# lsl036/STM-Multifrontal-QR-Factorization-Empowered-by-GCN

Hardware: AMD Instinct MI355X
Metric: numerical-factorization GFLOP/s (higher is better)
Workload: dtype f64; 1 GPU; xenon1_colamd_standin: m=49248 n=49248 nnz=1258432 fronts=686 flops/step=5.029e+11, ordering default (COLAMD: qrtest without an ordering argument) (stand-in for xenon1.mtx, absent from the reference checkout); inputs=values resident in HBM, factors left in HBM, parallelism=replica x1, levels=16, retries=0

## Files before the change

include/stmmqr_hip.h:

```cpp
#ifndef STMMQR_HIP_H
#define STMMQR_HIP_H

#include <stddef.h>

#ifdef __cplusplus
extern "C" {
#endif

typedef long stm_long;

#define STMMQR_OK                0
#define STMMQR_ERR_OUT_OF_MEMORY (-2)
#define STMMQR_ERR_TOO_LARGE     (-3)
#define STMMQR_ERR_INVALID       (-4)
#define STMMQR_ERR_DEVICE        (-5)
#define STMMQR_ERR_RESCHEDULE    (-6)


typedef struct stm_sparse_csc {
    size_t nrow, ncol, nzmax;
    void *p, *i, *nz, *x, *z;
    int stype, itype, xtype, dtype, sorted, packed;
} stm_sparse_csc;

typedef struct stm_qr_symbolic {
    stm_long m, n, anz;
    stm_long *Sp, *Sj, *Qfill, *PLinv, *Sleft;
    stm_long nf, maxfn;
    stm_long *Parent, *Child, *Childp, *Super, *Rp, *Rj, *Post;
    stm_long rjsize, do_rank_detection, maxstack, hisize, keepH;
    stm_long *Hip;
    stm_long ntasks, ns;
    stm_long *TaskChildp, *TaskChild, *TaskStack, *TaskFront, *TaskFrontp, *On_stack, *Stack_maxstack;
    stm_long *Fm, *Cm;
} stm_qr_symbolic;

typedef struct stm_qr_numeric {
    double **Rblock;
    double **Stacks;
    stm_long *Stack_size;
    stm_long hisize, n, m, nf, ntasks, ns, maxstack;
    char *Rdead;
    stm_long rank, rank1, maxfrank;
    double norm_E_fro;
    stm_long keepH, rjsize;
    stm_long *HStair;
    double *HTau;
    stm_long *Hii, *HPinv, *Hm, *Hr;
    stm_long maxfm;
} stm_qr_numeric;

typedef struct sparse_common_struct stm_sparse_common;
typedef struct stm_common_layout {
    size_t status, malloc_count, memory_usage, memory_inuse, blas_ok;
    size_t SPQR_grain, SPQR_small, SPQR_shrink, SPQR_flopcount, SPQR_flopcount_bound;
} stm_common_layout;
void stmmqr_set_common_layout(const stm_common_layout *layout);
void stmmqr_get_common_layout(stm_common_layout *layout);
void *stmmqr_cc_malloc(size_t n, size_t size, stm_sparse_common *cc);
void stmmqr_cc_free(size_t n, size_t size, void *p, stm_sparse_common *cc);
void stmmqr_cc_set_status(stm_sparse_common *cc, int code);


stm_qr_numeric *qr_factorize(stm_sparse_csc **Ahandle, stm_long freeA, double tol, stm_long ntol,
                             stm_qr_symbolic *QRsym, stm_sparse_common *cc);

void stmmqr_plan_cache_clear(void);
void stmmqr_free_numeric(stm_qr_numeric **QRnum, stm_sparse_common *cc);

int chunk_getSettings(size_t fchunk, size_t small_, size_t minchunk, size_t minchunk_ratio);

void qr_stranspose2(stm_sparse_csc *A, stm_long *Qfill, stm_long *Sp, stm_long *PLinv, double *Sx, stm_long *W);
void qr_hpinv(stm_qr_symbolic *QRsym, stm_qr_numeric *QRnum, stm_long *W);
stm_long qr_fsize(stm_long f, stm_long *Super, stm_long *Rp, stm_long *Rj, stm_long *Sleft, stm_long *Child,
                  stm_long *Childp, stm_long *Cm, stm_long *Fmap, stm_long *Stair);
void qr_assemble(stm_long f, stm_long fm, int keepH, stm_long *Super, stm_long *Rp, stm_long *Rj, stm_long *Sp,
                 stm_long *Sj, stm_long *Sleft, stm_long *Child, stm_long *Childp, double *Sx, stm_long *Fmap,
                 stm_long *Cm, double **Cblock, stm_long *Hr, stm_long *Stair, stm_long *Hii, stm_long *Hip,
                 double *F, stm_long *Cmap);
stm_long qr_csize(stm_long c, stm_long *Rp, stm_long *Cm, stm_long *Super);
stm_long qr_front(stm_long m, stm_long n, stm_long npiv, double tol, stm_long ntol, stm_long fchunk, double *F,
                  stm_long *Stair, char *Rdead, double *Tau, double *W, double *wscale, double *wssq,
                  stm_sparse_common *cc);
stm_long qr_fcsize(stm_long m, stm_long n, stm_long npiv, stm_long g);
stm_long qr_cpack(stm_long m, stm_long n, stm_long npiv, stm_long g, double *F, double *C);
stm_long qr_rhpack(int keepH, stm_long m, stm_long n, stm_long npiv, stm_long *Stair, double *F, double *R,
                   stm_long *p_rm);
void qr_larftb(int method, stm_long m, stm_long n, stm_long k, stm_long ldc, stm_long ldv, double *V,
               double *Tau, double *C, double *W, stm_sparse_common *cc);


typedef struct stmmqr_symbolic_view {
    stm_long m, n, anz, nf, maxfn, rjsize, hisize, do_rank_detection;
    const stm_long *Sp, *Sj, *Qfill, *PLinv, *Sleft;
    const stm_long *Child, *Childp, *Super, *Rp, *Rj, *Post, *Hip, *Fm;
    stm_long maxstack;
} stmmqr_symbolic_view;

typedef struct stmmqr_stats {
    double flops;
    double ms_total;
    double ms_assemble;
    double ms_front;
    double ms_pack;
    double ms_h2d, ms_d2h;
    double ms_host;
    double bytes_assemble;
    double bytes_pack;
    double flops_update;
    double ms_update;
    stm_long nlaunch;
    stm_long nlevels;
    double ms_panel;
    double ms_small;
    stm_long npanel_launch, nupdate_launch;
    stm_long nsteps;
    double flops_update_pair;
    stm_long retries;
    double device_bytes;
    stm_long reschedules;
} stmmqr_stats;

typedef struct stmmqr_plan stmmqr_plan;

stmmqr_plan *stmmqr_plan_create(const stmmqr_symbolic_view *sym, int device, int *status);
void stmmqr_plan_destroy(stmmqr_plan *plan);

int stmmqr_plan_set_pattern(stmmqr_plan *plan, const stm_long *Ap, const stm_long *Ai);

int stmmqr_factorize_device(stmmqr_plan *plan, const stm_long *Ap, const stm_long *Ai, const double *Ax,
                            int ax_on_device, double tol, stm_long ntol, stmmqr_stats *stats);

int stmmqr_factorize_begin(stmmqr_plan *plan, const stm_long *Ap, const stm_long *Ai, const double *Ax,
                           int ax_on_device, double tol, stm_long ntol);
int stmmqr_factorize_group(stmmqr_plan *plan, int group, int detail);
int stmmqr_factorize_finish(stmmqr_plan *plan, stmmqr_stats *stats);

int stmmqr_plan_set_groups(stmmqr_plan *plan, const int *group );
int stmmqr_plan_front_info(stmmqr_plan *plan, stm_long f, stm_long *info);
int stmmqr_plan_export_front(stmmqr_plan *plan, stm_long f, double *C, stm_long *rows, int c_on_device);
int stmmqr_plan_import_front(stmmqr_plan *plan, stm_long f, stm_long fm, stm_long rank, stm_long cm, const double *C,
                             const stm_long *rows, int c_on_device);

#define STMMQR_GROUP_SHARED  (1 << 30)
#define STMMQR_STEP_PREP     1
#define STMMQR_STEP_PANEL    2
#define STMMQR_STEP_UPDATE   4
#define STMMQR_STEP_GRAM     8
#define STMMQR_STEP_POST     16
int stmmqr_plan_group_steps(stmmqr_plan *plan, int group);
int stmmqr_factorize_step(stmmqr_plan *plan, int group, int step, int what, int cb_first, int cb_stride, int cb_count);
int stmmqr_plan_panel_doubles(stmmqr_plan *plan, stm_long f, stm_long *ndoubles);
int stmmqr_plan_export_panel(stmmqr_plan *plan, stm_long f, stm_long p, double *buf, int on_device);
int stmmqr_plan_import_panel(stmmqr_plan *plan, stm_long f, stm_long p, const double *buf, int on_device);
int stmmqr_plan_export_front_cols(stmmqr_plan *plan, stm_long f, int part, int nparts, double *buf, int on_device,
                                  stm_long *ndoubles);
int stmmqr_plan_import_front_cols(stmmqr_plan *plan, stm_long f, int part, int nparts, const double *buf, int on_device);
typedef struct stmmqr_transport {
    void *ctx;
    int (*send)(void *ctx, const void *dev_buf, size_t bytes, int peer, void *hip_stream);
    int (*recv)(void *ctx, void *dev_buf, size_t bytes, int peer, void *hip_stream);
    int (*group_begin)(void *ctx);
    int (*group_end)(void *ctx);
    int rank, size;
} stmmqr_transport;
int stmmqr_factorize_shared_front(stmmqr_plan *plan, int group, stm_long f, int first_rank, int nranks, const stmmqr_transport *tr);
int stmmqr_factorize_exchange(stmmqr_plan *plan, stm_long nout, const stm_long *out_front, const int *out_peer, stm_long nin,
                              const stm_long *in_front, const int *in_peer, const stmmqr_transport *tr);
int stmmqr_shared_front_gather(stmmqr_plan *plan, stm_long f, int first_rank, int nranks, const stmmqr_transport *tr);
int stmmqr_plan_set_early_end(stmmqr_plan *plan, int mode);
typedef struct stmmqr_shard_phases {
    int nphase;
    const stm_long *out_ptr, *out_front;
    const int *out_peer;
    const stm_long *in_ptr, *in_front;
    const int *in_peer;
    const stm_long *shared_front;
    const int *shared_first, *shared_span;
    const int *has_group;
} stmmqr_shard_phases;
int stmmqr_factorize_phases(stmmqr_plan *plan, const stmmqr_shard_phases *ph, const stmmqr_transport *tr);
int stmmqr_device_copy(void *dst, const void *src, size_t bytes, void *hip_stream);
int stmmqr_rccl_unique_id(char id[128]);
int stmmqr_rccl_transport_create(int world, int rank, const char id[128], stmmqr_transport **out);
void stmmqr_rccl_transport_destroy(stmmqr_transport *tr);
int stmmqr_transport_sendrecv(const stmmqr_transport *tr, const void *sendbuf, size_t sendbytes, int dst, void *recvbuf, size_t recvbytes,
                              int src, void *hip_stream);

int stmmqr_plan_front_rhoff(stmmqr_plan *plan, stm_long f, stm_long *off);

double stmmqr_plan_device_bytes(const stmmqr_plan *plan);

int stmmqr_plan_front_flops(stmmqr_plan *plan, stm_long f, double *out);

int stmmqr_plan_result_sizes(const stmmqr_plan *plan, stm_long *rh_total, stm_long *rank);

int stmmqr_plan_download(stmmqr_plan *plan, double *Stack, stm_long *Rblock_off, char *Rdead, stm_long *HStair,
                         double *HTau, stm_long *Hii, stm_long *HPinv, stm_long *Hm, stm_long *Hr,
                         stm_long *scalars , stmmqr_stats *stats);

int stmmqr_factorize_arrays(const stmmqr_symbolic_view *sym, const stm_long *Ap, const stm_long *Ai,
                            const double *Ax, double tol, stm_long ntol, double *Stack, stm_long stack_cap,
                            stm_long *Rblock_off, char *Rdead, stm_long *HStair, double *HTau, stm_long *Hii,
                            stm_long *HPinv, stm_long *Hm, stm_long *Hr, stm_long *scalars, stmmqr_stats *stats);

int stmmqr_plan_qmult(stmmqr_plan *plan, int method, double *X, stm_long ldx, stm_long nrhs);
int stmmqr_plan_solve(stmmqr_plan *plan, const double *B, stm_long ldb, double *X, stm_long ldx, stm_long nrhs);
int stmmqr_plan_rsolve(stmmqr_plan *plan, int system, const double *B, stm_long ldb, double *X, stm_long ldx,
                       stm_long nrhs);

stm_long stmmqr_front(stm_long m, stm_long n, stm_long npiv, double tol, stm_long ntol, double *F,
                      stm_long *Stair, char *Rdead, double *Tau, double *flops);
int stmmqr_larftb_qtx(stm_long m, stm_long n, stm_long k, stm_long ldc, stm_long ldv, const double *V,
                      const double *Tau, double *C);
int stmmqr_larftb(int method, stm_long m, stm_long n, stm_long k, stm_long ldc, stm_long ldv, const double *V,
                  const double *Tau, double *C);
double stmmqr_last_seam_ms(void);

typedef struct stmmqr_options {
    int panel_width;
    int big_front_cols;
    int verbose;
    int use_graph;
    int panel_algo;
    int split_update;
    int tall_min_rows;
    int lookahead;
    int fused_update;
    int pair_update;
} stmmqr_options;
void stmmqr_get_options(stmmqr_options *opt);
void stmmqr_set_options(const stmmqr_options *opt);

int stmmqr_read_matrix_market(const char *path, stm_long *nrow, stm_long *ncol, stm_long *nnz, stm_long **Ap,
                              stm_long **Ai, double **Ax);
const char *stmmqr_mm_last_error(void);
void stmmqr_free(void *p);

typedef struct stmmqr_relax { stm_long nrelax[3]; double zrelax[3]; } stmmqr_relax;
typedef struct stmmqr_analysis stmmqr_analysis;
void stmmqr_relax_for_qr(stm_long n, stm_long nnz, stmmqr_relax *relax);
int stmmqr_analyze(stm_long m, stm_long n, const stm_long *Ap, const stm_long *Ai, const stm_long *Quser,
                   int do_rank_detection, const stmmqr_relax *relax, stmmqr_analysis **out);
const stm_qr_symbolic *stmmqr_analysis_symbolic(const stmmqr_analysis *a);
int stmmqr_analysis_info(const stmmqr_analysis *a, double *info);
void stmmqr_analysis_free(stmmqr_analysis *a);

typedef struct stmmqr_qr stmmqr_qr;
int stmmqr_sparseqr(int ordering, double tol, stm_long m, stm_long n, const stm_long *Ap, const stm_long *Ai, const double *Ax,
                    const stm_long *Quser, const stmmqr_relax *relax, int device, stmmqr_qr **out);
int stmmqr_sparseqr_symbolic(int ordering, double tol, stm_long m, stm_long n, const stm_long *Ap, const stm_long *Ai,
                             const double *Ax, const stm_long *Quser, const stmmqr_relax *relax, stmmqr_qr **out);
int stmmqr_sparseqr_numeric(stmmqr_qr *qr, int device);
void stmmqr_sparseqr_free(stmmqr_qr *qr);
int stmmqr_sparseqr_info(const stmmqr_qr *qr, double *info);
double stmmqr_sparseqr_tol(const stmmqr_qr *qr);
const stm_long *stmmqr_sparseqr_q1fill(const stmmqr_qr *qr);
const stm_qr_symbolic *stmmqr_sparseqr_symbolic_view(const stmmqr_qr *qr);
stmmqr_plan *stmmqr_sparseqr_plan(stmmqr_qr *qr);
int stmmqr_sparseqr_y(const stmmqr_qr *qr, const stm_long **Yp, const stm_long **Yi, const double **Yx);
int stmmqr_sparseqr_qmult(stmmqr_qr *qr, int method, const double *X, stm_long ldx, stm_long nrow, stm_long ncol, double *Y,
                          stm_long ldy);
int stmmqr_sparseqr_solve(stmmqr_qr *qr, int system, const double *B, stm_long ldb, stm_long nrhs, double *X, stm_long ldx);

void qr_rcount(stm_qr_symbolic *QRsym, stm_qr_numeric *QRnum, stm_long n1rows, stm_long econ, stm_long n2, int getT, stm_long *Ra,
               stm_long *Rb, stm_long *H2p, stm_long *p_nh);
void qr_rconvert(stm_qr_symbolic *QRsym, stm_qr_numeric *QRnum, stm_long n1rows, stm_long econ, stm_long n2, int getT,
                 stm_long *Rap, stm_long *Rai, double *Rax, stm_long *Rbp, stm_long *Rbi, double *Rbx, stm_long *H2p, stm_long *H2i,
                 double *H2x, double *H2Tau);
stm_long qr_trapezoidal(stm_long n, stm_long *Rp, stm_long *Ri, double *Rx, stm_long bncols, stm_long *Qfill,
                        int skip_if_trapezoidal, stm_long **p_Tp, stm_long **p_Ti, double **p_Tx, stm_long **p_Qtrap,
                        stm_sparse_common *cc);
int stmmqr_plan_export_r(stmmqr_plan *plan, const stm_qr_symbolic *sym, stm_long econ, stm_long **Rp, stm_long **Ri, double **Rx,
                         stm_long *nh, stm_long **Hp, stm_long **Hi, double **Hx, double **HTau);
int stmmqr_sparselq(int ordering, double tol, stm_long m, stm_long n, const stm_long *Ap, const stm_long *Ai, const double *Ax,
                    const stmmqr_relax *relax, int device, stmmqr_qr **out);

void stmmqr_shutdown(void);
int stmmqr_device_alloc(size_t bytes, void **ptr);
int stmmqr_device_free(void *ptr);
int stmmqr_device_count(void);
const char *stmmqr_device_name(int device);
const char *stmmqr_last_error(void);
const char *stmmqr_version(void);

#ifdef __cplusplus
}
#endif
#endif
```

stm-multifrontal-qr-factorization-empowered-by-gcn_amd/capi.py:

```python
from __future__ import annotations

import ctypes as C
from pathlib import Path

import numpy as np

_HERE = Path(__file__).resolve().parent
lib_path = _HERE / "libstmmqr_hip.so"

c_long_p = C.POINTER(C.c_long)
c_double_p = C.POINTER(C.c_double)
I64 = np.int64


class StmmqrError(RuntimeError):
    code = 0


ERR_RESCHEDULE = -6


if not lib_path.exists():
    raise ImportError(
        f"{lib_path} is missing: build it with `python -c 'import __graft_entry__ as g; g.build()'` "
        "(hipcc --offload-arch=gfx950).  There is no CPU fallback for this path.")


def _preload_torch_hip_runtime():
    import importlib.util
    import os
    if os.environ.get("STMMQR_SYSTEM_HIP") == "1":
        return
    try:
        spec = importlib.util.find_spec("torch")
    except (ImportError, ValueError):
        spec = None
    if spec is None or not spec.origin:
        return
    rt = Path(spec.origin).parent / "lib" / "libamdhip64.so"
    if rt.exists():
        C.CDLL(str(rt), mode=C.RTLD_GLOBAL)


_preload_torch_hip_runtime()
lib = C.CDLL(str(lib_path))


class SymbolicView(C.Structure):
    _fields_ = [(k, C.c_long) for k in ["m", "n", "anz", "nf", "maxfn", "rjsize", "hisize", "do_rank_detection"]] + \
               [(k, c_long_p) for k in ["Sp", "Sj", "Qfill", "PLinv", "Sleft", "Child", "Childp", "Super", "Rp", "Rj",
                                        "Post", "Hip", "Fm"]] + [("maxstack", C.c_long)]


class Stats(C.Structure):
    _fields_ = [(k, C.c_double) for k in ["flops", "ms_total", "ms_assemble", "ms_front", "ms_pack", "ms_h2d", "ms_d2h",
                                          "ms_host", "bytes_assemble", "bytes_pack", "flops_update", "ms_update"]] + \
               [("nlaunch", C.c_long), ("nlevels", C.c_long), ("ms_panel", C.c_double), ("ms_small", C.c_double),
                ("npanel_launch", C.c_long), ("nupdate_launch", C.c_long), ("nsteps", C.c_long),
                ("flops_update_pair", C.c_double), ("retries", C.c_long), ("device_bytes", C.c_double), ("reschedules", C.c_long)]

    def as_dict(self):
        return {k: getattr(self, k) for k, _ in self._fields_}


class Options(C.Structure):
    _fields_ = [("panel_width", C.c_int), ("big_front_cols", C.c_int), ("verbose", C.c_int), ("use_graph", C.c_int),
                ("panel_algo", C.c_int), ("split_update", C.c_int), ("tall_min_rows", C.c_int),
                ("lookahead", C.c_int), ("fused_update", C.c_int), ("pair_update", C.c_int)]


def _ip(a):
    return None if a is None else a.ctypes.data_as(c_long_p)


def _dp(a):
    return None if a is None else a.ctypes.data_as(c_double_p)


lib.stmmqr_last_error.restype = C.c_char_p
lib.stmmqr_version.restype = C.c_char_p
lib.stmmqr_device_name.restype = C.c_char_p
lib.stmmqr_device_name.argtypes = [C.c_int]
lib.stmmqr_plan_create.restype = C.c_void_p
lib.stmmqr_plan_create.argtypes = [C.POINTER(SymbolicView), C.c_int, C.POINTER(C.c_int)]
lib.stmmqr_plan_destroy.argtypes = [C.c_void_p]
lib.stmmqr_plan_destroy.restype = None
lib.stmmqr_plan_set_pattern.argtypes = [C.c_void_p, c_long_p, c_long_p]
lib.stmmqr_factorize_device.argtypes = [C.c_void_p, c_long_p, c_long_p, C.c_void_p, C.c_int, C.c_double, C.c_long,
                                        C.POINTER(Stats)]
lib.stmmqr_plan_result_sizes.argtypes = [C.c_void_p, c_long_p, c_long_p]
lib.stmmqr_plan_download.argtypes = [C.c_void_p, c_double_p, c_long_p, C.c_char_p, c_long_p, c_double_p, c_long_p,
                                     c_long_p, c_long_p, c_long_p, c_long_p, C.POINTER(Stats)]
lib.stmmqr_front.restype = C.c_long
lib.stmmqr_front.argtypes = [C.c_long, C.c_long, C.c_long, C.c_double, C.c_long, c_double_p, c_long_p, C.c_char_p,
                             c_double_p, c_double_p]
lib.stmmqr_larftb_qtx.argtypes = [C.c_long] * 5 + [c_double_p, c_double_p, c_double_p]
lib.stmmqr_larftb.argtypes = [C.c_int] + [C.c_long] * 5 + [c_double_p, c_double_p, c_double_p]
lib.qr_larftb.restype = None
lib.qr_larftb.argtypes = [C.c_int] + [C.c_long] * 5 + [c_double_p, c_double_p, c_double_p, c_double_p, C.c_void_p]
lib.stmmqr_last_seam_ms.restype = C.c_double
lib.stmmqr_last_seam_ms.argtypes = []
lib.qr_cpack.restype = C.c_long
lib.qr_cpack.argtypes = [C.c_long] * 4 + [c_double_p, c_double_p]
lib.qr_rhpack.restype = C.c_long
lib.qr_rhpack.argtypes = [C.c_int, C.c_long, C.c_long, C.c_long, c_long_p, c_double_p, c_double_p, c_long_p]
lib.qr_fcsize.restype = C.c_long
lib.qr_fcsize.argtypes = [C.c_long] * 4
lib.qr_assemble.restype = None
lib.qr_assemble.argtypes = [C.c_long, C.c_long, C.c_int] + [c_long_p] * 8 + [c_double_p, c_long_p, c_long_p,
                                                                             C.POINTER(c_double_p), c_long_p, c_long_p,
                                                                             c_long_p, c_long_p, c_double_p, c_long_p]
lib.stmmqr_plan_rsolve.argtypes = [C.c_void_p, C.c_int, c_double_p, C.c_long, c_double_p, C.c_long, C.c_long]
lib.stmmqr_read_matrix_market.argtypes = [C.c_char_p, c_long_p, c_long_p, c_long_p, C.POINTER(c_long_p), C.POINTER(c_long_p), C.POINTER(c_double_p)]
lib.qr_fsize.argtypes = [C.c_long] + [c_long_p] * 9
lib.stmmqr_factorize_begin.argtypes = [C.c_void_p, c_long_p, c_long_p, C.c_void_p, C.c_int, C.c_double, C.c_long]
lib.stmmqr_factorize_group.argtypes = [C.c_void_p, C.c_int, C.c_int]
lib.stmmqr_factorize_finish.argtypes = [C.c_void_p, C.POINTER(Stats)]
lib.stmmqr_plan_set_groups.argtypes = [C.c_void_p, C.POINTER(C.c_int)]
lib.stmmqr_plan_set_early_end.argtypes = [C.c_void_p, C.c_int]
lib.stmmqr_plan_front_info.argtypes = [C.c_void_p, C.c_long, c_long_p]
lib.stmmqr_plan_export_front.argtypes = [C.c_void_p, C.c_long, C.c_void_p, c_long_p, C.c_int]
lib.stmmqr_plan_import_front.argtypes = [C.c_void_p, C.c_long, C.c_long, C.c_long, C.c_long, C.c_void_p, c_long_p, C.c_int]
lib.stmmqr_plan_qmult.argtypes = [C.c_void_p, C.c_int, c_double_p, C.c_long, C.c_long]
lib.stmmqr_plan_group_steps.argtypes = [C.c_void_p, C.c_int]
lib.stmmqr_factorize_step.argtypes = [C.c_void_p] + [C.c_int] * 6
lib.stmmqr_plan_panel_doubles.argtypes = [C.c_void_p, C.c_long, c_long_p]
lib.stmmqr_plan_export_panel.argtypes = [C.c_void_p, C.c_long, C.c_long, C.c_void_p, C.c_int]
lib.stmmqr_plan_import_panel.argtypes = [C.c_void_p, C.c_long, C.c_long, C.c_void_p, C.c_int]
lib.stmmqr_plan_export_front_cols.argtypes = [C.c_void_p, C.c_long, C.c_int, C.c_int, C.c_void_p, C.c_int, c_long_p]
lib.stmmqr_plan_import_front_cols.argtypes = [C.c_void_p, C.c_long, C.c_int, C.c_int, C.c_void_p, C.c_int]
lib.stmmqr_plan_front_rhoff.argtypes = [C.c_void_p, C.c_long, c_long_p]
lib.stmmqr_plan_front_flops.argtypes = [C.c_void_p, C.c_long, c_double_p]
lib.stmmqr_plan_device_bytes.argtypes = [C.c_void_p]
lib.stmmqr_plan_device_bytes.restype = C.c_double
lib.stmmqr_plan_solve.argtypes = [C.c_void_p, c_double_p, C.c_long, c_double_p, C.c_long, C.c_long]
lib.stmmqr_get_options.argtypes = [C.POINTER(Options)]
lib.stmmqr_set_options.argtypes = [C.POINTER(Options)]


class TransportC(C.Structure):
    SEND = C.CFUNCTYPE(C.c_int, C.c_void_p, C.c_void_p, C.c_size_t, C.c_int, C.c_void_p)
    RECV = C.CFUNCTYPE(C.c_int, C.c_void_p, C.c_void_p, C.c_size_t, C.c_int, C.c_void_p)
    GRP = C.CFUNCTYPE(C.c_int, C.c_void_p)
    _fields_ = [("ctx", C.c_void_p), ("send", SEND), ("recv", RECV), ("group_begin", GRP), ("group_end", GRP), ("rank", C.c_int),
                ("size", C.c_int)]


lib.stmmqr_factorize_shared_front.argtypes = [C.c_void_p, C.c_int, C.c_long, C.c_int, C.c_int, C.POINTER(TransportC)]


class ShardPhasesC(C.Structure):
    _LP, _IP = C.POINTER(C.c_long), C.POINTER(C.c_int)
    _fields_ = [("nphase", C.c_int), ("out_ptr", _LP), ("out_front", _LP), ("out_peer", _IP), ("in_ptr", _LP), ("in_front", _LP),
                ("in_peer", _IP), ("shared_front", _LP), ("shared_first", _IP), ("shared_span", _IP), ("has_group", _IP)]


lib.stmmqr_factorize_exchange.argtypes = [C.c_void_p, C.c_long, C.POINTER(C.c_long), C.POINTER(C.c_int), C.c_long, C.POINTER(C.c_long),
                                          C.POINTER(C.c_int), C.POINTER(TransportC)]
lib.stmmqr_shared_front_gather.argtypes = [C.c_void_p, C.c_long, C.c_int, C.c_int, C.POINTER(TransportC)]
lib.stmmqr_factorize_phases.argtypes = [C.c_void_p, C.POINTER(ShardPhasesC), C.POINTER(TransportC)]
lib.stmmqr_rccl_unique_id.argtypes = [C.c_char_p]
lib.stmmqr_rccl_transport_create.argtypes = [C.c_int, C.c_int, C.c_char_p, C.POINTER(C.POINTER(TransportC))]
lib.stmmqr_rccl_transport_destroy.restype = None
lib.stmmqr_rccl_transport_destroy.argtypes = [C.POINTER(TransportC)]
lib.stmmqr_transport_sendrecv.argtypes = [C.POINTER(TransportC), C.c_void_p, C.c_size_t, C.c_int, C.c_void_p, C.c_size_t, C.c_int, C.c_void_p]
lib.stmmqr_device_copy.argtypes = [C.c_void_p, C.c_void_p, C.c_size_t, C.c_void_p]


class RcclTransport:

    def __init__(self, dist, device=None):
        import torch
        rank, world = dist.get_rank(), dist.get_world_size()
        ident = C.create_string_buffer(128)
        if rank == 0:
            _check(lib.stmmqr_rccl_unique_id(ident), "stmmqr_rccl_unique_id")
        t = torch.frombuffer(bytearray(ident.raw), dtype=torch.uint8).clone()
        if device is not None and dist.get_backend() == "nccl":
            t = t.to(device)
        dist.broadcast(t, 0)
        raw = bytes(t.cpu().numpy().tobytes())
        self._p = C.POINTER(TransportC)()
        _check(lib.stmmqr_rccl_transport_create(world, rank, raw, C.byref(self._p)), "stmmqr_rccl_transport_create")
        self.rank, self.size = rank, world

    @property
    def ptr(self):
        return self._p

    def sendrecv(self, send_ptr, send_bytes, dst, recv_ptr, recv_bytes, src, stream=None):
        _check(lib.stmmqr_transport_sendrecv(self._p, send_ptr, send_bytes, dst, recv_ptr, recv_bytes, src, stream), "stmmqr_transport_sendrecv")

    def close(self):
        if self._p:
            lib.stmmqr_rccl_transport_destroy(self._p)
            self._p = C.POINTER(TransportC)()


class CallbackTransport:

    def __init__(self, rank, size, send, recv):
        self._send = TransportC.SEND(lambda ctx, buf, nbytes, peer, stream: int(send(buf, nbytes, peer, stream) or 0))
        self._recv = TransportC.RECV(lambda ctx, buf, nbytes, peer, stream: int(recv(buf, nbytes, peer, stream) or 0))
        self._t = TransportC(None, self._send, self._recv, TransportC.GRP(), TransportC.GRP(), rank, size)
        self.rank, self.size = rank, size

    @property
    def ptr(self):
        return C.pointer(self._t)


def device_copy(dst: int, src: int, nbytes: int, stream=None):
    _check(lib.stmmqr_device_copy(C.c_void_p(dst), C.c_void_p(src), nbytes, stream), "stmmqr_device_copy")


def last_error() -> str:
    return lib.stmmqr_last_error().decode()


def device_count() -> int:
    return int(lib.stmmqr_device_count())


def device_name(i: int = 0) -> str:
    return lib.stmmqr_device_name(i).decode()


def get_options() -> dict:
    o = Options()
    lib.stmmqr_get_options(C.byref(o))
    return {k: getattr(o, k) for k, _ in o._fields_}


lib.stmmqr_device_alloc.argtypes = [C.c_size_t, C.POINTER(C.c_void_p)]
lib.stmmqr_device_free.argtypes = [C.c_void_p]


def device_alloc(nbytes: int) -> int:
    p = C.c_void_p()
    _check(lib.stmmqr_device_alloc(nbytes, C.byref(p)), "stmmqr_device_alloc")
    return p.value


def device_free(ptr: int):
    _check(lib.stmmqr_device_free(ptr), "stmmqr_device_free")


def set_options(**kw):
    o = Options()
    lib.stmmqr_get_options(C.byref(o))
    for k, v in kw.items():
        setattr(o, k, v)
    lib.stmmqr_set_options(C.byref(o))


def _check(rc: int, what: str):
    if rc != 0:
        e = StmmqrError(f"{what} failed ({rc}): {last_error()}")
        e.code = int(rc)
        raise e


class QRNumeric:

    def __init__(self, nf, n, m, rjsize, hisize, rh_total):
        self.Stack = np.zeros(max(rh_total, 1))
        self.Rblock_off = np.zeros(max(nf, 1), I64)
        self.Rdead = np.zeros(max(n, 1), np.int8)
        self.HStair = np.zeros(max(rjsize, 1), I64)
        self.HTau = np.zeros(max(rjsize, 1))
        self.Hii = np.zeros(max(hisize, 1), I64)
        self.HPinv = np.zeros(max(m, 1), I64)
        self.Hm = np.zeros(max(nf, 1), I64)
        self.Hr = np.zeros(max(nf, 1), I64)
        self.rh_total = rh_total
        self.rank = self.rank1 = self.maxfrank = self.maxfm = 0
        self.stats = {}


class HipQR:

    def __init__(self, sym: dict, device: int = -1):
        self._keep = {}
        v = SymbolicView()
        for k in ["m", "n", "anz", "nf", "maxfn", "rjsize", "hisize", "do_rank_detection"]:
            setattr(v, k, int(sym[k]))
        for k in ["Sp", "Sj", "Qfill", "PLinv", "Sleft", "Child", "Childp", "Super", "Rp", "Rj", "Post", "Hip", "Fm"]:
            a = sym.get(k)
            if a is not None and np.size(a) == 0 and k == "Qfill":
                a = None
            if a is not None:
                a = np.ascontiguousarray(a, dtype=I64)
                self._keep[k] = a
            setattr(v, k, _ip(a))
        v.maxstack = int(sym.get("maxstack", 0) or 0)
        self.sym = {k: int(sym[k]) for k in ["m", "n", "anz", "nf", "maxfn", "rjsize", "hisize"]}
        st = C.c_int(0)
        self._h = lib.stmmqr_plan_create(C.byref(v), device, C.byref(st))
        if not self._h:
            raise StmmqrError(f"stmmqr_plan_create failed ({st.value}): {last_error()}")

    def close(self):
        if getattr(self, "_h", None):
            lib.stmmqr_plan_destroy(self._h)
            self._h = None

    __del__ = close

    def set_pattern(self, Ap, Ai):
        Ap = np.ascontiguousarray(Ap, I64); Ai = np.ascontiguousarray(Ai, I64)
        _check(lib.stmmqr_plan_set_pattern(self._h, _ip(Ap), _ip(Ai)), "stmmqr_plan_set_pattern")

    def factorize(self, Ax, tol, ntol, Ap=None, Ai=None, device_ptr: int | None = None, detail=False) -> dict:
        st = Stats()
        if detail:
            st.nlaunch = -1
        if Ap is not None:
            Ap = np.ascontiguousarray(Ap, I64); Ai = np.ascontiguousarray(Ai, I64)
        if device_ptr is not None:
            rc = lib.stmmqr_factorize_device(self._h, _ip(Ap), _ip(Ai), C.c_void_p(device_ptr), 1, float(tol), int(ntol),
                                             C.byref(st))
        else:
            Ax = np.ascontiguousarray(Ax, np.float64)
            rc = lib.stmmqr_factorize_device(self._h, _ip(Ap), _ip(Ai), Ax.ctypes.data_as(C.c_void_p), 0, float(tol),
                                             int(ntol), C.byref(st))
        _check(rc, "stmmqr_factorize_device")
        return st.as_dict()

    def set_groups(self, group):
        g = np.ascontiguousarray(group, np.int32)
        assert g.size == self.sym["nf"]
        _check(lib.stmmqr_plan_set_groups(self._h, g.ctypes.data_as(C.POINTER(C.c_int))), "stmmqr_plan_set_groups")

    def set_early_end(self, mode: int):
        _check(lib.stmmqr_plan_set_early_end(self._h, int(mode)), "stmmqr_plan_set_early_end")

    def begin(self, Ax, tol, ntol, Ap=None, Ai=None, device_ptr=None):
        if Ap is not None:
            Ap = np.ascontiguousarray(Ap, I64); Ai = np.ascontiguousarray(Ai, I64)
        if device_ptr is not None:
            rc = lib.stmmqr_factorize_begin(self._h, _ip(Ap), _ip(Ai), C.c_void_p(device_ptr), 1, float(tol), int(ntol))
        else:
            Ax = np.ascontiguousarray(Ax, np.float64)
            rc = lib.stmmqr_factorize_begin(self._h, _ip(Ap), _ip(Ai), Ax.ctypes.data_as(C.c_void_p), 0, float(tol), int(ntol))
        _check(rc, "stmmqr_factorize_begin")

    def run_group(self, g, detail=False):
        _check(lib.stmmqr_factorize_group(self._h, int(g), int(detail)), "stmmqr_factorize_group")

    def finish(self) -> dict:
        st = Stats()
        _check(lib.stmmqr_factorize_finish(self._h, C.byref(st)), "stmmqr_factorize_finish")
        return st.as_dict()

    def front_info(self, f) -> dict:
        info = np.zeros(6, I64)
        _check(lib.stmmqr_plan_front_info(self._h, int(f), _ip(info)), "stmmqr_plan_front_info")
        return dict(zip(["fm", "rank", "cm", "csize", "fn", "fp"], (int(x) for x in info)))

    def export_front(self, f):
        info = self.front_info(f)
        Cb = np.zeros(max(info["csize"], 1)); rows = np.zeros(max(info["cm"], 1), I64)
# ... 551 lines not shown
```

stm-multifrontal-qr-factorization-empowered-by-gcn_amd/csrc/stmmqr_host.cpp:

```cpp
#include "stmmqr_plan.h"

thread_local std::string g_err;
stmmqr_options g_opt = {STM_NB, 64, 0, 0, 0, 1, STM_TALL_MIN, 2, 0, 4};
size_t g_chunk[4] = {32, 5000, 4, 4};

stm_common_layout g_layout = {
     1004,  1032,  1040,  1048,
     1100,  1104,  1112,  1120,
     1128,  1136};

int fail(int code, const std::string &msg)
{
    g_err = msg;
    if (g_opt.verbose) fprintf(stderr, "[stmmqr_hip] error %d: %s\n", code, msg.c_str());
    return code;
}

namespace {

const int LDS_CAP_DOUBLES = STM_LDS_CAP_DOUBLES;
const int LDS_CAP_SMALL = 15360;

std::mutex g_side_mu;
hipStream_t g_side[64] = {};
// ... 153 lines not shown
            *objs[(size_t)i].out = at;
            peak = std::max(peak, top);
        }
    }
    return peak;
}

std::pair<long long, long long> timeline_offsets(stmmqr_plan &P, const std::vector<char> &kept, int nstep, bool apply)
{
    const long nf = P.nf;
    std::vector<long long> foff((size_t)std::max(1L, nf), 0), coff((size_t)std::max(1L, nf), 0);
    long long base = 0;
    for (long f = 0; f < nf; f++)
        if (kept[(size_t)f]) { foff[(size_t)f] = base; base += (long long)P.fs[f].ld * P.fs[f].fn; }
    std::vector<TlObj> fo, co;
    for (long f = 0; f < nf; f++) {
        const FrontSym &s = P.fs[f];
        if (!kept[(size_t)f]) fo.push_back({(long long)s.ld * s.fn, P.f_t0[f], P.f_t1[f], &foff[(size_t)f]});
        const long cn = s.fn - s.fp, fm = s.fm_ub;
        const long cm = P.do_rank ? std::min(fm, cn) : std::min(std::max(fm - std::min(fm, (long)s.fp), 0L), cn);
        const long long csz = (long long)cm * (cm + 1) / 2 + (long long)cm * (cn - cm);
        if (apply) P.c_slot[(size_t)f] = csz;
        co.push_back({csz, P.f_t1[f], std::max(P.f_t1[f], P.c_t1[f]), &coff[(size_t)f]});
    }
    const long long fpeak = timeline_first_fit(fo, base, nstep), cpeak = timeline_first_fit(co, 0, nstep);
    if (apply)
        for (long f = 0; f < nf; f++) { P.fs[f].foff = foff[(size_t)f]; P.fs[f].coff = coff[(size_t)f]; }
    return {std::max(1LL, fpeak), std::max(1LL, cpeak)};
}

void build_schedule(stmmqr_plan &P, std::vector<int> &tslot)
{
    P.sched_gen++;
    P.tune = getenv("STMMQR_TUNE") ? atoi(getenv("STMMQR_TUNE")) : 0;
    P.tall_min = g_opt.tall_min_rows;
    P.plan_algo = g_opt.panel_algo;
    P.ca_min = getenv("STMMQR_CA_MIN") ? atoi(getenv("STMMQR_CA_MIN")) : STM_CA_MIN_ROWS;
    const long nf = P.nf;
    int ngroups = 1;
    for (long f = 0; f < nf; f++) ngroups = std::max(ngroups, P.group[f] + 1);
    {
        bool whole = (ngroups == 1) && nf > 0;
        for (long f = 0; f < nf && whole; f++) whole = (P.group[f] == 0) && !((size_t)f < P.shared.size() && P.shared[(size_t)f]);
        const char *ev = getenv("STMMQR_RECYCLE");
        const int mode = ev ? atoi(ev) : 1;
        long long slabs = 0;
        for (long f = 0; f < nf; f++) slabs += (long long)P.fs[f].ld * P.fs[f].fn;
        P.recycle = whole && !P.overflowed && (mode == 2 || (mode == 1 && slabs >= (32LL << 20)));
    }
    auto is_big = [&](int f) {
        const FrontSym &s = P.fs[f];
        return s.fn >= g_opt.big_front_cols && s.fm_ub >= 64;
    };
    const int sched_policy = getenv("STMMQR_SCHED") ? atoi(getenv("STMMQR_SCHED")) : 0;
    const long pair_min = getenv("STMMQR_PAIR_MIN") ? atol(getenv("STMMQR_PAIR_MIN")) : STM_PAIR_MIN_ROWS;
    auto is_pair = [&](int f) {
        const FrontSym &s = P.fs[f];
        if ((size_t)f < P.shared.size() && P.shared[f]) return false;
        return g_opt.pair_update && is_big(f) && s.fm_est >= pair_min && s.npanels >= 4;
    };
    P.sweep = (g_opt.pair_update == 4) ? 4 : 2;
    P.pair_front.assign(std::max(1L, nf), 0);
    for (long f = 0; f < nf; f++) P.pair_front[f] = (P.group[f] >= 0 && is_pair((int)f)) ? 1 : 0;
    P.ypoff.assign(std::max(1L, nf), -1);
    P.yp_doubles = 0;
    for (long f = 0; f < nf; f++)
        if (P.pair_front[f]) {
            P.ypoff[f] = P.yp_doubles;
            P.yp_doubles += (long long)((P.fs[f].fn + 31) / 32) * (P.sweep * STM_NB * 32);
        }
    tslot.assign(std::max(1L, nf), 0);
    P.glevels.assign(ngroups, std::vector<Level>());
    P.gsteps.assign(ngroups, std::vector<Step>());
    P.lists.clear();
    P.wlists.clear();
    P.tslots = 1;
    P.gp_slabs = 1;
    P.wp_doubles = 0;
    P.wp2_doubles = 0;
    {
        bool whole = (ngroups == 1) && nf > 0;
        for (long f = 0; f < nf && whole; f++) whole = (P.group[f] == 0) && !((size_t)f < P.shared.size() && P.shared[(size_t)f]);
        const bool early = (whole || P.early_phased) && !P.full_schedule && !(getenv("STMMQR_EARLY_END") && atoi(getenv("STMMQR_EARLY_END")) == 0);
        const int slack = getenv("STMMQR_EARLY_SLACK") ? atoi(getenv("STMMQR_EARLY_SLACK")) : 0;
        for (long f = 0; f < nf; f++) {
            FrontSym &s = P.fs[f];
            s.nsched = s.npanels;
            if (early && is_big((int)f) && !is_pair((int)f) && P.group[f] >= 0 && !((size_t)f < P.shared.size() && P.shared[(size_t)f])) s.nsched = std::min(s.npanels, std::min(s.fm_est, s.fn) / STM_NB + 1 + slack);
        }
        P.early_end = early;
    }
    for (int grp = 0; grp < ngroups; grp++) {
        std::vector<int> level(nf, -1), start(nf, 0), end(nf, 0);
        int nlev = 0, nstep = 0;
        for (long kf = 0; kf < nf; kf++) {
            const long f = P.Post[kf];
            if (P.group[f] != grp) continue;
            int lv = 0, t0 = 0;
            for (long q = P.Childp[f]; q < P.Childp[f + 1]; q++) {
                const long ch = P.Child[q];
                if (P.group[ch] != grp) continue;
                lv = std::max(lv, level[ch] + 1);
                t0 = std::max(t0, end[ch]);
            }
            level[f] = lv;
            nlev = std::max(nlev, lv + 1);
            start[f] = t0;
            end[f] = t0 + (is_big((int)f) ? P.fs[f].nsched : 1);
            nstep = std::max(nstep, end[f]);
        }
        std::vector<int> lstart(nf, 0), lend(nf, 0);
        int nstep_level = 0;
        {
            std::vector<int> lvl_end(nlev + 1, 0);
            for (int lv = 0; lv < nlev; lv++) {
                int e1 = lvl_end[lv];
                for (long kf = 0; kf < nf; kf++) {
                    const long f = P.Post[kf];
                    if (P.group[f] != grp || level[f] != lv) continue;
                    lstart[f] = lvl_end[lv];
                    lend[f] = lstart[f] + (is_big((int)f) ? P.fs[f].nsched : 1);
                    e1 = std::max(e1, lend[f]);
                }
                lvl_end[lv + 1] = e1;
            }
            nstep_level = lvl_end[nlev];
        }
        const bool use_level = sched_policy == 1 || (sched_policy == 0 && 100L * nstep > 97L * nstep_level);
        if (use_level) {
            start = lstart; end = lend;
            nstep = nstep_level;
        }
        std::vector<std::vector<int>> byl(nlev);
        for (long kf = 0; kf < nf; kf++)
            if (P.group[P.Post[kf]] == grp) byl[level[P.Post[kf]]].push_back((int)P.Post[kf]);
        std::vector<Level> &LV = P.glevels[grp];
        LV.assign(nlev, Level());
        for (int lv = 0; lv < nlev; lv++) {
            Level &L = LV[lv];
            std::vector<int> small, big;
            for (int f : byl[lv]) (is_big(f) ? big : small).push_back(f);
            std::stable_sort(big.begin(), big.end(), [&](int a, int b) { return P.fs[a].npanels > P.fs[b].npanels; });
            L.all_off = (int)P.lists.size();
            L.n_small = (int)small.size(); L.n_big = (int)big.size(); L.n_all = L.n_small + L.n_big;
            P.lists.insert(P.lists.end(), small.begin(), small.end());
            P.lists.insert(P.lists.end(), big.begin(), big.end());
        }
        std::vector<std::vector<std::pair<int, int>>> panel_at;
        std::vector<std::vector<int>> small_at;
        if (use_level || sched_policy == 2) {
            panel_at.assign(nstep, {});
            small_at.assign(nstep, {});
            for (long kf = 0; kf < nf; kf++) {
                const int f = (int)P.Post[kf];
                if (P.group[f] != grp) continue;
                if (!is_big(f)) { small_at[start[f]].push_back(f); continue; }
                for (int q = 0; q < P.fs[f].nsched; q++) panel_at[start[f] + q].push_back({f, q});
            }
        } else {
            std::vector<int> parent_in(nf, -1), pend(nf, 0), tails(nf, 0);
            for (long f = 0; f < nf; f++) {
                if (P.group[f] != grp) continue;
                for (long q = P.Childp[f]; q < P.Childp[f + 1]; q++)
                    if (P.group[P.Child[q]] == grp) { parent_in[P.Child[q]] = (int)f; pend[f]++; }
            }
            for (long kf = nf; kf-- > 0;) {
                const long f = P.Post[kf];
                if (P.group[f] != grp) continue;
                tails[f] = (is_big((int)f) ? P.fs[f].nsched : 1) + (parent_in[f] >= 0 ? tails[parent_in[f]] : 0);
            }
            std::vector<int> ready;
            for (long kf = 0; kf < nf; kf++)
                if (P.group[P.Post[kf]] == grp && pend[P.Post[kf]] == 0) ready.push_back((int)P.Post[kf]);
            const double ride = getenv("STMMQR_RIDE") ? atof(getenv("STMMQR_RIDE")) : 1.0;
            struct Fly { int f, p; };
            std::vector<Fly> fly;
            while (!ready.empty() || !fly.empty()) {
                std::vector<int> newly, smalls;
                for (int f : ready) {
                    if (is_big(f)) fly.push_back({f, 0});
                    else smalls.push_back(f);
                }
                panel_at.push_back({});
                small_at.push_back(smalls);
                auto finish = [&](int f) {
                    const int pf = parent_in[f];
                    if (pf >= 0 && --pend[pf] == 0) newly.push_back(pf);
                };
                if (!fly.empty()) {
                    auto rem = [&](const Fly &e) { return tails[e.f] - e.p; };
                    auto rows = [&](const Fly &e) { return stm_panel_rows_est(P.fs[e.f], e.p); };
                    int rl = 0, env = 0;
                    for (const Fly &e : fly) rl = std::max(rl, rem(e));
                    for (const Fly &e : fly)
                        if (rem(e) == rl) env = std::max(env, rows(e));
                    std::vector<Fly> keep;
                    for (Fly &e : fly) {
                        if (rem(e) == rl || rows(e) <= ride * env) {
                            panel_at.back().push_back({e.f, e.p});
                            if (++e.p >= P.fs[e.f].nsched) { finish(e.f); continue; }
                        }
                        keep.push_back(e);
                    }
                    fly.swap(keep);
                }
                for (int f : smalls) finish(f);
                ready.swap(newly);
            }
            nstep = (int)panel_at.size();
        }
        std::vector<std::vector<int>> starting(nstep), ending(nstep);
        std::vector<int> pan_now(nf, 0);
        for (int t = 0; t < nstep; t++) {
            for (int f : small_at[t]) starting[t].push_back(f);
            for (const auto &fp : panel_at[t]) {
                if (fp.second == 0) starting[t].push_back(fp.first);
                if (fp.second == P.fs[fp.first].nsched - 1) ending[t].push_back(fp.first);
            }
        }
        for (int t = 0, carry_from = -1; t < nstep; t++) {
            const bool flush = (t + 1 == nstep) || !starting[t + 1].empty();
            if (carry_from >= 0 && carry_from != t) {
                ending[t].insert(ending[t].begin(), ending[carry_from].begin(), ending[carry_from].end());
                ending[carry_from].clear();
            }
            carry_from = (flush || ending[t].empty()) ? -1 : t;
            if (!flush && !ending[t].empty()) carry_from = t;
        }
        std::vector<Step> &SV = P.gsteps[grp];
        SV.assign(nstep, Step());
        std::vector<int> active, freeslots;
        int nslots = 0;
        for (int t = 0; t < nstep; t++) {
            Step &S = SV[t];
            std::vector<int> small, big;
            for (int f : starting[t]) (is_big(f) ? big : small).push_back(f);
            S.start_off = (int)P.lists.size();
            S.n_small = (int)small.size(); S.n_start = (int)(small.size() + big.size());
            P.lists.insert(P.lists.end(), small.begin(), small.end());
            P.lists.insert(P.lists.end(), big.begin(), big.end());
            S.asm_parts_off = (int)P.lists.size();
            long maxfm_small = 0;
            for (int i = 0; i < S.n_start; i++) {
                const FrontSym &s = P.fs[P.lists[S.start_off + i]];
                const long work = (long)s.fm_ub * s.fn;
                static const long pg = getenv("STMMQR_PART_GRAIN") ? atol(getenv("STMMQR_PART_GRAIN")) : 2048, pc = getenv("STMMQR_PART_CAP") ? atol(getenv("STMMQR_PART_CAP")) : 4096;
                const int parts = (int)std::min(pc, std::max(1L, (work + pg - 1) / pg));
                P.lists.push_back(parts);
                S.asm_maxparts = std::max(S.asm_maxparts, parts);
                if (i < S.n_small) maxfm_small = std::max(maxfm_small, (long)s.fm_ub);
            }
            S.lds_small = (int)std::min((long)LDS_CAP_SMALL, (((maxfm_small + 63) & ~63L) | 1) * STM_NB + 64);
            if (S.n_small > 0) S.lds_small = std::max(S.lds_small, STM_NB * 128 + 64);
            for (int f : big) {
                if (!freeslots.empty()) { tslot[f] = freeslots.back(); freeslots.pop_back(); }
                else tslot[f] = nslots++;
            }
            active.clear();
            for (const auto &fp : panel_at[t]) { active.push_back(fp.first); pan_now[fp.first] = fp.second; }
            auto work_at = [&](int f) { return (long)stm_upd_ncb(P.fs[f], pan_now[f]) * stm_upd_nsl(P.fs[f]); };
            auto cls = [&](int f) { return !is_pair(f) ? 0 : 1 + pan_now[f] % P.sweep; };
            std::stable_sort(active.begin(), active.end(), [&](int a, int b) {
                return cls(a) != cls(b) ? cls(a) < cls(b) : work_at(a) > work_at(b);
            });
            S.act_off = (int)P.lists.size();
            S.n_act = (int)active.size();
            P.lists.insert(P.lists.end(), active.begin(), active.end());
            S.plist_off = (int)P.lists.size();
            for (int f : active) P.lists.push_back(pan_now[f]);
            S.wp_off = (int)P.wlists.size();
            long long wp = 0, ncbsum = 0;
            long maxfm_big = 0;
            for (int f : active) {
                const FrontSym &s = P.fs[f];
                const int p = pan_now[f];
                const int ncb = stm_upd_ncb(s, p), nsl = stm_upd_nsl(s);
                P.wlists.push_back(wp);
                if (is_pair(f))
                    wp += std::max((long long)(ncb + P.sweep - 1) * (P.sweep == 4 ? stm_quad_slots(nsl, P.tune) : stm_pair_slots(nsl, P.tune)) *
                                       (P.sweep * STM_NB * 32),
                                   (P.sweep + 1LL) * nsl * (STM_NB * 32));
                else
                    wp += (long long)(ncb + 1) * nsl * (STM_NB * 32);
                const int k = cls(f);
                if (k == 0) {
                    S.n_norm++;
                    ncbsum += ncb;
                    S.maxcb = std::max(S.maxcb, ncb);
                    S.maxsl = std::max(S.maxsl, nsl);
                } else {
                    S.n_pk[k - 1]++;
                    S.maxsl_pk[k - 1] = std::max(S.maxsl_pk[k - 1], nsl);
                    if (k == P.sweep) S.maxcbp_po = std::max(S.maxcbp_po, ncb - 1);
                }
                S.nsub = std::max(S.nsub, stm_tall_launches(s, p, P.tall_min));
                S.nca = std::max(S.nca, stm_ca_slabs(s));
                (stm_use_ca(s, p, g_opt.panel_algo, P.ca_min) ? S.nca_use : S.npipe_use)++;
                P.gp_slabs = std::max(P.gp_slabs, stm_ca_slabs(s));
                maxfm_big = std::max(maxfm_big, (long)s.fm_ub);
                if (!stm_tall_panel(s, p, P.tall_min) && !stm_use_ca(s, p, g_opt.panel_algo, P.ca_min))
                    S.lds_plan = std::max(S.lds_plan, stm_front_lds(s));
                if (stm_tall_panel(s, p, P.tall_min) && !stm_use_ca(s, p, g_opt.panel_algo, P.ca_min))
                    S.lds_plan = std::max(S.lds_plan, STM_NB * STM_WP_ROWS);
            }
            S.lds_big = (int)std::min((long)LDS_CAP_DOUBLES, (((maxfm_big + 63) & ~63L) | 1) * STM_NB + 64);
            S.split = (S.maxsl >= 3 || ncbsum >= 512) ? 1 : 0;
            P.wp_doubles = std::max(P.wp_doubles, wp);
            if (S.n_sweep() == 0) P.wp2_doubles = std::max(P.wp2_doubles, wp);
            S.cpk_off = (int)P.lists.size();
            S.n_cpk = (int)ending[t].size();
            P.lists.insert(P.lists.end(), ending[t].begin(), ending[t].end());
            S.cpk_parts_off = (int)P.lists.size();
            for (int f : ending[t]) {
                const FrontSym &s = P.fs[f];
                const long cn = s.fn - s.fp;
                const long work = cn * std::min((long)s.fm_ub, cn);
                static const long pg = getenv("STMMQR_PART_GRAIN") ? atol(getenv("STMMQR_PART_GRAIN")) : 2048, pc = getenv("STMMQR_PART_CAP") ? atol(getenv("STMMQR_PART_CAP")) : 4096;
                const int parts = (int)std::min(pc, std::max(1L, (work + pg - 1) / pg));
                P.lists.push_back(parts);
                S.cpk_maxparts = std::max(S.cpk_maxparts, parts);
                freeslots.push_back(tslot[f]);
            }
        }
        P.tslots = std::max(P.tslots, nslots);
        if (P.recycle && grp == 0) {
            P.f_t0.assign((size_t)std::max(1L, nf), 0); P.f_t1.assign((size_t)std::max(1L, nf), 0); P.c_t1.assign((size_t)std::max(1L, nf), 0);
            for (int t = 0; t < nstep; t++) {
                for (int f : starting[t]) { P.f_t0[(size_t)f] = t; if (!is_big(f)) P.f_t1[(size_t)f] = t; }
                for (int f : ending[t]) P.f_t1[(size_t)f] = t;
            }
            for (long f = 0; f < nf; f++) {
                const int par = P.fs[f].parent;
                P.c_t1[(size_t)f] = (par >= 0) ? P.f_t0[(size_t)par] : P.f_t1[(size_t)f];
            }
            std::vector<int> bysize((size_t)nf);
            for (long f = 0; f < nf; f++) bysize[(size_t)f] = (int)f;
            std::stable_sort(bysize.begin(), bysize.end(), [&](int a, int b) {
                return (long long)P.fs[a].ld * P.fs[a].fn > (long long)P.fs[b].ld * P.fs[b].fn; });
            long long best = -1;
            int bestk = 0;
            for (int k = 0; k <= std::min(3L, nf); k++) {
                std::vector<char> kp((size_t)std::max(1L, nf), 0);
                long long rec = 0;
                for (int q = 0; q < k; q++) kp[(size_t)bysize[(size_t)q]] = 1;
                for (long f = 0; f < nf; f++) if (!kp[(size_t)f]) rec += (long long)P.fs[f].ld * P.fs[f].fn;
                const auto pk = timeline_offsets(P, kp, nstep, false);
                const long long cap = (P.maxstack > 0) ? std::min((long long)P.maxstack, rec) : rec;
                const long long tot = pk.first + pk.second + cap;
                if (best < 0 || tot < best - best / 50) { best = tot; bestk = k; }
            }
            P.kept.assign((size_t)std::max(1L, nf), 0);
            long long rec = 0;
            for (int q = 0; q < bestk; q++) P.kept[(size_t)bysize[(size_t)q]] = 1;
            for (long f = 0; f < nf; f++) if (!P.kept[(size_t)f]) rec += (long long)P.fs[f].ld * P.fs[f].fn;
            P.rh_cap = std::max(1LL, (P.maxstack > 0) ? std::min((long long)P.maxstack, rec) : rec);
            if (!P.rh_grow && P.rh_est_total > 0) {
                const double sc = getenv("STMMQR_RH_EST_SCALE") ? atof(getenv("STMMQR_RH_EST_SCALE")) : 1.0;
                const long long est = (long long)((double)P.rh_est_total * sc);
                P.rh_cap = std::max(1LL, std::min(P.rh_cap, est + est / 8 + 4096));
            }
            const auto pk = timeline_offsets(P, P.kept, nstep, true);
            P.farena = pk.first; P.carena = pk.second;
            P.has_c.assign((size_t)std::max(1L, nf), 1);
            for (int t = 0; t < nstep; t++) {
                Step &S = SV[t];
                std::vector<int> rhp;
                for (int f : starting[t]) if (!is_big(f) && !P.kept[(size_t)f]) rhp.push_back(f);
                for (int f : ending[t]) if (!P.kept[(size_t)f]) rhp.push_back(f);
                S.rhp_off = (int)P.lists.size();
                S.n_rhp = (int)rhp.size();
                P.lists.insert(P.lists.end(), rhp.begin(), rhp.end());
                S.rhp_parts_off = (int)P.lists.size();
                for (int f : rhp) {
                    const int parts = std::min(256, std::max(1, P.fs[f].fn / 16));
                    P.lists.push_back(parts);
                    S.rhp_maxparts = std::max(S.rhp_maxparts, parts);
                }
            }
            P.fs_scr = P.fs;
            P.scr_doubles = 1;
            for (size_t l = 0; l < LV.size(); l++) {
                long long o = 0;
                for (int q = 0; q < LV[l].n_all; q++) {
                    const int f = P.lists[(size_t)(LV[l].all_off + q)];
                    if (P.kept[(size_t)f]) continue;
                    P.fs_scr[(size_t)f].foff = o;
                    o += (long long)P.fs[f].ld * P.fs[f].fn;
                }
                P.scr_doubles = std::max(P.scr_doubles, o);
            }
        }
    }
    P.own_off = (int)P.lists.size();
    P.n_own = 0;
    for (long kf = 0; kf < nf; kf++)
        if (P.group[P.Post[kf]] >= 0) { P.lists.push_back((int)P.Post[kf]); P.n_own++; }
    P.rh_parts_off = (int)P.lists.size();
    P.rh_maxparts = 1;
    for (long kf = 0; kf < nf; kf++) {
        if (P.group[P.Post[kf]] < 0) continue;
        const FrontSym &s = P.fs[P.Post[kf]];
        int parts = std::min(256, std::max(1, s.fn / 16));
        P.lists.push_back(parts);
        P.rh_maxparts = std::max(P.rh_maxparts, parts);
    }
    P.post_off = (int)P.lists.size();
    for (long kf = 0; kf < nf; kf++) P.lists.push_back((int)P.Post[kf]);
    if (P.lists.empty()) P.lists.push_back(0);
    if (P.wlists.empty()) P.wlists.push_back(0);
    P.h_tslot = tslot;
}

int upload_recycle(stmmqr_plan &P)
{
    if (!P.d_rhtop.p) LCHK(P.d_rhtop.alloc(2));
    if (!P.d_fin.p || P.d_fin.n < (size_t)std::max(1L, P.nf)) LCHK(P.d_fin.alloc((size_t)std::max(1L, P.nf)));
    HIPCHK(hipMemsetAsync(P.d_rhtop.p, 0, 2 * sizeof(long long), P.stream));
    if (!P.recycle) return 0;
    LCHK(P.d_kept.upload(P.kept, P.stream));
    HIPCHK(hipStreamSynchronize(P.stream));
    P.d_scr.release();
    P.d_RH.release();
    return 0;
}

int build_plan(stmmqr_plan &P, const stmmqr_symbolic_view &v)
{
    P.m = v.m; P.n = v.n; P.anz = v.anz; P.nf = v.nf; P.maxfn = v.maxfn; P.rjsize = v.rjsize;
    P.hisize = v.hisize; P.do_rank = v.do_rank_detection ? 1 : 0;
    P.maxstack = v.maxstack > 0 ? v.maxstack : 0;
    const long m = v.m, n = v.n, nf = v.nf;
    if (m < 0 || n < 0 || nf < 0) return fail(STMMQR_ERR_INVALID, "negative dimension");
    if (v.anz >= (1L << 31) - 1 || v.rjsize >= (1L << 31) - 1 || v.hisize >= (1L << 31) - 1 || m >= (1L << 30) ||
        n >= (1L << 30))
        return fail(STMMQR_ERR_TOO_LARGE, "problem exceeds the 32-bit device index range");
    auto cp = [](std::vector<long> &dst, const stm_long *src, long cnt) {
        dst.assign(src, src + (cnt > 0 ? cnt : 0));
    };
    cp(P.Sp, v.Sp, m + 1); cp(P.Sj, v.Sj, v.anz); cp(P.PLinv, v.PLinv, m); cp(P.Sleft, v.Sleft, n + 2);
    cp(P.Child, v.Child, nf + 1); cp(P.Childp, v.Childp, nf + 2); cp(P.Super, v.Super, nf + 1);
    cp(P.Rp, v.Rp, nf + 1); cp(P.Rj, v.Rj, v.rjsize); cp(P.Post, v.Post, nf); cp(P.Hip, v.Hip, nf + 1);
    P.has_qfill = v.Qfill != nullptr;
    if (P.has_qfill) cp(P.Qfill, v.Qfill, n);

    std::vector<long> parent(nf, -1);
    for (long f = 0; f < nf; f++)
        for (long q = P.Childp[f]; q < P.Childp[f + 1]; q++) parent[P.Child[q]] = f;

    P.Fm.assign(nf, 0);
    if (v.Fm) {
        for (long f = 0; f < nf; f++) P.Fm[f] = v.Fm[f];
    } else {
        std::vector<long> cmub(nf, 0);
        for (long kf = 0; kf < nf; kf++) {
            const long f = P.Post[kf];
            const long fp = P.Super[f + 1] - P.Super[f], fn = P.Rp[f + 1] - P.Rp[f];
            long fm = P.Sleft[P.Super[f + 1]] - P.Sleft[P.Super[f]];
            for (long q = P.Childp[f]; q < P.Childp[f + 1]; q++) fm += cmub[P.Child[q]];
            P.Fm[f] = fm;
            const long cn = fn - fp;
            cmub[f] = P.do_rank ? std::min(fm, cn) : std::min(std::max(fm - std::min(fm, fp), 0L), cn);
        }
    }

    std::vector<long> fmest(nf, 0), cmest(nf, 0);
    for (long kf = 0; kf < nf; kf++) {
        const long f = P.Post[kf];
        const long fp = P.Super[f + 1] - P.Super[f], fn = P.Rp[f + 1] - P.Rp[f];
        long fe = P.Sleft[P.Super[f + 1]] - P.Sleft[P.Super[f]];
        for (long q = P.Childp[f]; q < P.Childp[f + 1]; q++) fe += cmest[P.Child[q]];
        fmest[f] = std::min(fe, P.Fm[f]);
        cmest[f] = std::min(std::max(fe - std::min(fe, fp), 0L), fn - fp);
    }

    P.fs.assign(nf, FrontSym());
    long long foff = 0, coff = 0, tpan_total = 0;
    for (long kf = 0; kf < nf; kf++) {
        const long f = P.Post[kf];
        FrontSym &s = P.fs[f];
        const long fp = P.Super[f + 1] - P.Super[f], fn = P.Rp[f + 1] - P.Rp[f];
        const long fm = P.Fm[f];
        if (fm * fn >= (1L << 36)) return fail(STMMQR_ERR_TOO_LARGE, "a single front exceeds 2^36 entries");
        s.fn = (int)fn; s.fp = (int)fp; s.col1 = (int)P.Super[f]; s.rp = (int)P.Rp[f]; s.hip = (int)P.Hip[f];
        s.child0 = (int)P.Childp[f]; s.child1 = (int)P.Childp[f + 1];
        s.srow0 = (int)P.Sleft[P.Super[f]]; s.srow1 = (int)P.Sleft[P.Super[f + 1]];
        s.fm_ub = (int)fm;
        s.fm_est = (int)fmest[f];
        s.ld = (int)std::max(2L, (fm + 1) & ~1L);
        s.npanels = (int)((fn + STM_NB - 1) / STM_NB);
        s.tpan = (int)tpan_total;
        tpan_total += s.npanels;
        {
            const long qbig_min = getenv("STMMQR_QBIG_MIN") ? atol(getenv("STMMQR_QBIG_MIN")) : (1L << 20);
            s.qbig = (fm * fn >= qbig_min && fn >= 1) ? 1 : 0;
        }
        s.parent = (int)parent[f];
        s.foff = 0; s.coff = 0;
    }
    (void)foff; (void)coff;
    P.tpanels = tpan_total;

    std::vector<int> Rjrel(std::max(1L, v.rjsize), 0), Sjrel(std::max(1L, v.anz), 0), Sj0(std::max(1L, m), -1);
    {
        std::vector<int> Fmap(std::max(1L, n), -1);
        for (long f = 0; f < nf; f++) {
            const long p1 = P.Rp[f], fn = P.Rp[f + 1] - p1;
            for (long j = 0; j < fn; j++) Fmap[P.Rj[p1 + j]] = (int)j;
            for (long r = P.fs[f].srow0; r < P.fs[f].srow1; r++)
                for (long p = P.Sp[r]; p < P.Sp[r + 1]; p++) Sjrel[p] = Fmap[P.Sj[p]];
            for (long q = P.Childp[f]; q < P.Childp[f + 1]; q++) {
                const long c = P.Child[q];
                const long fpc = P.Super[c + 1] - P.Super[c], pc = P.Rp[c] + fpc, cn = P.Rp[c + 1] - pc;
                for (long cj = 0; cj < cn; cj++) Rjrel[pc + cj] = Fmap[P.Rj[pc + cj]];
                P.bytes_assemble_idx += 4.0 * (double)(2 * cn);
            }
        }
        for (long r = 0; r < m; r++)
            if (P.Sp[r + 1] > P.Sp[r]) Sj0[r] = (int)P.Sj[P.Sp[r]];
        P.bytes_assemble_idx += 4.0 * (double)v.anz;
    }
    P.rh_est_total = 0;
    {
        std::vector<long> stair;
        for (long kf = 0; kf < nf; kf++) {
            const long f = P.Post[kf];
            const long fp = P.fs[f].fp, fn = P.fs[f].fn, fm = fmest[f];
            stair.assign((size_t)fn + 1, 0);
            for (long j = 0; j < fp; j++) stair[(size_t)j] = P.Sleft[P.Super[f] + j + 1] - P.Sleft[P.Super[f] + j];
            for (long q = P.Childp[f]; q < P.Childp[f + 1]; q++) {
                const long c = P.Child[q];
                const long fpc = P.Super[c + 1] - P.Super[c], pc = P.Rp[c] + fpc;
                for (long i = 0; i < cmest[c]; i++) stair[(size_t)Rjrel[(size_t)(pc + i)]]++;
            }
            long run = 0;
            for (long j = 0; j < fn; j++) { run += stair[(size_t)j]; stair[(size_t)j] = run; }
            long g = 0, rm = 0;
            long long sz = 0;
            for (long k = 0; k < fn; k++) {
                long t;
                if (g >= fm) t = (k < fp) ? 0 : fm;
                else { t = std::min(fm, std::max(g + 1, stair[(size_t)k])); g++; }
                if (k < fp) { if (t > 0) rm++; sz += (t > 0) ? t : rm; }
                else { const long h = std::min(rm + (k - fp) + 1, fm); sz += rm + std::max(t - h, 0L); }
            }
            P.rh_est_total += sz;
        }
    }

    P.group.assign(nf, 0);
    assign_arenas(P);
    std::vector<int> tslot;
    build_schedule(P, tslot);

    size_t freeb = 0, totalb = 0;
    HIPCHK(hipMemGetInfo(&freeb, &totalb));
    const double need = 8.0 * 1024.0 * (double)P.tpanels * 1.05 + 64.0 * (double)(v.rjsize + v.anz);
    if (need > 0.92 * (double)freeb)
        return fail(STMMQR_ERR_OUT_OF_MEMORY, "the plan's index arrays do not fit in free HBM");
    hipStream_t st = P.stream;
    auto up32 = [&](DevBuf<int> &d, const std::vector<long> &h) {
        std::vector<int> t(h.begin(), h.end());
        return d.upload(t, st);
    };
    LCHK(P.d_fs.upload(P.fs, st));
    LCHK(P.d_fnum.alloc(std::max(1L, nf)));
    HIPCHK(hipMemsetAsync(P.d_fnum.p, 0, std::max(1L, nf) * sizeof(FrontNum), st));
    LCHK(P.d_T.alloc((size_t)STM_PD_RING * P.tslots * STM_NB * STM_NB));
    LCHK(P.d_Gp.alloc((size_t)P.tslots * (P.gp_slabs + 1) * STM_NB * STM_NB));
    LCHK(P.d_Tall.alloc((size_t)std::max(1LL, P.tpanels) * STM_NB * STM_NB));
    LCHK(P.d_Wp.alloc((size_t)P.wp_doubles));
    LCHK(P.d_Ypend.alloc((size_t)std::max(1LL, P.yp_doubles)));
    LCHK(P.d_ypoff.upload(P.ypoff, st));
    LCHK(P.d_Wp2.alloc((size_t)std::max(1LL, P.wp2_doubles)));
    P.wcnt_n = (size_t)(P.wp_doubles / (STM_NB * 32) + 1);
    LCHK(P.d_wcnt.alloc(P.wcnt_n));
    LCHK(P.d_wcnt2.alloc(P.wcnt_n));
    LCHK(P.d_wflag.alloc(P.wcnt_n));
    if (!P.d_abort.p) LCHK(P.d_abort.alloc(4));
    LCHK(P.d_wflag2.alloc(P.wcnt_n));
    HIPCHK(hipMemset(P.d_wcnt.p, 0, P.wcnt_n * sizeof(int)));
    HIPCHK(hipMemset(P.d_wcnt2.p, 0, P.wcnt_n * sizeof(int)));
    LCHK(P.d_tslot.upload(tslot, st));
    LCHK(P.d_Sx.alloc((size_t)v.anz));
    LCHK(P.d_Ax.alloc((size_t)v.anz));
    LCHK(P.d_smap.alloc((size_t)v.anz));
    LCHK(up32(P.d_Sp, P.Sp));
    LCHK(P.d_Sjrel.upload(Sjrel, st));
    LCHK(P.d_Sj0.upload(Sj0, st));
    LCHK(up32(P.d_Sleft, P.Sleft));
    LCHK(up32(P.d_Child, P.Child));
    LCHK(P.d_Rjrel.upload(Rjrel, st));
    LCHK(P.d_Stair.alloc((size_t)v.rjsize));
    LCHK(P.d_Tau.alloc((size_t)v.rjsize));
    LCHK(P.d_Hii.alloc((size_t)v.hisize));
    LCHK(P.d_Cmap.alloc((size_t)v.rjsize));
    LCHK(P.d_Cursor.alloc((size_t)v.rjsize));
    LCHK(P.d_Rhoff.alloc((size_t)v.rjsize));
    LCHK(P.d_Rboff.alloc((size_t)std::max(1L, nf)));
    LCHK(P.d_total.alloc(1));
    LCHK(P.d_dbg.alloc(2048));
    LCHK(P.d_amax.alloc(1));
    LCHK(P.d_sig.alloc(2));
    HIPCHK(hipMemsetAsync(P.d_dbg.p, 0, 2048 * sizeof(unsigned long long), st));
    LCHK(P.d_Rdead.alloc((size_t)std::max(1L, n)));
    LCHK(P.d_lists.upload(P.lists, st));
    LCHK(P.d_wlists.upload(P.wlists, st));
    HIPCHK(hipStreamSynchronize(st));
    LCHK(upload_recycle(P));
    return 0;
}

int set_pattern(stmmqr_plan &P, const stm_long *Ap, const stm_long *Ai)
{
    const long m = P.m, n = P.n;
    if (!Ap || !Ai) return fail(STMMQR_ERR_INVALID, "Ap/Ai are required");
    if (Ap[n] != P.anz) return fail(STMMQR_ERR_INVALID, "nnz(A) differs from the symbolic analysis");
    std::vector<long> W(P.Sp.begin(), P.Sp.begin() + m);
    std::vector<int> smap(std::max(1L, P.anz), 0);
    for (long col = 0; col < n; col++) {
        const long j = P.has_qfill ? P.Qfill[col] : col;
        for (long p = Ap[j]; p < Ap[j + 1]; p++) {
            const long i = Ai[p];
            if (i < 0 || i >= m) return fail(STMMQR_ERR_INVALID, "row index out of range");
            smap[W[P.PLinv[i]]++] = (int)p;
        }
    }
    if (P.anz > 0)
        HIPCHK(hipMemcpyAsync(P.d_smap.p, smap.data(), (size_t)P.anz * sizeof(int), hipMemcpyHostToDevice, P.stream));
    HIPCHK(hipStreamSynchronize(P.stream));
    P.pattern_set = true;
    return 0;
}

int reset_factorization(stmmqr_plan &P)
{
    hipStream_t st = P.stream;
    LCHK(ensure_arenas(P));
    if (!P.recycle) HIPCHK(hipMemsetAsync(P.d_F.p, 0, (size_t)P.farena * sizeof(double), st));
    HIPCHK(hipMemsetAsync(P.d_rhtop.p, 0, 2 * sizeof(long long), st));
    HIPCHK(hipMemsetAsync(P.d_Rdead.p, 0, (size_t)std::max(1L, P.n), st));
    HIPCHK(hipMemsetAsync(P.d_fnum.p, 0, (size_t)std::max(1L, P.nf) * sizeof(FrontNum), st));
    HIPCHK(hipMemsetAsync(P.d_wcnt.p, 0, P.wcnt_n * sizeof(int), st));
    HIPCHK(hipMemsetAsync(P.d_wcnt2.p, 0, P.wcnt_n * sizeof(int), st));
    HIPCHK(hipMemsetAsync(P.d_wflag.p, 0, P.wcnt_n * sizeof(int), st));
    HIPCHK(hipMemsetAsync(P.d_wflag2.p, 0, P.wcnt_n * sizeof(int), st));
    HIPCHK(hipMemsetAsync(P.d_abort.p, 0, 4 * sizeof(int), st));
    LCHK(stm_launch_sigma(P.d_Ax.p, (int)P.anz, P.d_amax.p, P.d_sig.p, st));
    LCHK(stm_launch_gather_sx(P.d_Ax.p, P.d_smap.p, P.d_Sx.p, (int)P.anz, st));
    P.stats.nlaunch += 6;
    return 0;
}

int reset_group(stmmqr_plan &P, int grp)
{
    hipStream_t st = P.stream;
    const FrontNum zero = FrontNum();
    for (long f = 0; f < P.nf; f++) {
        if (P.group[f] != grp) continue;
        const FrontSym &s = P.fs[f];
        HIPCHK(hipMemsetAsync(P.d_F.p + s.foff, 0, (size_t)s.ld * (size_t)s.fn * sizeof(double), st));
        HIPCHK(hipMemcpyAsync(P.d_fnum.p + f, &zero, sizeof zero, hipMemcpyHostToDevice, st));
        if (s.fp > 0) HIPCHK(hipMemsetAsync(P.d_Rdead.p + s.col1, 0, (size_t)s.fp, st));
    }
    HIPCHK(hipMemsetAsync(P.d_wcnt.p, 0, P.wcnt_n * sizeof(int), st));
    HIPCHK(hipMemsetAsync(P.d_wcnt2.p, 0, P.wcnt_n * sizeof(int), st));
    HIPCHK(hipMemsetAsync(P.d_wflag.p, 0, P.wcnt_n * sizeof(int), st));
    HIPCHK(hipMemsetAsync(P.d_wflag2.p, 0, P.wcnt_n * sizeof(int), st));
    HIPCHK(hipMemsetAsync(P.d_abort.p, 0, 3 * sizeof(int), st));
    if (P.recycle) HIPCHK(hipMemsetAsync(P.d_rhtop.p, 0, 2 * sizeof(long long), st));
    HIPCHK(hipStreamSynchronize(st));
    return 0;
}


static unsigned la_event_flags()
{
    const bool sysfence = getenv("STMMQR_LA_SYSFENCE") && atoi(getenv("STMMQR_LA_SYSFENCE")) != 0;
    return hipEventDisableTiming | (sysfence ? 0u : (unsigned)hipEventDisableSystemFence);
}

int run_schedule(stmmqr_plan &P, bool detail, int grp, const StepReq *req = nullptr)
{
    hipStream_t st = P.stream;
    DevCtx c = P.ctx();
    if (req) c.cbskip = std::max(1, req->cb_stride) - 1;
    const int *L0 = P.d_lists.p;
    long nlaunch = 0;
    enum { CAT_ASM = 0, CAT_SMALL = 1, CAT_PANEL = 2, CAT_UPD = 3, CAT_CPK = 4 };
    int cur_step = 0;
    auto timed = [&](int cat, auto &&fn) -> int {
        if (!detail) return fn();
        if (P.evused == P.evpairs.size()) {
            stmmqr_plan::EvPair q = {nullptr, nullptr, 0, 0};
            HIPCHK(hipEventCreate(&q.a));
            HIPCHK(hipEventCreate(&q.b));
            P.evpairs.push_back(q);
        }
        stmmqr_plan::EvPair &q = P.evpairs[P.evused++];
        q.cat = cat;
        q.step = cur_step;
        HIPCHK(hipEventRecord(q.a, st));
        int e = fn();
        if (e) return e;
        HIPCHK(hipEventRecord(q.b, st));
        return 0;
    };
    const int t_asm = CAT_ASM, t_front = CAT_SMALL, t_panel = CAT_PANEL, t_upd = CAT_UPD, t_cpk = CAT_CPK;

    if (grp < 0 || grp >= (int)P.gsteps.size()) return fail(STMMQR_ERR_INVALID, "no such front group");
    const std::vector<Step> &SV = P.gsteps[grp];
    auto prep = [&](const Step &S, hipStream_t q) -> int {
        const int *starting = L0 + S.start_off;
        if (S.n_start > 0) {
            int e = timed(t_asm, [&]() -> int {
                if (P.recycle) { LCHK(stm_launch_zero_slabs(c, starting, S.n_start, S.asm_maxparts, q)); nlaunch++; }
                LCHK(stm_launch_setup(c, starting, S.n_start, q));
                LCHK(stm_launch_assemble(c, starting, L0 + S.asm_parts_off, S.n_start, S.asm_maxparts, q));
                return 0;
            });
            if (e) return e;
            nlaunch += 2;
        }
        if (S.n_small > 0) {
            int e = timed(t_front, [&]() -> int {
                LCHK(stm_launch_front_wg(c, starting, S.n_small, S.lds_small, q));
                return 0;
            });
            if (e) return e;
            nlaunch++;
        }
        return 0;
    };
    auto panels = [&](const Step &S) -> int {
        const int *act = L0 + S.act_off, *pl = L0 + S.plist_off;
        return timed(t_panel, [&]() -> int {
            if (S.nca_use && !P.serial_panels) { LCHK(stm_launch_panel_ca(c, act, pl, S.n_act, S.nca, 1, st)); nlaunch++; }
            if (S.npipe_use || P.serial_panels) {
                const int lds = (P.serial_panels || (c.dbg & (64 | 256))) ? S.lds_big : S.lds_plan;
                LCHK(stm_launch_panel(c, act, pl, S.n_act, S.nsub, 1, lds, st));
                nlaunch++;
            }
            return 0;
        });
    };
    auto update = [&](const Step &S, int cb0, int ncb, bool gram, double *Wp, hipStream_t q) -> int {
        const bool split = S.split && g_opt.split_update;
        const bool whole = (cb0 == 0 && gram);
        const bool pairs = whole && S.n_sweep() > 0;
        if (S.n_norm <= 0 || (ncb <= 0 && !(gram && split))) {
            if (!pairs) return 0;
        }
        const int *act = L0 + S.act_off, *pl = L0 + S.plist_off;
        const bool main_ws = (Wp == P.d_Wp.p);
        int *wcnt = main_ws ? P.d_wcnt.p : P.d_wcnt2.p;
        const long long *wl = P.d_wlists.p + S.wp_off;
        return timed(t_upd, [&]() -> int {
            if (S.n_norm > 0 && (ncb > 0 || (gram && split))) {
                if (split && g_opt.fused_update && S.maxsl <= 256 && !P.serial_panels && c.cbskip == 0) {
                    const int epoch = (int)(&S - SV.data()) + 1 + grp * (1 << 20);
                    LCHK(stm_launch_update_fused(c, act, pl, S.n_norm, cb0, ncb, S.maxsl, Wp, wl, wcnt,
                                                 main_ws ? P.d_wflag.p : P.d_wflag2.p, epoch, gram ? 1 : 0, q));
                    nlaunch++;
                } else if (split) {
                    LCHK(stm_launch_update_split(c, act, pl, S.n_norm, cb0, ncb, S.maxsl, Wp, wl, wcnt, gram ? 1 : 0, q));
                    nlaunch += 2;
                } else {
                    LCHK(stm_launch_update(c, act, pl, S.n_norm, cb0, ncb, q));
                    nlaunch++;
                }
            }
            if (pairs) {
                int o = S.n_norm;
                for (int r = 0; r < P.sweep; r++) {
                    const int n = S.n_pk[r];
                    if (n <= 0) continue;
                    LCHK(stm_launch_update_split(c, act + o, pl + o, n, 0, P.sweep - r, S.maxsl_pk[r], Wp, wl + o, wcnt, 1, q));
                    nlaunch += 2;
                    if (r == P.sweep - 1) {
                        if (P.sweep == 4) LCHK(stm_launch_update_quad(c, act + o, pl + o, n, S.maxcbp_po, S.maxsl_pk[r], Wp, wl + o, wcnt, q));
                        else LCHK(stm_launch_update_pair(c, act + o, pl + o, n, S.maxcbp_po, S.maxsl_pk[r], Wp, wl + o, wcnt, q));
                        nlaunch += 3;
                    }
                    o += n;
                }
            }
            return 0;
        });
    };
    auto update_b0_fused = [&](const Step &S, hipStream_t q) -> int {
        const int *act = L0 + S.act_off, *pl = L0 + S.plist_off;
        const long long *wl = P.d_wlists.p + S.wp_off;
        const int epoch = (int)(&S - SV.data()) + 1 + grp * (1 << 20);
        nlaunch++;
        return timed(t_upd, [&]() -> int {
            LCHK(stm_launch_update_fused(c, act, pl, S.n_norm, 0, 1, S.maxsl, P.d_Wp.p, wl, P.d_wcnt.p, P.d_wflag.p, epoch, 1, q));
            return 0;
        });
    };
    auto post = [&](const Step &S, hipStream_t q) -> int {
        if (S.n_cpk <= 0 && !(P.recycle && S.n_rhp > 0)) return 0;
        return timed(t_cpk, [&]() -> int {
            if (S.n_cpk > 0) { LCHK(stm_launch_cpack(c, L0 + S.cpk_off, L0 + S.cpk_parts_off, S.n_cpk, S.cpk_maxparts, q)); nlaunch++; }
            if (P.recycle && S.n_rhp > 0) {
                LCHK(stm_launch_rh_count(c, L0 + S.rhp_off, S.n_rhp, q));
                LCHK(stm_launch_rh_copy(c, L0 + S.rhp_off, L0 + S.rhp_parts_off, S.n_rhp, S.rhp_maxparts, P.d_RH.p, q));
                nlaunch += 2;
            }
            return 0;
        });
    };
    if (req) {
        if (req->step < 0 || req->step >= (int)SV.size()) return fail(STMMQR_ERR_INVALID, "no such step in the group");
        const Step &S = SV[(size_t)req->step];
        cur_step = req->step;
        int e = 0;
        if (req->what & STMMQR_STEP_PREP) e = prep(S, st);
        if (!e && (req->what & STMMQR_STEP_PANEL) && S.n_act > 0) e = panels(S);
        if (!e && (req->what & (STMMQR_STEP_UPDATE | STMMQR_STEP_GRAM)) && S.n_act > 0) {
            if (S.n_sweep() > 0) return fail(STMMQR_ERR_INVALID, "pair-update fronts cannot be stepped (mark the front STMMQR_GROUP_SHARED)");
            int nmine = 0;
            if ((req->what & STMMQR_STEP_UPDATE) && req->cb_first >= 0 && req->cb_first < S.maxcb)
                nmine = (S.maxcb - req->cb_first + c.cbskip) / (1 + c.cbskip);
            if (req->cb_count >= 0) nmine = std::min(nmine, req->cb_count);
            e = update(S, std::max(0, req->cb_first), nmine, (req->what & STMMQR_STEP_GRAM) != 0, P.d_Wp.p, st);
        }
        if (!e && (req->what & STMMQR_STEP_POST)) e = post(S, st);
        P.stats.nlaunch += nlaunch;
        return e;
    }
    const long la_min = getenv("STMMQR_LA_MIN") ? atol(getenv("STMMQR_LA_MIN")) : 2500;
    const int la_fused_rows = getenv("STMMQR_LA_FUSED_ROWS") ? atoi(getenv("STMMQR_LA_FUSED_ROWS")) : 5120;
    const long la_min_fused = getenv("STMMQR_LA_MIN_FUSED") ? atol(getenv("STMMQR_LA_MIN_FUSED")) : 1500;
    const long la_slots = 2 * (getenv("STMMQR_SIDE_RESERVE") ? std::max(0L, atol(getenv("STMMQR_SIDE_RESERVE"))) : 32L);
    auto b0_fused = [&](const Step &S) -> bool {
        if (la_fused_rows <= 0 || !S.split || !g_opt.split_update || S.maxsl > 256 || S.n_sweep() > 0 || c.cbskip != 0) return false;
        long wgs = 0;
        for (int i = 0; i < S.n_norm; i++) wgs += 2L * stm_upd_nsl(P.fs[P.lists[S.act_off + i]]);
        if (wgs > la_slots) return false;
        for (int i = 0; i < S.n_act; i++)
            if (stm_panel_rows_est(P.fs[P.lists[S.act_off + i]], P.lists[S.plist_off + i]) > la_fused_rows) return false;
        return true;
    };
    const long la_maxpwg = getenv("STMMQR_LA_MAXPWG") ? atol(getenv("STMMQR_LA_MAXPWG")) : 48;
    auto worth_it = [&](const Step &S) -> bool {
        long tiles = 0, pwg = 0;
        for (int i = 0; i < S.n_act; i++) {
            const FrontSym &fsym = P.fs[P.lists[S.act_off + i]];
            const int p = P.lists[S.plist_off + i];
            const int ncb = stm_upd_ncb(fsym, p);
            if (ncb > 1) tiles += (long)(ncb - 1) * ((stm_panel_rows_est(fsym, p) + STM_UPD_SLAB - 1) / STM_UPD_SLAB);
            pwg += stm_use_ca(fsym, p, P.plan_algo, P.ca_min) ? stm_ca_slabs(fsym) : stm_tall_launches(fsym, p, P.tall_min);
        }
        return tiles >= (b0_fused(S) ? std::min(la_min, la_min_fused) : la_min) && pwg <= la_maxpwg && S.n_sweep() == 0;
    };
    const bool pass = g_opt.lookahead >= 2 && !detail && !P.serial_panels && c.cbskip == 0 && g_opt.split_update && !(c.dbg & 512) &&
                      !(getenv("STMMQR_PASSENGERS") && atoi(getenv("STMMQR_PASSENGERS")) == 0);
    bool la = g_opt.lookahead && !pass && !detail && !P.serial_panels && SV.size() > 1;
    if (la) {
        bool any = false;
        for (const Step &S : SV)
            if (S.n_act > 0 && S.maxcb > 1 && worth_it(S)) { any = true; break; }
        la = any;
    }
    if (pass) {
        const long fw_max = getenv("STMMQR_PASS_MAXWG") ? atol(getenv("STMMQR_PASS_MAXWG")) : 384;
        const int pass_rows = getenv("STMMQR_PASS_ROWS") ? atoi(getenv("STMMQR_PASS_ROWS")) : 16384;
        const double pass_k = getenv("STMMQR_PASS_K") ? atof(getenv("STMMQR_PASS_K")) : 1e30;
        const long pass_tiles = getenv("STMMQR_PASS_TILES") ? atol(getenv("STMMQR_PASS_TILES")) : (1L << 40);
        const int abl = getenv("STMMQR_PASS_ABL") ? atoi(getenv("STMMQR_PASS_ABL")) : 0;
        const Step *pend = nullptr;
        auto flush_alone = [&]() -> int {
            if (!pend) return 0;
            const Step &Q = *pend;
            pend = nullptr;
            LCHK(stm_launch_update_c(c, L0 + Q.act_off, L0 + Q.plist_off, Q.n_norm, 1, Q.maxcb - 1, Q.maxsl, P.d_Wp2.p,
                                     P.d_wlists.p + Q.wp_off, st));
            nlaunch++;
            return 0;
        };
        for (const Step &S : SV) {
            cur_step = (int)(&S - SV.data());
            int e = prep(S, st);
            if (e) return e;
            if (S.n_act > 0) {
                const int *act = L0 + S.act_off, *pl = L0 + S.plist_off;
                if (S.nca_use && !S.npipe_use && pend && !(abl & 6) && !(getenv("STMMQR_CA_RIDERS") && atoi(getenv("STMMQR_CA_RIDERS")) == 0)) {
                    const Step &Q = *pend;
                    pend = nullptr;
                    LCHK(stm_launch_panel_ca_pc(c, act, pl, S.n_act, S.nca, 1, L0 + Q.act_off, L0 + Q.plist_off, Q.n_norm, 1, Q.maxcb - 1, Q.maxsl,
                                                P.d_Wp2.p, P.d_wlists.p + Q.wp_off, st));
                    nlaunch++;
                } else if (S.nca_use) { LCHK(stm_launch_panel_ca(c, act, pl, S.n_act, S.nca, 1, st)); nlaunch++; }
                if (S.npipe_use) {
                    const int lds = (c.dbg & (64 | 256)) ? S.lds_big : S.lds_plan;
                    if (pend && (abl & 2)) pend = nullptr;
                    if (pend) {
                        long tiles = 0;
                        for (int i = 0; i < pend->n_norm; i++) {
                            const FrontSym &fsym = P.fs[P.lists[pend->act_off + i]];
                            const int pp = P.lists[pend->plist_off + i];
                            const int ncb = stm_upd_ncb(fsym, pp);
                            if (ncb > 1) tiles += (long)(ncb - 1) * ((stm_panel_rows_est(fsym, pp) + STM_UPD_SLAB - 1) / STM_UPD_SLAB);
                        }
                        int prow = 0;
                        for (int i = 0; i < S.n_act; i++) prow = std::max(prow, stm_panel_rows_est(P.fs[P.lists[S.act_off + i]], P.lists[S.plist_off + i]));
                        const double panel_us = prow <= 512 ? 25.0 : prow <= 4096 ? 48.0 : 72.0;
                        if ((tiles > pass_tiles || (double)tiles > pass_k * panel_us) && (e = flush_alone())) return e;
                    }
                    if (pend && (abl & 4)) {
                        LCHK(stm_launch_panel(c, act, pl, S.n_act, S.nsub, 1, lds, st));
                        if (abl & 8) {
                            const Step &Q = *pend;
                            pend = nullptr;
                            LCHK(stm_launch_panel_pc(c, act, pl, -1, S.nsub, 1, lds, L0 + Q.act_off, L0 + Q.plist_off, Q.n_norm, 1, Q.maxcb - 1,
                                                     Q.maxsl, P.d_Wp2.p, P.d_wlists.p + Q.wp_off, st));
                        }
                        if ((e = flush_alone())) return e;
                    } else if (pend) {
                        const Step &Q = *pend;
                        pend = nullptr;
                        LCHK(stm_launch_panel_pc(c, act, pl, S.n_act, S.nsub, 1, lds, L0 + Q.act_off, L0 + Q.plist_off, Q.n_norm, 1, Q.maxcb - 1,
                                                 Q.maxsl, P.d_Wp2.p, P.d_wlists.p + Q.wp_off, st));
                    } else
                        LCHK(stm_launch_panel(c, act, pl, S.n_act, S.nsub, 1, lds, st));
                    nlaunch++;
                } else if ((e = flush_alone()))
                    return e;
                long fwg = 0;
                int rows_max = 0;
                for (int i = 0; i < S.n_norm; i++) {
                    fwg += 2L * stm_upd_nsl(P.fs[P.lists[S.act_off + i]]);
                    rows_max = std::max(rows_max, stm_panel_rows_est(P.fs[P.lists[S.act_off + i]], P.lists[S.plist_off + i]));
                }
                const bool ride = S.split && S.n_sweep() == 0 && S.n_norm > 0 && S.maxcb > 1 && S.maxsl <= 256 && fwg <= fw_max &&
                                  rows_max <= pass_rows && !g_opt.fused_update;
                if (ride) {
                    const int epoch = cur_step + 1 + grp * (1 << 20);
                    if (abl & 4) {
                        LCHK(stm_launch_update_fw(c, act, pl, S.n_norm, 1, S.maxsl, P.d_Wp.p, P.d_wlists.p + S.wp_off, P.d_wcnt.p, P.d_wflag.p,
                                                  epoch, P.d_Wp2.p, P.d_wcnt2.p, st));
                        LCHK(stm_launch_update_w(c, act, pl, S.n_norm, 1, S.maxcb - 1, S.maxsl, P.d_Wp2.p, P.d_wlists.p + S.wp_off, P.d_wcnt2.p, st));
                    } else
                    LCHK(stm_launch_update_fw(c, act, pl, S.n_norm, (abl & 1) ? 1 : S.maxcb, S.maxsl, P.d_Wp.p, P.d_wlists.p + S.wp_off, P.d_wcnt.p,
                                              P.d_wflag.p, epoch, P.d_Wp2.p, P.d_wcnt2.p, st));
                    nlaunch++;
                    pend = &S;
                } else if ((e = update(S, 0, S.maxcb, true, P.d_Wp.p, st)))
                    return e;
            }
            if (pend && P.early_end && (S.n_cpk > 0 || (P.recycle && S.n_rhp > 0)) && (e = flush_alone())) return e;
            if ((e = post(S, st))) return e;
        }
        int e = flush_alone();
        if (e) return e;
    } else if (!la) {
        for (const Step &S : SV) {
            cur_step = (int)(&S - SV.data());
            int e = prep(S, st);
            if (!e && S.n_act > 0) e = panels(S);
            if (!e && S.n_act > 0) e = update(S, 0, S.maxcb, true, P.d_Wp.p, st);
            if (!e) e = post(S, st);
            if (e) return e;
        }
    } else {
        const size_t ns = SV.size();
        for (auto *v : {&P.ev_main, &P.ev_prep, &P.ev_side})
            while (v->size() < ns + 1) {
                hipEvent_t ev = nullptr;
                HIPCHK(hipEventCreateWithFlags(&ev, la_event_flags()));
                v->push_back(ev);
            }
        hipStream_t sd = P.side;
        long side_ev = -1;
        bool prep_on_side = false;
        int e = 0;
        for (size_t t = 0; t < ns; t++) {
            const Step &S = SV[t];
            if (prep_on_side) HIPCHK(hipStreamWaitEvent(st, P.ev_prep[t], 0));
            else {
                if (S.n_start > 0 && side_ev >= 0) { HIPCHK(hipStreamWaitEvent(st, P.ev_side[side_ev], 0)); side_ev = -1; }
                if ((e = prep(S, st))) return e;
            }
            prep_on_side = false;
            if (S.n_act > 0 && (e = panels(S))) return e;
            const bool offload = S.n_act > 0 && S.maxcb > 1 && worth_it(S) && !(P.early_end && (S.n_cpk > 0 || (P.recycle && S.n_rhp > 0)));
            if (!offload) {
                if (S.n_act > 0) {
                    if (side_ev >= 0) { HIPCHK(hipStreamWaitEvent(st, P.ev_side[side_ev], 0)); side_ev = -1; }
                    if ((e = update(S, 0, S.maxcb, true, P.d_Wp.p, st))) return e;
                }
                if ((e = post(S, st))) return e;
                continue;
            }
            if (b0_fused(S)) {
                if (side_ev >= 0) { HIPCHK(hipStreamWaitEvent(st, P.ev_side[side_ev], 0)); side_ev = -1; }
                if ((e = update_b0_fused(S, st))) return e;
                HIPCHK(hipEventRecord(P.ev_main[t], st));
            } else {
                if ((e = update(S, 0, 0, true, P.d_Wp.p, st))) return e;
                HIPCHK(hipEventRecord(P.ev_main[t], st));
                if (side_ev >= 0) { HIPCHK(hipStreamWaitEvent(st, P.ev_side[side_ev], 0)); side_ev = -1; }
                if ((e = update(S, 0, 1, false, P.d_Wp.p, st))) return e;
            }
            HIPCHK(hipStreamWaitEvent(sd, P.ev_main[t], 0));
            if ((e = post(S, sd))) return e;
            if (t + 1 < ns && SV[t + 1].n_start > 0) {
                if ((e = prep(SV[t + 1], sd))) return e;
                HIPCHK(hipEventRecord(P.ev_prep[t + 1], sd));
                prep_on_side = true;
            }
            if ((e = update(S, 1, S.maxcb - 1, false, P.d_Wp2.p, sd))) return e;
            HIPCHK(hipEventRecord(P.ev_side[t], sd));
            side_ev = (long)t;
        }
        if (side_ev >= 0) HIPCHK(hipStreamWaitEvent(st, P.ev_side[side_ev], 0));
    }
    P.stats.nlaunch += nlaunch;
    P.stats.nlevels += (long)P.glevels[grp].size();
    P.stats.nsteps += (long)P.gsteps[grp].size();
    return 0;
}

int run_pack(stmmqr_plan &P)
{
    hipStream_t st = P.stream;
    const DevCtx c = P.ctx();
    const int *L0 = P.d_lists.p;
    if (P.recycle) {
        std::vector<int> kl;
        for (long f = 0; f < P.nf; f++) if (P.kept[(size_t)f]) kl.push_back((int)f);
        if (!kl.empty()) {
            DevBuf<int> d_kl;
            LCHK(d_kl.upload(kl, st));
            DevCtx ck = c;
            ck.rh_top = nullptr;
            LCHK(stm_launch_rh_count(ck, d_kl.p, (int)kl.size(), st));
            HIPCHK(hipStreamSynchronize(st));
        }
        LCHK(stm_launch_rh_scan(c, L0 + P.post_off, (int)P.nf, P.d_total.p, P.d_fin.p, st));
        long long total = 0, top[2] = {0, 0};
        HIPCHK(hipMemcpyAsync(&total, P.d_total.p, sizeof(long long), hipMemcpyDeviceToHost, st));
        HIPCHK(hipMemcpyAsync(top, P.d_rhtop.p, 2 * sizeof(long long), hipMemcpyDeviceToHost, st));
        HIPCHK(hipStreamSynchronize(st));
        P.rh_total = total;
        P.stats.nlaunch += 2;
        if (top[1] != 0) {
            if (!P.rh_grow) P.rh_grow = 1;
            else P.overflowed = true;
            P.arena_overflow = true;
            return fail(STMMQR_ERR_OUT_OF_MEMORY, "the packed factors exceed the R+H arena of the slab recycling");
        }
        return 0;
    }
    LCHK(stm_launch_rh_count(c, L0 + P.own_off, P.n_own, st));
    LCHK(stm_launch_rh_scan(c, L0 + P.post_off, (int)P.nf, P.d_total.p, P.d_Rboff.p, st));
    long long total = 0;
    HIPCHK(hipMemcpyAsync(&total, P.d_total.p, sizeof(long long), hipMemcpyDeviceToHost, st));
    HIPCHK(hipStreamSynchronize(st));
    P.rh_total = total;
    if ((size_t)total > P.d_RH.n) LCHK(P.d_RH.alloc((size_t)(total + total / 64 + 1024)));
    LCHK(stm_launch_rh_copy(c, L0 + P.own_off, L0 + P.rh_parts_off, P.n_own, P.rh_maxparts, P.d_RH.p, st));
    P.stats.nlaunch += 3;
    return 0;
}

}

int stm_run_schedule(stmmqr_plan &P, bool detail, int grp, const StepReq *req) { return run_schedule(P, detail, grp, req); }
int stm_ensure_device(int device) { return ensure_device(device); }

extern "C" {

const char *stmmqr_version(void) { return "stmmqr_hip 0.1 (gfx950)"; }
const char *stmmqr_last_error(void) { return g_err.c_str(); }
void stmmqr_get_options(stmmqr_options *o) { if (o) *o = g_opt; }
void stmmqr_set_options(const stmmqr_options *o)
{
    if (!o) return;
    g_opt = *o;
    if (g_opt.big_front_cols < 1) g_opt.big_front_cols = 1;
}
void stmmqr_set_common_layout(const stm_common_layout *l) { if (l) g_layout = *l; }
void stmmqr_get_common_layout(stm_common_layout *l) { if (l) *l = g_layout; }

int stmmqr_device_alloc(size_t bytes, void **ptr)
{
    if (!ptr) return fail(STMMQR_ERR_INVALID, "null argument");
    *ptr = nullptr;
    if (hipMalloc(ptr, bytes ? bytes : 1) != hipSuccess) return fail(STMMQR_ERR_OUT_OF_MEMORY, "hipMalloc failed");
    return 0;
}
int stmmqr_device_copy(void *dst, const void *src, size_t bytes, void *hip_stream)
{
    if (hip_stream) HIPCHK(hipStreamSynchronize((hipStream_t)hip_stream));
    if (bytes) HIPCHK(hipMemcpy(dst, src, bytes, hipMemcpyDeviceToDevice));
    HIPCHK(hipDeviceSynchronize());
    return 0;
}
int stmmqr_device_free(void *ptr)
{
    if (ptr && hipFree(ptr) != hipSuccess) return fail(STMMQR_ERR_DEVICE, "hipFree failed");
    return 0;
}

void stmmqr_plan_cache_clear(void);
void stmmqr_shutdown(void)
{
    stmmqr_plan_cache_clear();
    int cnt = 0;
    if (hipGetDeviceCount(&cnt) == hipSuccess && cnt > 0) {
        (void)hipDeviceSynchronize();
        int dev = 0;
        (void)hipGetDevice(&dev);
        destroy_side_streams();
        (void)hipSetDevice(dev);
    }
}

int stmmqr_device_count(void)
{
    int cnt = 0;
    if (hipGetDeviceCount(&cnt) != hipSuccess) return 0;
    return cnt;
}
const char *stmmqr_device_name(int device)
{
    static thread_local char name[256];
    hipDeviceProp_t prop;
    if (hipGetDeviceProperties(&prop, device) != hipSuccess) return "";
    snprintf(name, sizeof name, "%s", prop.gcnArchName);
    return name;
}

int chunk_getSettings(size_t a, size_t b, size_t c, size_t d)
{
    g_chunk[0] = a; g_chunk[1] = b; g_chunk[2] = c; g_chunk[3] = d;
    return 0;
}

stmmqr_plan *stmmqr_plan_create(const stmmqr_symbolic_view *sym, int device, int *status)
{
    int st = 0;
    stmmqr_plan *P = nullptr;
    if (!sym) st = fail(STMMQR_ERR_INVALID, "null symbolic view");
    if (!st) st = ensure_device(device);
    if (!st) {
        P = new (std::nothrow) stmmqr_plan();
        if (!P) st = fail(STMMQR_ERR_OUT_OF_MEMORY, "host allocation failed");
    }
    if (!st) {
        (void)hipGetDevice(&P->device);
        int prio_lo = 0, prio_hi = 0;
        (void)hipDeviceGetStreamPriorityRange(&prio_lo, &prio_hi);
        if (hipStreamCreateWithPriority(&P->stream, hipStreamNonBlocking, prio_hi) != hipSuccess)
            st = fail(STMMQR_ERR_DEVICE, "hipStreamCreate failed");
        for (auto &e : P->ev)
            if (!st && hipEventCreate(&e) != hipSuccess) st = fail(STMMQR_ERR_DEVICE, "hipEventCreate failed");
    }
    if (!st) {
        const double t0 = now_ms();
        st = build_plan(*P, *sym);
        if (!st) P->stats.ms_host = now_ms() - t0;
    }
    if (st && P) { delete P; P = nullptr; }
    if (status) *status = st;
    return P;
}

void stmmqr_plan_release_rings(stmmqr_plan *plan);
void stmmqr_plan_destroy(stmmqr_plan *plan)
{
    if (plan) stmmqr_plan_release_rings(plan);
    delete plan;
}

int stmmqr_plan_set_pattern(stmmqr_plan *plan, const stm_long *Ap, const stm_long *Ai)
{
    if (!plan) return fail(STMMQR_ERR_INVALID, "null plan");
    HIPCHK(hipSetDevice(plan->device));
    return set_pattern(*plan, Ap, Ai);
}

int stmmqr_factorize_begin(stmmqr_plan *plan, const stm_long *Ap, const stm_long *Ai, const double *Ax,
                           int ax_on_device, double tol, stm_long ntol)
{
    if (!plan || !Ax) return fail(STMMQR_ERR_INVALID, "null plan / values");
    stmmqr_plan &P = *plan;
    HIPCHK(hipSetDevice(P.device));
    if (Ap && Ai) {
        int e = set_pattern(P, Ap, Ai);
        if (e) return e;
    }
    if (!P.pattern_set) return fail(STMMQR_ERR_INVALID, "pattern of A was never given");
    if (((P.early_end && !P.early_phased) || P.early_end_failed) && !P.whole_call) {
        P.early_end_failed = false;
        P.full_schedule = true;
        P.begun = false;
        std::vector<int> grp(P.group.begin(), P.group.end());
        int e = stmmqr_plan_set_groups(plan, grp.data());
        if (e) return e;
    }
    if (P.arena_overflow && P.recycle && !P.whole_call) {
        P.arena_overflow = false;
        P.begun = false;
        std::vector<int> grp(P.group.begin(), P.group.end());
        for (size_t f = 0; f < grp.size(); f++) if (f < P.shared.size() && P.shared[f]) grp[f] |= STMMQR_GROUP_SHARED;
        int e = stmmqr_plan_set_groups(plan, grp.data());
        if (e) return e;
    }
    const double host_ms_plan = P.stats.ms_host;
    P.stats = stmmqr_stats();
    P.stats.ms_host = host_ms_plan;
    P.factored = false;
    P.rowmap_ready = false;
    P.scr_valid = false;
    P.t4_valid = false;
    P.evused = 0;
    P.begun = true;
    P.first_group = true;
    if (!P.do_rank) tol = -1;
    P.last_tol = tol; P.last_ntol = ntol;
    hipStream_t st = P.stream;
    HIPCHK(hipEventRecord(P.ev[0], st));
    if (P.anz > 0) {
        HIPCHK(hipMemcpyAsync(P.d_Ax.p, Ax, (size_t)P.anz * sizeof(double),
                              ax_on_device ? hipMemcpyDeviceToDevice : hipMemcpyHostToDevice, st));
    }
    HIPCHK(hipEventRecord(P.ev[1], st));
    return reset_factorization(P);
}

int stmmqr_factorize_group(stmmqr_plan *plan, int group, int detail)
{
    if (!plan || !plan->begun) return fail(STMMQR_ERR_INVALID, "stmmqr_factorize_begin was not called");
    stmmqr_plan &P = *plan;
    HIPCHK(hipSetDevice(P.device));
    int e = 0;
    const bool graph_ok = g_opt.use_graph && !detail && group == 0 && P.first_group && !getenv("STMMQR_DUMPLV");
    if (graph_ok) {
        const DevCtx c = P.ctx();
        auto envl = [](const char *k, long dflt) { return getenv(k) ? atol(getenv(k)) : dflt; };
        long long optkey = 1469598103934665603LL;
        for (long long v : {(long long)g_opt.lookahead, (long long)g_opt.split_update, (long long)g_opt.fused_update, (long long)g_opt.pair_update,
                            (long long)P.serial_panels, (long long)c.tune, (long long)envl("STMMQR_LA_MIN", 2500), (long long)envl("STMMQR_LA_MIN_FUSED", 1500),
                            (long long)envl("STMMQR_LA_FUSED_ROWS", 5120), (long long)envl("STMMQR_LA_MAXPWG", 48), (long long)envl("STMMQR_LA_SYSFENCE", 0),
                            (long long)envl("STMMQR_SIDE_RESERVE", 32)})
            optkey = (optkey ^ v) * 1099511628211LL;
        if (!P.graph_exec || P.graph_tol != c.tol || P.graph_ntol != c.ntol || P.graph_dbg != c.dbg || P.graph_gen != P.sched_gen ||
            P.graph_opt != optkey) {
            if (P.graph_exec) { (void)hipGraphExecDestroy(P.graph_exec); P.graph_exec = nullptr; }
            P.graph_nlaunch = 0;
            if (g_opt.lookahead && !P.serial_panels && P.gsteps[0].size() > 1) {
                if (!P.side) P.side = side_stream_for(P.device);
                for (auto *v : {&P.ev_main, &P.ev_prep, &P.ev_side})
                    while (v->size() < P.gsteps[0].size() + 1) {
                        hipEvent_t ev = nullptr;
                        HIPCHK(hipEventCreateWithFlags(&ev, la_event_flags()));
                        v->push_back(ev);
                    }
            }
            const long nl0 = P.stats.nlaunch;
            hipGraph_t gph = nullptr;
            static std::mutex capture_mu;
            std::lock_guard<std::mutex> lock(capture_mu);
            HIPCHK(hipStreamBeginCapture(P.stream, hipStreamCaptureModeThreadLocal));
            e = run_schedule(P, false, 0);
            const hipError_t ce = hipStreamEndCapture(P.stream, &gph);
            if (e) { if (gph) (void)hipGraphDestroy(gph); return e; }
            HIPCHK(ce);
            HIPCHK(hipGraphInstantiate(&P.graph_exec, gph, nullptr, nullptr, 0));
            (void)hipGraphDestroy(gph);
            P.graph_tol = c.tol; P.graph_ntol = c.ntol; P.graph_dbg = c.dbg; P.graph_gen = P.sched_gen; P.graph_opt = optkey;
            P.graph_nlaunch = P.stats.nlaunch - nl0;
        } else {
            P.stats.nlaunch += P.graph_nlaunch;
            P.stats.nlevels += (long)P.glevels[0].size();
            P.stats.nsteps += (long)P.gsteps[0].size();
        }
        HIPCHK(hipGraphLaunch(P.graph_exec, P.stream));
    } else
        e = run_schedule(P, detail != 0, group);
    if (!e && !P.whole_call && !P.serial_panels) {
        int failed = 0;
        HIPCHK(hipMemcpyAsync(&failed, P.d_abort.p + 1, sizeof(int), hipMemcpyDeviceToHost, P.stream));
        HIPCHK(hipStreamSynchronize(P.stream));
        if (failed) {
            if (g_opt.verbose) fprintf(stderr, "[stmmqr_hip] a panel wait ran out in group %d: running it again with one-workgroup panels\n", group);
            P.stats.retries++;
            e = reset_group(P, group);
            P.serial_panels = true;
            if (!e) e = run_schedule(P, detail != 0, group);
            P.serial_panels = false;
        }
    }
    P.first_group = false;
    return e;
}

int stmmqr_factorize_finish(stmmqr_plan *plan, stmmqr_stats *stats)
{
    if (!plan || !plan->begun) return fail(STMMQR_ERR_INVALID, "stmmqr_factorize_begin was not called");
    stmmqr_plan &P = *plan;
    HIPCHK(hipSetDevice(P.device));
    hipStream_t st = P.stream;
    HIPCHK(hipEventRecord(P.ev[4], st));
    int e = run_pack(P);
    if (e) return e;
    HIPCHK(hipEventRecord(P.ev[5], st));
    int hard[2] = {0, 0};
    HIPCHK(hipMemcpyAsync(hard, P.d_abort.p + 2, 2 * sizeof(int), hipMemcpyDeviceToHost, st));
    HIPCHK(hipStreamSynchronize(st));
    if (hard[1]) return fail(STMMQR_ERR_DEVICE, "a contribution block received from another rank does not fit its front's symbolic bounds");
    if (hard[0]) {
        P.early_end_failed = true;
        P.evused = 0;
        return fail(STMMQR_ERR_RESCHEDULE, "a front was not finished by its last scheduled panel (the schedule is rebuilt with every panel)");
    }
    float ms = 0;
    HIPCHK(hipEventElapsedTime(&ms, P.ev[0], P.ev[1])); P.stats.ms_h2d = ms;
    HIPCHK(hipEventElapsedTime(&ms, P.ev[1], P.ev[5])); P.stats.ms_total = ms;
    HIPCHK(hipEventElapsedTime(&ms, P.ev[4], P.ev[5])); P.stats.ms_pack += ms;
    FILE *dump = (P.evused && getenv("STMMQR_DUMPSTEPS")) ? fopen(getenv("STMMQR_DUMPSTEPS"), "w") : nullptr;
    std::vector<float> st_panel, st_upd;
    if (dump && !P.gsteps.empty()) { st_panel.assign(P.gsteps[0].size(), 0.f); st_upd.assign(P.gsteps[0].size(), 0.f); }
    for (size_t q = 0; q < P.evused; q++) {
        float t = 0;
        HIPCHK(hipEventElapsedTime(&t, P.evpairs[q].a, P.evpairs[q].b));
        if (dump && (size_t)P.evpairs[q].step < st_panel.size()) {
            if (P.evpairs[q].cat == 2) st_panel[(size_t)P.evpairs[q].step] += t;
            if (P.evpairs[q].cat == 3) st_upd[(size_t)P.evpairs[q].step] += t;
        }
        switch (P.evpairs[q].cat) {
            case 0: P.stats.ms_assemble += t; break;
            case 1: P.stats.ms_front += t; P.stats.ms_small += t; break;
            case 2: P.stats.ms_front += t; P.stats.ms_panel += t; P.stats.npanel_launch++; break;
            case 3: P.stats.ms_front += t; P.stats.ms_update += t; P.stats.nupdate_launch++; break;
            default: P.stats.ms_pack += t; break;
        }
    }
    P.evused = 0;
    if (dump) {
        for (size_t t = 0; t < st_panel.size(); t++) {
            const Step &S = P.gsteps[0][t];
            int maxrows = 0, pwg = 0;
            long tiles = 0;
            for (int i = 0; i < S.n_act; i++) {
                const FrontSym &fsym = P.fs[P.lists[S.act_off + i]];
                const int p = P.lists[S.plist_off + i];
                maxrows = std::max(maxrows, stm_panel_rows_est(fsym, p));
                pwg += stm_use_ca(fsym, p, P.plan_algo, P.ca_min) ? stm_ca_slabs(fsym) : stm_tall_launches(fsym, p, P.tall_min);
                tiles += (long)stm_upd_ncb(fsym, p) * stm_upd_nsl(fsym);
            }
            fprintf(dump, "%zu n_act %d maxrows %d nsub %d pwg %d nca_use %d maxcb %d maxsl %d split %d tiles %ld panel_us %.1f upd_us %.1f\n", t,
                    S.n_act, maxrows, S.nsub, pwg, S.nca_use, S.maxcb, S.maxsl, S.split, tiles, 1e3 * st_panel[t], 1e3 * st_upd[t]);
        }
        fclose(dump);
    }

    P.h_fnum.resize((size_t)std::max(1L, P.nf));
    if (P.nf > 0)
        HIPCHK(hipMemcpy(P.h_fnum.data(), P.d_fnum.p, (size_t)P.nf * sizeof(FrontNum), hipMemcpyDeviceToHost));
    double flops = 0, bytes_asm = 0, bytes_pack = 0, fl_upd = 0, fl_upd_pair = 0;
    long rank = 0;
    for (long f = 0; f < P.nf; f++) {
        if (P.group[f] < 0) continue;
        const FrontNum &nm = P.h_fnum[f];
        const FrontSym &s = P.fs[f];
        flops += nm.flops;
        fl_upd += nm.flops_upd;
        if (getenv("STMMQR_DBG_EARLY") && s.nsched < s.npanels && (!nm.done || nm.g < std::min(nm.fm, s.fn)))
            fprintf(stderr, "[early] front %ld fn %d fp %d fm %d fm_est %d fm_ub %d g %d rank %d done %d nsched %d npanels %d\n", f, s.fn, s.fp, nm.fm, s.fm_est,
                    s.fm_ub, nm.g, nm.rank, nm.done, s.nsched, s.npanels);
        if ((size_t)f < P.pair_front.size() && P.pair_front[f]) fl_upd_pair += nm.flops_upd;
        rank += nm.rank;
        if (nm.perr) {
            P.panel_wait_failed = true;
            return fail(STMMQR_ERR_DEVICE, "a panel workgroup gave up waiting for its neighbours (device shared with another job?)");
        }
        const double cn = s.fn - s.fp, cm = nm.cm;
        const double csize = cm * (cm + 1) / 2 + cm * (cn - cm);
        bytes_asm += 8.0 * ((double)nm.fm * s.fn) + 8.0 * csize;
        bytes_pack += 16.0 * (csize + (double)nm.rsize);
    }
    bytes_asm += 8.0 * (double)P.anz + P.bytes_assemble_idx;
    if (getenv("STMMQR_DBG") && (atoi(getenv("STMMQR_DBG")) & 32) && getenv("STMMQR_TIMELINE")) {
        std::vector<unsigned long long> hb(2048);
        HIPCHK(hipMemcpy(hb.data(), P.d_dbg.p, hb.size() * sizeof(unsigned long long), hipMemcpyDeviceToHost));
        unsigned long long t0 = ~0ull;
        for (int b = 0; b < 16; b++) if (hb[16 + 64 * b]) t0 = std::min(t0, hb[16 + 64 * b]);
        for (int b = 0; b < 16; b++) {
            const unsigned long long *q = &hb[16 + 64 * b];
            if (!q[0]) continue;
            fprintf(stderr, "[panel timeline] group %2d:", b);
            auto us = [&](int i) { return q[i] ? 0.01 * (double)(q[i] - t0) : -1.0; };
            fprintf(stderr, " start %.2f loaded %.2f |", us(0), us(1));
            for (int h = 0; h < 6 && q[2 + 3 * h]; h++) fprintf(stderr, " wait %.2f vload %.2f applied %.2f |", us(2 + 3 * h), us(3 + 3 * h), us(4 + 3 * h));
            fprintf(stderr, " cols");
            for (int j = 0; j < 8; j++) if (q[20 + j]) fprintf(stderr, " %.2f", us(20 + j));
            fprintf(stderr, " | published %.2f final %.2f\n", us(30), us(31));
        }
    }
    if (getenv("STMMQR_DBG") && (atoi(getenv("STMMQR_DBG")) & 32768)) {
        unsigned long long hb[64];
        HIPCHK(hipMemcpy(hb, P.d_dbg.p, sizeof hb, hipMemcpyDeviceToHost));
        const double n = hb[56] ? 100.0 * (double)hb[56] : 1.0;
        fprintf(stderr, "[block-0 launch, slab 0, us] descriptors+loads issued %.2f  phase 1 %.2f  partials+ticket %.2f  wait %.2f  sums %.2f  T %.2f  W2 %.2f  phase 2 %.2f  (%llu)\n",
                hb[48] / n, hb[49] / n, hb[50] / n, hb[51] / n, hb[52] / n, hb[53] / n, hb[54] / n, hb[55] / n, hb[56]);
        HIPCHK(hipMemset(P.d_dbg.p, 0, sizeof hb));
    }
    if (getenv("STMMQR_DBG") && (atoi(getenv("STMMQR_DBG")) & 48)) {
        unsigned long long hb[64];
        HIPCHK(hipMemcpy(hb, P.d_dbg.p, sizeof hb, hipMemcpyDeviceToHost));
        fprintf(stderr, "[pipeline panels by actual rows] <=128 %llu  <=256 %llu  <=512 %llu  <=1024 %llu  <=2048 %llu  <=4096 %llu  more %llu;  of the <=512: %llu with a row estimate > 512\n",
                hb[32], hb[33], hb[34], hb[35], hb[36], hb[37], hb[38], hb[39]);
        fprintf(stderr, "[k_upd_w workgroups] launched %llu  with work %llu\n", hb[40], hb[41]);
        fprintf(stderr, "[panel cycles, summed over workgroups] stage-in+apply %llu  columns %llu  write-back %llu  - %llu  gram %llu\n",
                hb[0], hb[1], hb[2], hb[3], hb[4]);
        fprintf(stderr, "[last group of the panel pipeline, cycles] load %llu  waits %llu  apply-loads %llu  applies %llu  factor %llu  gram %llu\n", hb[6],
                hb[7], hb[12], hb[8] + hb[11], hb[9], hb[10]);
        fprintf(stderr, "[panel workgroups] %llu  cycles %llu  100 MHz ticks %llu  => %.3f GHz, %.2f us per workgroup\n", hb[46], hb[44], hb[45],
                hb[45] ? 0.1 * (double)hb[44] / (double)hb[45] : 0.0, hb[46] ? 0.01 * (double)hb[45] / (double)hb[46] : 0.0);
        fprintf(stderr, "[Gram-based panels] panels %llu  refresh rounds %llu  slab workgroups %llu\n", hb[13], hb[14], hb[15]);
        HIPCHK(hipMemset(P.d_dbg.p, 0, sizeof hb));
    }
    P.rank = rank;
    P.stats.flops = flops;
    P.stats.flops_update = fl_upd;
    P.stats.flops_update_pair = fl_upd_pair;
    P.stats.bytes_assemble = bytes_asm;
    P.stats.bytes_pack = bytes_pack;
    P.stats.device_bytes = P.device_bytes();
    if (getenv("STMMQR_MEMDUMP")) {
        auto gb = [](const auto &b) { return (double)b.n * sizeof(*b.p) * 1e-9; };
        fprintf(stderr, "[stmmqr_hip] device memory (GB): fronts %.3f  contribution blocks %.3f  R+H %.3f  update workspaces %.3f + %.3f  "
                        "kept T %.3f  pair -Y %.3f  Sx/Ax/smap %.3f  per-column arrays %.3f  total %.3f  (recycle %d, kept fronts %d, maxstack %.3f)\n",
                gb(P.d_F), gb(P.d_C), gb(P.d_RH), gb(P.d_Wp), gb(P.d_Wp2), gb(P.d_Tall), gb(P.d_Ypend), gb(P.d_Sx) + gb(P.d_Ax) + gb(P.d_smap),
                gb(P.d_Stair) + gb(P.d_Tau) + gb(P.d_Hii) + gb(P.d_Cmap) + gb(P.d_Cursor) + gb(P.d_Rhoff) + gb(P.d_Rjrel) + gb(P.d_Sjrel),
                P.stats.device_bytes * 1e-9, (int)P.recycle, (int)std::count(P.kept.begin(), P.kept.end(), (char)1), 8e-9 * (double)P.maxstack);
    }
    P.factored = true;
    P.begun = false;
    if (stats) *stats = P.stats;
    return 0;
}

int stmmqr_factorize_device(stmmqr_plan *plan, const stm_long *Ap, const stm_long *Ai, const double *Ax,
                            int ax_on_device, double tol, stm_long ntol, stmmqr_stats *stats)
{
    if (!plan) return fail(STMMQR_ERR_INVALID, "null plan");
    const bool detail = g_opt.verbose >= 2 || (stats && stats->nlaunch == -1);
    int arena_retries = 0, reschedules = 0;
    for (int attempt = 0; attempt < 2; attempt++) {
        plan->serial_panels = (attempt == 1);
        plan->panel_wait_failed = false;
        plan->whole_call = true;
        int e = stmmqr_factorize_begin(plan, Ap, Ai, Ax, ax_on_device, tol, ntol);
        if (!e) plan->stats.retries = (attempt == 1 ? 1 : 0) + arena_retries;
        if (!e) plan->stats.reschedules = reschedules;
        for (int g = 0; g < (int)plan->glevels.size() && !e; g++) e = stmmqr_factorize_group(plan, g, detail);
        if (!e) e = stmmqr_factorize_finish(plan, stats);
        plan->whole_call = false;
        if (e && plan->arena_overflow && plan->recycle) {
            plan->arena_overflow = false;
            if (g_opt.verbose) fprintf(stderr, "[stmmqr_hip] R+H arena overflow: factorizing again %s\n", plan->overflowed ? "without slab recycling" : "with the arena at its hard bound");
            plan->begun = false;
            std::vector<int> grp(plan->group.begin(), plan->group.end());
            for (size_t f = 0; f < grp.size(); f++) if ((size_t)f < plan->shared.size() && plan->shared[f]) grp[f] |= STMMQR_GROUP_SHARED;
            int e2 = stmmqr_plan_set_groups(plan, grp.data());
            if (e2) return e2;
            arena_retries++;
            attempt = -1;
            Ap = nullptr; Ai = nullptr;
            continue;
        }
        if (e && plan->early_end_failed) {
            plan->early_end_failed = false;
            plan->full_schedule = true;
            if (g_opt.verbose) fprintf(stderr, "[stmmqr_hip] a front outlived its schedule (rank-deficient fronts): factorizing again on the full schedule\n");
            plan->begun = false;
            std::vector<int> grp(plan->group.begin(), plan->group.end());
            int e2 = stmmqr_plan_set_groups(plan, grp.data());
            if (e2) return e2;
            reschedules++;
            attempt = -1;
            Ap = nullptr; Ai = nullptr;
            continue;
        }
        const bool retry = e && plan->panel_wait_failed && attempt == 0;
        plan->serial_panels = false;
        if (!retry) return e;
        if (g_opt.verbose) fprintf(stderr, "[stmmqr_hip] a panel wait ran out: factorizing again with one-workgroup panels\n");
        if (stats && detail) stats->nlaunch = -1;
        Ap = nullptr; Ai = nullptr;
    }
    return fail(STMMQR_ERR_DEVICE, "panel kernels failed twice");
}

int stmmqr_plan_set_early_end(stmmqr_plan *plan, int mode)
{
    if (!plan) return fail(STMMQR_ERR_INVALID, "null plan");
    stmmqr_plan &P = *plan;
    if (P.begun && !P.early_end_failed) return fail(STMMQR_ERR_INVALID, "stmmqr_plan_set_early_end between factorize_begin and factorize_finish");
    P.begun = false;
    P.early_end_failed = false;
    P.early_phased = (mode != 0);
    P.full_schedule = (mode == 0);
    std::vector<int> grp(P.group.begin(), P.group.end());
    for (size_t f = 0; f < grp.size(); f++) if (f < P.shared.size() && P.shared[f]) grp[f] |= STMMQR_GROUP_SHARED;
    return stmmqr_plan_set_groups(plan, grp.data());
}

int stmmqr_plan_set_groups(stmmqr_plan *plan, const int *group)
{
    if (!plan || !group) return fail(STMMQR_ERR_INVALID, "null plan / groups");
    stmmqr_plan &P = *plan;
    HIPCHK(hipSetDevice(P.device));
    auto gid = [&](long f) { return group[f] < 0 ? -1 : (group[f] & ~STMMQR_GROUP_SHARED); };
    for (long f = 0; f < P.nf; f++)
        for (long q = P.Childp[f]; q < P.Childp[f + 1]; q++)
            if (gid(f) >= 0 && gid(P.Child[q]) > gid(f))
                return fail(STMMQR_ERR_INVALID, "a child is scheduled in a later phase than its parent");
    {
        std::vector<int> cnt, nsh;
        for (long f = 0; f < P.nf; f++) {
            const int g = gid(f);
            if (g < 0) continue;
            if (g >= (1 << 24)) return fail(STMMQR_ERR_INVALID, "group id out of range");
            if ((size_t)g >= cnt.size()) { cnt.resize((size_t)g + 1, 0); nsh.resize((size_t)g + 1, 0); }
            cnt[(size_t)g]++;
            if (group[f] & STMMQR_GROUP_SHARED) {
                nsh[(size_t)g]++;
                if (!(P.fs[f].fn >= g_opt.big_front_cols && P.fs[f].fm_ub >= 64))
                    return fail(STMMQR_ERR_INVALID, "a shared front must be one of the large fronts (options.big_front_cols)");
            }
        }
        for (size_t g = 0; g < cnt.size(); g++)
            if (nsh[g] > 0 && cnt[g] != 1) return fail(STMMQR_ERR_INVALID, "a shared front must be alone in its group");
    }
    if (P.begun) return fail(STMMQR_ERR_INVALID, "stmmqr_plan_set_groups between factorize_begin and factorize_finish");
    HIPCHK(hipStreamSynchronize(P.stream));
    P.shared.assign((size_t)std::max(1L, P.nf), 0);
    for (long f = 0; f < P.nf; f++) {
        P.group[f] = gid(f);
        P.shared[(size_t)f] = (group[f] >= 0 && (group[f] & STMMQR_GROUP_SHARED)) ? 1 : 0;
    }
    if (P.graph_exec) { (void)hipGraphExecDestroy(P.graph_exec); P.graph_exec = nullptr; }
    P.graph_nlaunch = 0;
    assign_arenas(P);
    P.factored = false;
    std::vector<int> tslot;
    build_schedule(P, tslot);
    LCHK(P.d_fs.upload(P.fs, P.stream));
    LCHK(upload_recycle(P));
    auto grow = [](auto &buf, size_t n) -> int { return buf.n >= n && buf.p ? 0 : buf.alloc(n); };
    LCHK(grow(P.d_T, (size_t)STM_PD_RING * P.tslots * STM_NB * STM_NB));
    LCHK(grow(P.d_Gp, (size_t)P.tslots * (P.gp_slabs + 1) * STM_NB * STM_NB));
    LCHK(grow(P.d_Wp, (size_t)P.wp_doubles));
    LCHK(grow(P.d_Ypend, (size_t)std::max(1LL, P.yp_doubles)));
    LCHK(P.d_ypoff.upload(P.ypoff, P.stream));
    LCHK(grow(P.d_Wp2, (size_t)std::max(1LL, P.wp2_doubles)));
    P.wcnt_n = std::max(P.wcnt_n, (size_t)(P.wp_doubles / (STM_NB * 32) + 1));
    LCHK(grow(P.d_wcnt, P.wcnt_n));
    LCHK(grow(P.d_wcnt2, P.wcnt_n));
    LCHK(grow(P.d_wflag, P.wcnt_n));
    if (!P.d_abort.p) LCHK(P.d_abort.alloc(4));
    LCHK(grow(P.d_wflag2, P.wcnt_n));
    HIPCHK(hipMemset(P.d_wcnt.p, 0, P.wcnt_n * sizeof(int)));
    HIPCHK(hipMemset(P.d_wcnt2.p, 0, P.wcnt_n * sizeof(int)));
    LCHK(P.d_tslot.upload(tslot, P.stream));
    LCHK(P.d_lists.upload(P.lists, P.stream));
    LCHK(P.d_wlists.upload(P.wlists, P.stream));
    HIPCHK(hipStreamSynchronize(P.stream));
    return 0;
}

int stm_check_c_slot(const stmmqr_plan &P, stm_long f, long long csize, const char *what)
{
    if (f < 0 || f >= P.nf) return fail(STMMQR_ERR_INVALID, std::string(what) + ": no such front");
    if (P.recycle)
        return fail(STMMQR_ERR_INVALID, std::string(what) + ": this plan holds the whole tree and recycles its contribution blocks "
                                        "(nothing to exchange; regroup with stmmqr_plan_set_groups first)");
    if ((size_t)f >= P.has_c.size() || !P.has_c[(size_t)f])
        return fail(STMMQR_ERR_INVALID, std::string(what) + ": the front has no contribution-block slot on this plan (it is neither "
                                        "factorized here nor a child of a front that is)");
    if (!P.d_C.p || P.d_C.n != (size_t)P.carena)
        return fail(STMMQR_ERR_INVALID, std::string(what) + ": the arenas of the current grouping are not allocated yet "
                                        "(stmmqr_factorize_begin comes first)");
    if (csize < 0 || csize > P.c_slot[(size_t)f])
        return fail(STMMQR_ERR_INVALID, std::string(what) + ": the block exceeds the front's slot");
    return 0;
}

int stmmqr_plan_download(stmmqr_plan *plan, double *Stack, stm_long *Rblock_off, char *Rdead, stm_long *HStair,
                         double *HTau, stm_long *Hii, stm_long *HPinv, stm_long *Hm, stm_long *Hr,
                         stm_long *scalars, stmmqr_stats *stats)
{
    if (!plan || !plan->factored) return fail(STMMQR_ERR_INVALID, "no factorization held by the plan");
    stmmqr_plan &P = *plan;
    HIPCHK(hipSetDevice(P.device));
    hipStream_t st = P.stream;
    const long nf = P.nf, m = P.m, n = P.n;
    HIPCHK(hipEventRecord(P.ev[6], st));
    if (Stack && P.rh_total > 0 && P.recycle) {
        const long long win = std::min<long long>(P.rh_total, 32LL << 20);
        if (P.d_bounce.n < (size_t)(2 * win)) LCHK(P.d_bounce.alloc((size_t)(2 * win)));
        const DevCtx c = P.ctx();
        const int parts = (int)std::min<long long>(64, std::max<long long>(1, win / (64 * 1024)));
        hipEvent_t evw[2] = {nullptr, nullptr};
        for (auto &e : evw) HIPCHK(hipEventCreateWithFlags(&e, hipEventDisableTiming));
        int rc = 0;
        for (long long w0 = 0, i = 0; w0 < P.rh_total && !rc; w0 += win, i++) {
            const long long w1 = std::min(P.rh_total, w0 + win);
            double *out = P.d_bounce.p + (i & 1) * win;
            if (i >= 2 && hipEventSynchronize(evw[i & 1]) != hipSuccess) rc = 1;
            if (!rc && stm_launch_rh_window(c, P.d_lists.p + P.own_off, P.n_own, parts, P.d_fin.p, P.d_kept.p, P.d_RH.p, w0, w1, out, st)) rc = 1;
            if (!rc && hipMemcpyAsync(Stack + w0, out, (size_t)(w1 - w0) * sizeof(double), hipMemcpyDeviceToHost, st) != hipSuccess) rc = 1;
            if (!rc && hipEventRecord(evw[i & 1], st) != hipSuccess) rc = 1;
        }
        if (hipStreamSynchronize(st) != hipSuccess) rc = 1;
        for (auto &e : evw) (void)hipEventDestroy(e);
        if (rc) return fail(STMMQR_ERR_DEVICE, "download of the packed factors failed");
    } else if (Stack && P.rh_total > 0)
        HIPCHK(hipMemcpyAsync(Stack, P.d_RH.p, (size_t)P.rh_total * sizeof(double), hipMemcpyDeviceToHost, st));
    std::vector<int> stair32((size_t)std::max(1L, P.rjsize)), hii32((size_t)std::max(1L, P.hisize));
    std::vector<long long> rboff((size_t)std::max(1L, nf));
    if (P.rjsize > 0)
        HIPCHK(hipMemcpyAsync(stair32.data(), P.d_Stair.p, (size_t)P.rjsize * sizeof(int), hipMemcpyDeviceToHost, st));
    if (P.hisize > 0)
        HIPCHK(hipMemcpyAsync(hii32.data(), P.d_Hii.p, (size_t)P.hisize * sizeof(int), hipMemcpyDeviceToHost, st));
    if (HTau && P.rjsize > 0)
        HIPCHK(hipMemcpyAsync(HTau, P.d_Tau.p, (size_t)P.rjsize * sizeof(double), hipMemcpyDeviceToHost, st));
    if (Rdead && n > 0) HIPCHK(hipMemcpyAsync(Rdead, P.d_Rdead.p, (size_t)n, hipMemcpyDeviceToHost, st));
    if (nf > 0)
        HIPCHK(hipMemcpyAsync(rboff.data(), P.recycle ? P.d_fin.p : P.d_Rboff.p, (size_t)nf * sizeof(long long), hipMemcpyDeviceToHost, st));
    HIPCHK(hipEventRecord(P.ev[7], st));
    HIPCHK(hipStreamSynchronize(st));
    float ms = 0;
    HIPCHK(hipEventElapsedTime(&ms, P.ev[6], P.ev[7]));
    P.stats.ms_d2h = ms;

    const double t0 = now_ms();
    if (HStair) for (long i = 0; i < P.rjsize; i++) HStair[i] = stair32[i];
    if (Rblock_off) for (long f = 0; f < nf; f++) Rblock_off[f] = (stm_long)rboff[f];
    long maxfrank = 1, maxfm = 0, rank = 0;
    bool all_here = true;
    for (long f = 0; f < nf; f++) {
        const FrontNum &nm = P.h_fnum[f];
        const bool own = P.group[f] >= 0;
        all_here = all_here && own;
        if (Hm) Hm[f] = own ? nm.fm : 0;
        if (Hr) Hr[f] = own ? nm.rank : 0;
        if (!own) continue;
        maxfrank = std::max(maxfrank, (long)nm.rank);
        maxfm = std::max(maxfm, (long)nm.fm);
        rank += nm.rank;
    }
    if (!all_here) {
        if (Hii)
            for (long f = 0; f < nf; f++)
                if (P.group[f] >= 0)
                    for (long i = 0; i < P.h_fnum[f].fm; i++) Hii[P.Hip[f] + i] = hii32[P.Hip[f] + i];
        Hii = nullptr; HPinv = nullptr;
    }
    if (Hii || HPinv) {
        std::vector<long> W((size_t)std::max(1L, m), 0);
        long row1 = 0, row2 = m;
        for (long i = P.Sleft[n]; i < m; i++) W[i] = --row2;
        for (long f = 0; f < nf; f++) {
            const int *Hi = hii32.data() + P.Hip[f];
            const FrontNum &nm = P.h_fnum[f];
            const long rm = nm.rank, fm = nm.fm;
            for (long i = 0; i < rm; i++) W[Hi[i]] = row1++;
            const long cn = P.fs[f].fn - P.fs[f].fp;
            const long cm = std::min(fm - rm, cn);
            for (long i = fm - 1; i >= rm + cm; i--) W[Hi[i]] = --row2;
        }
        if (HPinv) for (long i = 0; i < m; i++) HPinv[i] = W[P.PLinv[i]];
        if (Hii) {
            for (long f = 0; f < nf; f++) {
                const int *Hi = hii32.data() + P.Hip[f];
                stm_long *Ho = Hii + P.Hip[f];
                const long fm = P.h_fnum[f].fm;
                for (long i = 0; i < fm; i++) Ho[i] = W[Hi[i]];
            }
        }
    }
    if (scalars) {
        scalars[0] = rank;
        long rank1 = rank;
        if (P.last_ntol < n) {
            std::vector<char> rd((size_t)std::max(1L, n));
            if (Rdead) memcpy(rd.data(), Rdead, (size_t)n);
            else HIPCHK(hipMemcpy(rd.data(), P.d_Rdead.p, (size_t)n, hipMemcpyDeviceToHost));
            rank1 = 0;
            for (long j = 0; j < P.last_ntol; j++) rank1 += !rd[j];
        }
        scalars[1] = rank1; scalars[2] = maxfrank; scalars[3] = maxfm;
    }
    P.stats.ms_host += now_ms() - t0;
    if (stats) *stats = P.stats;
    return 0;
}

int stmmqr_factorize_arrays(const stmmqr_symbolic_view *sym, const stm_long *Ap, const stm_long *Ai,
                            const double *Ax, double tol, stm_long ntol, double *Stack, stm_long stack_cap,
                            stm_long *Rblock_off, char *Rdead, stm_long *HStair, double *HTau, stm_long *Hii,
                            stm_long *HPinv, stm_long *Hm, stm_long *Hr, stm_long *scalars, stmmqr_stats *stats)
{
    int st = 0;
    stmmqr_plan *P = stmmqr_plan_create(sym, -1, &st);
    if (!P) return st;
    st = stmmqr_factorize_device(P, Ap, Ai, Ax, 0, tol, ntol, stats);
    if (!st && Stack && P->rh_total > stack_cap) st = fail(STMMQR_ERR_INVALID, "Stack buffer too small");
    if (!st) st = stmmqr_plan_download(P, Stack, Rblock_off, Rdead, HStair, HTau, Hii, HPinv, Hm, Hr, scalars, stats);
    stmmqr_plan_destroy(P);
    return st;
}

}
```

stm-multifrontal-qr-factorization-empowered-by-gcn_amd/csrc/stmmqr_kernels.h:

```cpp
#pragma once
#include <hip/hip_runtime_api.h>
#include "stmmqr_device.h"

struct DevCtx {
    const FrontSym *fs;
    FrontNum *fnum;
    double *Farena;
    double *Carena;
    double *Tws;
    const int *tslot;
    double *Tall;
    double *Gp;
    int gp_slabs;
    const double *sig;
    int panel_algo;
    int ca_min_rows;
    const double *Sx;
    const int *Sp;
    const int *Sjrel;
    const int *Sj0;
    const int *Sleft;
    const int *Child;
    const int *Rjrel;
    int *Stair;
    double *Tau;
    int *Hii;
    char *Rdead;
    int *Cmap;
    int *Cursor;
    long long *Rhoff;
    long long *Rboff;
    double tol;
    int ntol;
    unsigned long long *dbgbuf;
    int *abort;
    int tall_min;
    int cbskip;
    double *Ypend;
    const long long *ypoff;
    long long *rh_top;
    long long rh_cap;
    int sweep;
    int tune;
    int dbg;
};

int stm_configure_kernels(void);
int stm_update_lds_bytes(void);
int stm_launch_sigma(const double *Ax, int anz, unsigned long long *amaxbits, double *sig, hipStream_t st);
int stm_launch_gather_sx(const double *Ax, const int *smap, double *Sx, int anz, hipStream_t st);
int stm_launch_setup(const DevCtx &c, const int *flist, int nfr, hipStream_t st);
int stm_launch_assemble(const DevCtx &c, const int *flist, const int *nparts, int nfr, int maxparts, hipStream_t st);
int stm_launch_front_wg(const DevCtx &c, const int *flist, int nfr, int lds_doubles, hipStream_t st);
int stm_launch_panel(const DevCtx &c, const int *flist, const int *plist, int nfr, int nsub, int defer_ok, int lds_doubles, hipStream_t st);
int stm_configure_capanel(void);
int stm_launch_panel_ca(const DevCtx &c, const int *flist, const int *plist, int nfr, int nw, int defer_ok, hipStream_t st);
int stm_launch_panel_ca_pc(const DevCtx &c, const int *flist, const int *plist, int nfr, int nw, int defer_ok, const int *uflist,
                           const int *uplist, int unfr, int ucb0, int uncb, int umaxsl, const double *Wp, const long long *uwpoff, hipStream_t st);
int stm_launch_update(const DevCtx &c, const int *flist, const int *plist, int nfr, int cb0, int ncb, hipStream_t st);
int stm_launch_update_fused(const DevCtx &c, const int *flist, const int *plist, int nfr, int cb0, int ncb, int maxsl, double *Wp,
                            const long long *wpoff, int *wcnt, int *wflag, int epoch, int with_gram, hipStream_t st);
int stm_launch_panel_pc(const DevCtx &c, const int *flist, const int *plist, int nfr, int nsub, int defer_ok, int lds_doubles,
                        const int *uflist, const int *uplist, int unfr, int ucb0, int uncb, int umaxsl, const double *Wp,
                        const long long *uwpoff, hipStream_t st);
int stm_launch_update_fw(const DevCtx &c, const int *flist, const int *plist, int nfr, int ncb, int maxsl, double *Wp,
                         const long long *wpoff, int *wcnt, int *wflag, int epoch, double *Wp2, int *wcnt2, hipStream_t st);
int stm_launch_update_w(const DevCtx &c, const int *flist, const int *plist, int nfr, int cb0, int ncb, int maxsl, double *Wp,
                        const long long *wpoff, int *wcnt, hipStream_t st);
int stm_launch_update_c(const DevCtx &c, const int *flist, const int *plist, int nfr, int cb0, int ncb, int maxsl, const double *Wp,
                        const long long *wpoff, hipStream_t st);
int stm_launch_update_pair(const DevCtx &c, const int *flist, const int *plist, int nfr, int ncbp, int maxsl, double *Wp,
                           const long long *wpoff, int *wcnt, hipStream_t st);
int stm_launch_update_quad(const DevCtx &c, const int *flist, const int *plist, int nfr, int ncbp, int maxsl, double *Wp,
                           const long long *wpoff, int *wcnt, hipStream_t st);
int stm_launch_update_split(const DevCtx &c, const int *flist, const int *plist, int nfr, int cb0, int ncb, int maxsl, double *Wp,
                            const long long *wpoff, int *wcnt, int with_gram, hipStream_t st);
int stm_launch_larft(const DevCtx &c, int f, hipStream_t st);
int stm_launch_update_notrans(const DevCtx &c, int f, int ncb, hipStream_t st);
int stm_launch_cpack(const DevCtx &c, const int *flist, const int *nparts, int nfr, int maxparts, hipStream_t st);
int stm_launch_rh_count(const DevCtx &c, const int *flist, int nfr, hipStream_t st);
int stm_launch_rh_scan(const DevCtx &c, const int *post, int nf, long long *rh_total, long long *outoff, hipStream_t st);
int stm_launch_zero_slabs(const DevCtx &c, const int *flist, int nfr, int maxparts, hipStream_t st);
int stm_launch_rh_unpack(const DevCtx &c, const FrontSym *cs, const int *flist, int nfr, int maxparts, const char *kept, const double *RH,
                         double *scratch, hipStream_t st);
int stm_launch_rh_window(const DevCtx &c, const int *flist, int nfr, int maxparts, const long long *fin, const char *kept, const double *RH,
                         long long w0, long long w1, double *out, hipStream_t st);
int stm_launch_rh_copy(const DevCtx &c, const int *flist, const int *nparts, int nfr, int maxparts, double *RH,
                       hipStream_t st);
struct RhsBatch { long long w, x, xf, wq, wq4, u; };

int stm_launch_qapply(const DevCtx &c, const int *flist, int nfr, int method, double *W, int lds_bytes, int *err, hipStream_t st);
int stm_launch_qapply_t(const DevCtx &c, const int *flist, int nfr, int method, double *W, int lds_bytes, hipStream_t st, int nb,
                        const RhsBatch &B);
int stm_qt4_doubles(void);
struct Qt4ItemHost { int f, g; long long off, dqo; };
int stm_launch_qt4_build(const DevCtx &c, const int *fl, const long long *dqo, int nfronts, const void *items, int nitems, int *Dq4, double *T4all,
                         hipStream_t st);
int stm_launch_qapply_big4(const DevCtx &c, const QbDesc *qd, const long long *t4off, int nq, int max_npanels, int max_nslab, int max_fm,
                           int method, double *W, double *Xf, int *Dq, double *Wq4, const double *T4all, hipStream_t st, int nb,
                           const RhsBatch &B);
int stm_launch_qapply_big(const DevCtx &c, const QbDesc *qd, int nq, int max_npanels, int max_nslab, int max_fm, int method, double *W,
                          double *Xf, int *Dq, double *Wq, hipStream_t st, int nb, const RhsBatch &B);
int stm_launch_rsolve_big(const DevCtx &c, const QbDesc *qd, int nq, int max_steps, int max_nslab, const int *Rj, const double *W,
                          double *X, double *Acc, int *Lc, int *Rm, int *err, hipStream_t st, int nb, const RhsBatch &B);
int stm_launch_rsolve(const DevCtx &c, const int *flist, int nfr, const int *Rj, const double *W, double *X, int lds_bytes,
                      int *err, hipStream_t st, int nb, const RhsBatch &B);
int stm_launch_rtsolve(const DevCtx &c, const int *flist, int nfr, const double *Bp, double *U, double *Xr, const int *rowbase,
                       int lds_bytes, hipStream_t st, int nb, const RhsBatch &B);
int stm_launch_panel_msg(void *const homes[6], const long long offs[6], const long long bytes[6], void *buf, int out, hipStream_t st);
struct StmFrontMsg { long long off, slot; int f, pad; };
struct StmFrontMsgs { StmFrontMsg m[16]; };
int stm_launch_front_msg(const DevCtx &c, const StmFrontMsgs &g, int nmsg, long long max_slot, double *buf, int out, hipStream_t st);
int stm_launch_front_cols(const DevCtx &c, int f, int part, int nparts, int nown, long long max_run, double *buf, int out, hipStream_t st);
int stm_launch_perm(const double *in, const int *perm, double *out, int n, int scatter, hipStream_t st, int nb = 1, long long sin = 0,
                    long long sout = 0);
```

stm-multifrontal-qr-factorization-empowered-by-gcn_amd/csrc/stmmqr_panel.hip:

```cpp
#include "stmmqr_kdev.h"
#include "stmmqr_riders.h"


template <int NTH>
__device__ __forceinline__ void dev_apply_subpanel(const double *Vl, long long pst, int gs, int r1, int sw, const int *diag,
                                   const double *tau, double *Fc , long long ld,
                                   int ncols)
{
    constexpr int NWV = NTH / 64;
    constexpr int MAXQ = 64;
    const int lane = threadIdx.x & 63, wid = threadIdx.x >> 6;
    const int rows = r1 - gs;
    if (rows <= 0) return;
    const int nq = (rows + 63) >> 6;
    for (int jc = wid; jc < ncols; jc += NWV) {
        double *cg = Fc + jc * ld + gs;
        if (nq <= MAXQ && NTH >= 512) {
            double creg[MAXQ];
#pragma unroll
            for (int q = 0; q < MAXQ; q++) {
                const int r = lane + 64 * q;
                creg[q] = (q < nq && r < rows) ? cg[r] : 0.0;
            }
            for (int i = 0; i < sw; i++) {
// ... 835 lines not shown
        pd->t_deferred = defer_t;
        pd->pk1 = k1; pd->pnb = nbp; pd->pc0 = k2;
        num->flops_upd += 4.0 * (double)(n - k2) * (prev_done ? ls_before : ls_before + lensum);
    }
    if (defer_t) {
        publish_progress(&num->prog, STM_PROG * p + NPART * b + NPART);
        return;
    }
    if (tid < STM_NB) {
        ps.diag[tid] = (tid < nbp) ? ld_agent(&pd->pdiag[tid]) : STM_BIGROW;
        ps.tau[tid] = (tid < nbp) ? ld_agent(&Tau[k1 + tid]) : 0.0;
    }
    __syncthreads();
    dev_gram_T<NTH>(F + (long long)k1 * ld, ld, g1, tlast, nbp, ps.diag, ps.tau, ps.G, ps.T, Tout, lds
#ifdef STMMQR_STAMPS
                    , ((dbg & 32) && dbgbuf && p == 1) ? dbgbuf + 16 + 64 * b + 40 : nullptr
#endif
                    );
    if (Tkeep)
        for (int e = tid; e < STM_NB * STM_NB; e += NTH) {
            const int ai = e % STM_NB, bi = e / STM_NB;
            Tkeep[e] = (ai < nbp && bi < nbp && ai <= bi) ? ps.T[ai][bi] : 0.0;
        }
    TSTAMP(10);
    TL(31);
    publish_progress(&num->prog, STM_PROG * p + NPART * b + NPART);
#undef TSTAMP
#undef TL
#undef TLW
#undef TCY
}

#define WP_SW 4
struct WaveShared {
    int ready[STM_NB];
    int d[STM_NB], t[STM_NB];
    double tau[STM_NB];
    int g, rank, done, tlast, nlive, jdone;
    long long iflops, ilen;
};

template <int RPT, int SW = WP_SW>
__device__ __forceinline__ void dev_wave_panel(PanelShared &ps, WaveShared &wsh, const FrontSym &s, FrontNum *num, PanelDesc *pd,
                                               double *F, int *St, double *Tau, char *Rdead, int p, int g1, int tmax, double tol,
                                               int ntol_global, double *Tout, double *lds, double *Tkeep, int defer_ok,
                                               const double *sigp)
{
    constexpr int NTH = 64 * (STM_NB / SW), RS = 64 * RPT;
    static_assert(SW == 4 || SW == 8, "a wave takes 4 or 8 columns");
    const int tid = threadIdx.x, lane = tid & 63, w = tid >> 6;
    const int m = num->fm, n = s.fn, npiv = s.fp;
    const long long ld = s.ld;
    const int k1 = p * STM_NB, k2 = min(n, k1 + STM_NB), nbp = k2 - k1;
    const int c0 = SW * w, sw = max(0, min(SW, nbp - c0));
    const int rb = g1;
    const double flops_before = num->flops;
    if (tid < STM_NB) {
        wsh.ready[tid] = 0; wsh.d[tid] = STM_BIGROW; wsh.t[tid] = 0; wsh.tau[tid] = 0.0;
        ps.stair[tid] = (tid < nbp) ? St[k1 + tid] : 0;
        ps.st_out[tid] = 0; ps.dead[tid] = 0;
    }
    if (tid == 0) {
        wsh.g = g1; wsh.rank = num->rank; wsh.done = 0; wsh.tlast = g1; wsh.nlive = 0; wsh.jdone = STM_NB;
        wsh.iflops = 0; wsh.ilen = 0;
    }
    double a[RPT][SW];
#pragma unroll
    for (int x = 0; x < SW; x++) {
        const double *src = F + (long long)(k1 + c0 + min(x, max(sw, 1) - 1)) * ld;
#pragma unroll
        for (int r = 0; r < RPT; r++) {
            const int i = rb + lane + 64 * r;
            const double val = src[min(i, tmax - 1)];
            a[r][x] = (x < sw && i < tmax) ? val : 0.0;
        }
    }
    __syncthreads();
    auto wait_col = [&](int j) {
        while (__hip_atomic_load(&wsh.ready[j], __ATOMIC_ACQUIRE, __HIP_MEMORY_SCOPE_WORKGROUP) == 0) __builtin_amdgcn_s_sleep(1);
    };
    const int ntol = min(ntol_global - s.col1, npiv);
    const double sg = sigp ? sigp[0] : 1.0, isg = sigp ? sigp[1] : 1.0;
    if (sw > 0) {
        for (int j = 0; j < c0; j++) {
            wait_col(j);
            const double tau = wsh.tau[j];
            const int d = wsh.d[j];
            if (tau == 0.0 || d >= STM_BIGROW) continue;
            const double *vs = lds + j * RS;
            double v[RPT], pv[8];
#pragma unroll
            for (int x = 0; x < 8; x++) pv[x] = 0.0;
#pragma unroll
            for (int r = 0; r < RPT; r++) {
                const int i = rb + lane + 64 * r;
                const double val = vs[lane + 64 * r];
                v[r] = (i < d) ? 0.0 : ((i == d) ? 1.0 : val);
#pragma unroll
                for (int x = 0; x < SW; x++) pv[x] += v[r] * a[r][x];
            }
            const double rw = wave_reduce8(pv);
            double wv[SW];
            wv[0] = tau * lane_bcast<red8_lane(0)>(rw); wv[1] = tau * lane_bcast<red8_lane(1)>(rw);
            wv[2] = tau * lane_bcast<red8_lane(2)>(rw); wv[3] = tau * lane_bcast<red8_lane(3)>(rw);
            if constexpr (SW == 8) {
                wv[4] = tau * lane_bcast<red8_lane(4)>(rw); wv[5] = tau * lane_bcast<red8_lane(5)>(rw);
                wv[6] = tau * lane_bcast<red8_lane(6)>(rw); wv[7] = tau * lane_bcast<red8_lane(7)>(rw);
            }
#pragma unroll
            for (int r = 0; r < RPT; r++) {
#pragma unroll
                for (int x = 0; x < SW; x++) a[r][x] -= wv[x] * v[r];
            }
        }
        if (c0 > 0) wait_col(c0 - 1);
        int g = wsh.g, rank = wsh.rank, done = wsh.done, tlast = wsh.tlast, nlive = wsh.nlive, jdone = wsh.jdone;
        long long iflops = wsh.iflops, ilen = wsh.ilen;
#pragma unroll
        for (int x = 0; x < SW; x++) {
            if (x >= sw) continue;
            const int jp = c0 + x, k = k1 + jp;
            if (!done && g >= m) {
                for (int kk = k + lane; kk < n; kk += 64) {
                    if (kk < npiv) { Rdead[kk] = (char)1; St[kk] = 0; }
                    else St[kk] = m;
                    Tau[kk] = 0.0;
                }
                for (int jj = jp + lane; jj < STM_NB; jj += 64) pd->pdiag[jj] = STM_BIGROW;
                done = 1;
                jdone = jp;
            }
            if (!done) {
                const int t = max(g + 1, ps.stair[jp]);
                double part[8];
#pragma unroll
                for (int e = 0; e < 8; e++) part[e] = 0.0;
#pragma unroll
                for (int r = 0; r < RPT; r++) {
                    const int i = rb + lane + 64 * r;
                    const double xv = (i > g && i < t) ? a[r][x] * sg : 0.0;
#pragma unroll
                    for (int y = x; y < SW; y++) part[y - x] += xv * a[r][y];
                }
                const double rw = wave_reduce8(part);
                const double sum0 = lane_bcast<red8_lane(0)>(rw), sum1 = lane_bcast<red8_lane(1)>(rw);
                const double sum2 = lane_bcast<red8_lane(2)>(rw), sum3 = lane_bcast<red8_lane(3)>(rw);
                double sum[SW] = {sum0, sum1, sum2, sum3};
                if constexpr (SW == 8) {
                    sum[4] = lane_bcast<red8_lane(4)>(rw); sum[5] = lane_bcast<red8_lane(5)>(rw);
                    sum[6] = lane_bcast<red8_lane(6)>(rw); sum[7] = lane_bcast<red8_lane(7)>(rw);
                }
                const int ol = g - rb;
                double top[SW];
#pragma unroll
                for (int y = x; y < SW; y++)
                    top[y - x] = __hiloint2double(__builtin_amdgcn_readlane(__double2hiint(a[0][y]), ol),
                                                  __builtin_amdgcn_readlane(__double2loint(a[0][y]), ol));
                const double alpha = top[0], ss = sum[0];
                double bb, tau0, scal0, scals0;
                stm_larfg_guarded(alpha, ss, sg, isg, bb, tau0, scal0, scals0);
                const bool ident = (ss == 0.0);
                const double beta = ident ? alpha : bb;
                const bool dead = (k < ntol) && (fabs(beta) <= tol);
                const bool upd = !ident && !dead;
                const double tau = upd ? tau0 : 0.0;
                const double scal = upd ? scal0 : 0.0, scals = upd ? scals0 : 0.0;
                double wv[SW];
#pragma unroll
                for (int y = 1; y < SW - x; y++) wv[y] = tau * (top[y] + scals * sum[y]);
#pragma unroll
                for (int r = 0; r < RPT; r++) {
                    const int i = rb + lane + 64 * r;
                    const bool act = (i > g && i < t);
                    const double v = act ? a[r][x] * scal : 0.0;
                    a[r][x] = act ? v : ((dead && i >= g) ? 0.0 : a[r][x]);
#pragma unroll
                    for (int y = x + 1; y < SW; y++) a[r][y] -= wv[y - x] * v;
                }
                if (lane == ol) {
#pragma unroll
                    for (int y = x + 1; y < SW; y++) a[0][y] -= wv[y - x];
                    a[0][x] = dead ? 0.0 : beta;
                }
                if (lane == 0) {
                    ps.st_out[jp] = dead ? 0 : t; ps.tau[jp] = tau; ps.diag[jp] = dead ? STM_BIGROW : g; ps.dead[jp] = dead ? 1 : 0;
                    wsh.tau[jp] = tau; wsh.d[jp] = dead ? STM_BIGROW : g; wsh.t[jp] = t;
                }
                if (!dead) {
                    iflops += (long long)(t - g) * (3 + 4 * (long long)(n - k - 1));
                    ilen += (t - g);
                    nlive += (tau != 0.0);
                    tlast = t;
                    g++;
                }
                if (k == npiv - 1) rank = g;
            }
            {
                double *dst = F + (long long)k * ld;
                double *vs = lds + jp * RS;
#pragma unroll
                for (int r = 0; r < RPT; r++) {
                    const int i = rb + lane + 64 * r;
                    if (i < tmax) dst[i] = a[r][x];
                    vs[lane + 64 * r] = a[r][x];
                }
            }
            if (x == sw - 1 || done) {
                if (lane == 0) {
                    wsh.g = g; wsh.rank = rank; wsh.done = done; wsh.tlast = tlast; wsh.nlive = nlive; wsh.jdone = jdone;
                    wsh.iflops = iflops; wsh.ilen = ilen;
                }
            }
            if (lane == 0) {
                __hip_atomic_store(&wsh.ready[jp], 1, __ATOMIC_RELEASE, __HIP_MEMORY_SCOPE_WORKGROUP);
            }
        }
    }
    __syncthreads();
    const int g = wsh.g, tlast = wsh.tlast, jdone = wsh.jdone, done = wsh.done;
    const double lensum = (double)wsh.ilen;
    if (tid < min(nbp, jdone)) {
        const int kk = k1 + tid;
        St[kk] = ps.st_out[tid]; Tau[kk] = ps.tau[tid]; pd->pdiag[tid] = ps.diag[tid];
        if (ps.dead[tid]) Rdead[kk] = (char)1;
    }
    const int defer_t = (defer_ok && k2 < n && tlast > g1) ? 1 : 0;
    if (tid == 0) {
        num->g = g; num->rank = wsh.rank; num->done = done;
        num->flops = flops_before + (double)wsh.iflops;
        pd->sg[0] = g1; pd->st[0] = tlast; pd->pt = tlast; pd->nlive = wsh.nlive; pd->lensum = lensum;
        pd->done_group = done ? 0 : -1;
        pd->t_deferred = defer_t;
        pd->pk1 = k1; pd->pnb = nbp; pd->pc0 = k2;
        num->flops_upd += 4.0 * (double)(n - k2) * lensum;
    }
    if (defer_t) return;
    __syncthreads();
    if (tid < STM_NB) {
        ps.diag[tid] = (tid < nbp) ? pd->pdiag[tid] : STM_BIGROW;
        ps.tau[tid] = (tid < nbp) ? Tau[k1 + tid] : 0.0;
    }
    __syncthreads();
    dev_gram_T<NTH>(F + (long long)k1 * ld, ld, g1, tlast, nbp, ps.diag, ps.tau, ps.G, ps.T, Tout, lds);
    if (Tkeep)
        for (int e = tid; e < STM_NB * STM_NB; e += NTH) {
            const int ai = e % STM_NB, bi = e / STM_NB;
            Tkeep[e] = (ai < nbp && bi < nbp && ai <= bi) ? ps.T[ai][bi] : 0.0;
        }
}

__global__ __launch_bounds__(NT) void k_front_wg(DevCtx c, const int *__restrict__ flist, int lds_doubles)
{
    extern __shared__ double dyn_lds[];
    __shared__ double s_Tw[STM_NB * STM_NB];
    __shared__ PanelShared ps;
    __shared__ WaveShared wsh;
    const int f = flist[blockIdx.x];
    const FrontSym s = c.fs[f];
    FrontNum *num = &c.fnum[f];
    double *F = c.Farena + s.foff;
    auto Tkeep = [&](int p) { return c.Tall ? c.Tall + (long long)(s.tpan + p) * STM_NB * STM_NB : (double *)nullptr; };
    for (int p = 0; p < s.npanels; p++) {
        {
            const int k2w = min(s.fn, (p + 1) * STM_NB), g1w = num->g;
            const int tmaxw = min(num->fm, max((c.Stair + s.rp)[k2w - 1], g1w + (k2w - p * STM_NB)));
            const int rowsw = tmaxw - g1w;
            if (!num->done && rowsw <= 128 && !(c.dbg & (64 | 16384)) && max(STM_NB * (rowsw <= 64 ? 64 : 128), 3072) <= lds_doubles) {
                PanelDesc *pdw = &num->pd[STM_PDI(p)];
                __syncthreads();
                if (threadIdx.x == 0) { pdw->mode = 2; pdw->pg1 = g1w; pdw->tmax = tmaxw; }
#define WAVE_ARGS ps, wsh, s, num, pdw, F, c.Stair + s.rp, c.Tau + s.rp, c.Rdead + s.col1, p, g1w, tmaxw, c.tol, c.ntol, s_Tw, dyn_lds, Tkeep(p), 0, c.sig
                if (rowsw <= 64) dev_wave_panel<1, 8>(WAVE_ARGS);
                else dev_wave_panel<2, 8>(WAVE_ARGS);
#undef WAVE_ARGS
                __syncthreads();
                const int k2 = min(s.fn, (p + 1) * STM_NB);
                const int ncb = (s.fn - k2 + BN - 1) / BN;
                for (int cb = 0; cb < ncb; cb++)
                    dev_update_block(F, s.ld, pdw->pg1, pdw->pt - pdw->pg1, pdw->pk1, pdw->pnb, pdw->pdiag, s_Tw, k2 + cb * BN,
                                     min(BN, s.fn - (k2 + cb * BN)), dyn_lds);
                __syncthreads();
                continue;
            }
        }
        if ((c.dbg & 64) || panel_rows(s, num, c.Stair + s.rp, p) > lds_doubles - 65)
            dev_panel<NT, true>(ps, s, num, F, c.Stair + s.rp, c.Tau + s.rp, c.Rdead + s.col1, p, c.tol, c.ntol, s_Tw,
                                dyn_lds, lds_doubles, c.dbg, nullptr, Tkeep(p), c.sig);
        else
            dev_panel<NT, false>(ps, s, num, F, c.Stair + s.rp, c.Tau + s.rp, c.Rdead + s.col1, p, c.tol, c.ntol, s_Tw,
                                 dyn_lds, lds_doubles, c.dbg, nullptr, Tkeep(p), c.sig);
        const int k2 = min(s.fn, (p + 1) * STM_NB);
        const int ncb = (s.fn - k2 + BN - 1) / BN;
        const PanelDesc *pd = &num->pd[STM_PDI(p)];
        for (int cb = 0; cb < ncb; cb++)
            dev_update_block(F, s.ld, pd->pg1, pd->pt - pd->pg1, pd->pk1, pd->pnb, pd->pdiag, s_Tw, k2 + cb * BN,
                             min(BN, s.fn - (k2 + cb * BN)), dyn_lds);
        __syncthreads();
    }
    dev_cpack(c, s, num, 0, 1);
}

#define NTP 512

__device__ __forceinline__ void dev_k_panel(const DevCtx &c, const int *__restrict__ flist, const int *__restrict__ plist, int fi, int b,
                                            int nsub, int defer_ok, int lds_doubles, PanelShared &ps, WaveShared &wsh, double *dyn_lds)
{
    const int f = flist[fi];
    const int p = plist[fi];
    __builtin_amdgcn_s_setprio(3);
    const FrontSym s = c.fs[f];
    if (p >= s.npanels || stm_use_ca(s, p, c.panel_algo, c.ca_min_rows)) return;
    FrontNum *num = &c.fnum[f];
    double *F = c.Farena + s.foff;
    double *T = c.Tws + (long long)STM_TSLOT(c.tslot[f], p) * STM_NB * STM_NB;
    int *St = c.Stair + s.rp;
    double *Tkeep = c.Tall ? c.Tall + (long long)(s.tpan + p) * STM_NB * STM_NB : nullptr;
    PanelDesc *pd = &num->pd[STM_PDI(p)];
    if ((c.dbg & 2048) && b == ((c.dbg >> 20) & 7)) {
        for (int it = 0; it < 4000; it++) __builtin_amdgcn_s_sleep(100);
    }
    if ((c.dbg & 4096) && b > 0) {
        if (threadIdx.x == 0) STM_SET_PERR(c, num);
        return;
    }
    bool tall = stm_tall_panel(s, p, c.tall_min) && !(c.dbg & 256);
    if (!tall && b > 0) return;
    if (tall) {
        const int k1 = p * STM_NB, k2 = min(s.fn, k1 + STM_NB), nbp = k2 - k1;
        int mode, g1, tmax, w;
        if (b == 0) {
            const int was_done = num->done;
            g1 = num->g;
            tmax = min(num->fm, max(St[k2 - 1], g1 + nbp));
            w = (tmax - g1 > STM_TALL_XWIDE) ? 2 : (tmax - g1 > STM_TALL_WIDE) ? 4 : STM_SW;
            mode = (was_done || tmax - g1 > STM_TALL_MAX || (nbp + w - 1) / w > min(nsub, stm_tall_launches(s, p, c.tall_min))) ? 0 : 1;
            if (!was_done && tmax - g1 <= STM_WP_ROWS && !(c.dbg & 16384) &&
                STM_NB * ((tmax - g1 <= 128) ? 128 : (tmax - g1 <= 256) ? 256 : 512) <= lds_doubles)
                mode = 2;
            if ((c.dbg & 16) && c.dbgbuf && threadIdx.x == 0 && !was_done) {
                const int rws = tmax - g1;
                atomicAdd(&c.dbgbuf[32 + (rws <= 128 ? 0 : rws <= 256 ? 1 : rws <= 512 ? 2 : rws <= 1024 ? 3 : rws <= 2048 ? 4 : rws <= 4096 ? 5 : 6)], 1ull);
                if (rws <= 512 && stm_panel_rows_est(s, p) > STM_WP_ROWS) atomicAdd(&c.dbgbuf[39], 1ull);
            }
            __syncthreads();
            if (threadIdx.x == 0) {
                st_agent(&pd->mode, mode); st_agent(&pd->pg1, g1); st_agent(&pd->pt, g1); st_agent(&pd->tmax, tmax);
                st_agent(&pd->nlive, 0); st_agent(&pd->sw, w); st_agent(&pd->done_group, -1);
                if (was_done) { pd->pnb = 0; pd->t_deferred = 0; }
            }
            publish_progress(&num->hdr, p + 1);
            if (was_done) return;
        } else {
            if (!wait_progress(&num->hdr, p + 1)) { if (threadIdx.x == 0) STM_SET_PERR(c, num); return; }
            mode = ld_agent(&pd->mode); g1 = ld_agent(&pd->pg1); tmax = ld_agent(&pd->tmax); w = ld_agent(&pd->sw);
            if (mode != 1 || b * w >= nbp) return;
        }
        if (mode == 2) {
            const int rows = tmax - g1;
#define WAVE_ARGS ps, wsh, s, num, pd, F, St, c.Tau + s.rp, c.Rdead + s.col1, p, g1, tmax, c.tol, c.ntol, T, dyn_lds, Tkeep, defer_ok, c.sig
            if (rows <= 128) dev_wave_panel<2>(WAVE_ARGS);
            else if (rows <= 256) dev_wave_panel<4>(WAVE_ARGS);
            else dev_wave_panel<8>(WAVE_ARGS);
#undef WAVE_ARGS
            return;
        }
        if (mode == 1) {
            const int rows = tmax - g1;
#define TALL_ARGS ps, s, num, pd, F, St, c.Tau + s.rp, c.Rdead + s.col1, p, b, g1, tmax, c.tol, c.ntol, T, dyn_lds, c.dbg, c.dbgbuf, Tkeep, defer_ok, c.sig, c.abort
            if (w == 2) dev_tall_group<NTP, 16, 2>(TALL_ARGS);
            else if (w == 4) dev_tall_group<NTP, 8, 4>(TALL_ARGS);
            else if (rows <= NTP) dev_tall_group<NTP, 1, 8>(TALL_ARGS);
            else if (rows <= 2 * NTP) dev_tall_group<NTP, 2, 8>(TALL_ARGS);
            else dev_tall_group<NTP, 4, 8>(TALL_ARGS);
#undef TALL_ARGS
            return;
        }
    }
    const int lds_front = stm_front_lds(s);
    if ((c.dbg & 64) || lds_front > lds_doubles || panel_rows(s, num, St, p) > lds_front - 65)
        dev_panel<NTP, true>(ps, s, num, F, St, c.Tau + s.rp, c.Rdead + s.col1, p, c.tol, c.ntol, T, dyn_lds,
                             lds_front, c.dbg, c.dbgbuf, Tkeep, c.sig);
    else
        dev_panel<NTP, false>(ps, s, num, F, St, c.Tau + s.rp, c.Rdead + s.col1, p, c.tol, c.ntol, T, dyn_lds,
                              lds_front, c.dbg, c.dbgbuf, Tkeep, c.sig);
    if (threadIdx.x == 0) { pd->mode = 0; pd->t_deferred = 0; }
}

__global__ __launch_bounds__(NTP) void k_panel(DevCtx c, const int *__restrict__ flist, const int *__restrict__ plist, int nsub,
                                               int defer_ok, int lds_doubles)
{
    extern __shared__ double dyn_lds[];
    __shared__ PanelShared ps;
    __shared__ WaveShared wsh;
    const unsigned long long t0c = clock64(), t0w = wall_clock64();
    dev_k_panel(c, flist, plist, blockIdx.x, blockIdx.y, nsub, defer_ok, lds_doubles, ps, wsh, dyn_lds);
    if ((c.dbg & 16) && c.dbgbuf && threadIdx.x == 0) {
        atomicAdd(&c.dbgbuf[44], clock64() - t0c); atomicAdd(&c.dbgbuf[45], wall_clock64() - t0w); atomicAdd(&c.dbgbuf[46], 1ull);
    }
}

__global__ __launch_bounds__(NTP) void k_panel_pc(DevCtx c, const int *__restrict__ flist, const int *__restrict__ plist, int npan,
                                                  int nsub, int defer_ok, int lds_doubles, const int *__restrict__ uflist,
                                                  const int *__restrict__ uplist, int ucb0, const double *Wp,
                                                  const long long *__restrict__ uwpoff, int rspw)
{
    extern __shared__ double dyn_lds[];
    __shared__ PanelShared ps;
    __shared__ WaveShared wsh;
    if (blockIdx.z == 0) {
        if ((int)blockIdx.x >= npan || (int)blockIdx.y >= nsub) return;
        const unsigned long long t0c = clock64(), t0w = wall_clock64();
        dev_k_panel(c, flist, plist, blockIdx.x, blockIdx.y, nsub, defer_ok, lds_doubles, ps, wsh, dyn_lds);
        if ((c.dbg & 16) && c.dbgbuf && threadIdx.x == 0) {
            atomicAdd(&c.dbgbuf[44], clock64() - t0c); atomicAdd(&c.dbgbuf[45], wall_clock64() - t0w); atomicAdd(&c.dbgbuf[46], 1ull);
        }
        return;
    }
    dev_upd_c_h2(c, uflist, uplist, ucb0, Wp, uwpoff, (int)blockIdx.z - 1, blockIdx.x, blockIdx.y, rspw, dyn_lds, ps.stair);
}
int stm_launch_front_wg(const DevCtx &c, const int *flist, int nfr, int lds_doubles, hipStream_t st)
{
    if (nfr <= 0) return 0;
    size_t bytes = (size_t)lds_doubles * sizeof(double);
    if (bytes < (size_t)stm_update_lds_bytes()) bytes = stm_update_lds_bytes();
    hipLaunchKernelGGL(k_front_wg, dim3(nfr), dim3(NT), bytes, st, c, flist, (int)(bytes / sizeof(double)));
    return (int)hipGetLastError();
}
int stm_launch_panel(const DevCtx &c, const int *flist, const int *plist, int nfr, int nsub, int defer_ok, int lds_doubles, hipStream_t st)
{
    if (nfr <= 0) return 0;
    size_t bytes = (size_t)lds_doubles * sizeof(double);
    if (bytes < (size_t)stm_update_lds_bytes()) bytes = stm_update_lds_bytes();
    int K = nfr;
    if (nsub > 1 && (c.dbg & 512)) K = getenv("STMMQR_CHUNK") ? atoi(getenv("STMMQR_CHUNK")) : 1;
    if (K < 1) K = 1;
    for (int i = 0; i < nfr; i += K)
        hipLaunchKernelGGL(k_panel, dim3(nfr - i < K ? nfr - i : K, nsub), dim3(NTP), bytes, st, c, flist + i, plist + i, nsub, defer_ok,
                           (int)(bytes / sizeof(double)));
    return (int)hipGetLastError();
}
int stm_launch_panel_pc(const DevCtx &c, const int *flist, const int *plist, int nfr, int nsub, int defer_ok, int lds_doubles,
                        const int *uflist, const int *uplist, int unfr, int ucb0, int uncb, int umaxsl, const double *Wp,
                        const long long *uwpoff, hipStream_t st)
{
    if (unfr <= 0 || uncb <= 0 || umaxsl <= 0 || (c.dbg & 512)) {
        if (unfr > 0 && uncb > 0 && umaxsl > 0)
            (void)stm_launch_update_c(c, uflist, uplist, unfr, ucb0, uncb, umaxsl, Wp, uwpoff, st);
        return stm_launch_panel(c, flist, plist, nfr, nsub, defer_ok, lds_doubles, st);
    }
    if (nfr <= 0 && !(nfr < 0)) {
        return stm_launch_update_c(c, uflist, uplist, unfr, ucb0, uncb, umaxsl, Wp, uwpoff, st);
    }
    if (nfr < 0) nfr = 0;
    size_t bytes = (size_t)lds_doubles * sizeof(double);
    if (bytes < (size_t)stm_update_lds_bytes()) bytes = stm_update_lds_bytes();
    const int lds_arg = (int)(bytes / sizeof(double));
    if (bytes < (size_t)STM_PC_LDS_DOUBLES * sizeof(double)) bytes = (size_t)STM_PC_LDS_DOUBLES * sizeof(double);
    int rspw = 1;
    {
        static int force = -1;
        if (force < 0) force = getenv("STMMQR_RSPW") ? atoi(getenv("STMMQR_RSPW")) : 0;
        double best = 1e30;
        for (int k = 1; k <= 16; k *= 2) {
            const long wgs = (long)unfr * uncb * ((umaxsl + k - 1) / k);
            const double t = (double)((wgs + 239) / 240) * (5.0 + 1.0 * k);
            if (t < best) { best = t; rspw = k; }
        }
        if (force > 0) rspw = force;
    }
    const int uy = (umaxsl + rspw - 1) / rspw;
    hipLaunchKernelGGL(k_panel_pc, dim3(nfr > uncb ? nfr : uncb, nsub > uy ? nsub : uy, 1 + unfr), dim3(NTP), bytes, st, c, flist,
                       plist, nfr, nsub, defer_ok, lds_arg, uflist, uplist, ucb0, Wp, uwpoff, rspw);
    return (int)hipGetLastError();
}
int stm_configure_update(void);
int stm_configure_sweep(void);
int stm_configure_resident(void);
int stm_configure_kernels(void)
{
    CK(hipFuncSetAttribute((const void *)k_front_wg, hipFuncAttributeMaxDynamicSharedMemorySize, 122880));
    CK(hipFuncSetAttribute((const void *)k_panel, hipFuncAttributeMaxDynamicSharedMemorySize, 131072));
    CK(hipFuncSetAttribute((const void *)k_panel_pc, hipFuncAttributeMaxDynamicSharedMemorySize, 131072));
    { int e = stm_configure_update(); if (e) return e; }
    { int e = stm_configure_sweep(); if (e) return e; }
    return stm_configure_resident();
}
```

stm-multifrontal-qr-factorization-empowered-by-gcn_amd/csrc/stmmqr_plan.h:

```cpp
#pragma once
#include <hip/hip_runtime.h>

#include <algorithm>
#include <chrono>
#include <cmath>
#include <cstdio>
#include <cstdlib>
#include <cstring>
#include <string>
#include <mutex>
#include <thread>
#include <vector>
#ifdef __linux__
#include <sys/mman.h>
#endif
#include <dlfcn.h>

#include "../../include/stmmqr_hip.h"
#include "stmmqr_device.h"
#include "stmmqr_kernels.h"
#include "stmmqr_internal.h"


extern thread_local std::string g_err;
extern stmmqr_options g_opt;
extern size_t g_chunk[4];

extern stm_common_layout g_layout;

int fail(int code, const std::string &msg);

#define HIPCHK(expr)                                                                                      \
    do {                                                                                                  \
        hipError_t e_ = (expr);                                                                           \
        if (e_ != hipSuccess)                                                                             \
            return fail(e_ == hipErrorOutOfMemory ? STMMQR_ERR_OUT_OF_MEMORY : STMMQR_ERR_DEVICE,        \
                        std::string(#expr) + ": " + hipGetErrorString(e_));                              \
    } while (0)
#define LCHK(expr)                                                                                        \
    do {                                                                                                  \
        int e_ = (expr);                                                                                  \
        if (e_ != 0) return fail(STMMQR_ERR_DEVICE, std::string(#expr) + ": " + hipGetErrorString((hipError_t)e_)); \
    } while (0)

inline double now_ms()
{
    using namespace std::chrono;
    return duration<double, std::milli>(steady_clock::now().time_since_epoch()).count();
}

template <class T> struct DevBuf {
    T *p = nullptr;
    size_t n = 0;
    int alloc(size_t count)
    {
        release();
        n = count;
        if (count == 0) count = 1;
        hipError_t e = hipMalloc((void **)&p, count * sizeof(T));
        if (e != hipSuccess) { p = nullptr; n = 0; return (int)e; }
        return 0;
    }
    int upload(const std::vector<T> &h, hipStream_t st)
    {
        int e = alloc(h.size());
        if (e) return e;
        if (!h.empty()) return (int)hipMemcpyAsync(p, h.data(), h.size() * sizeof(T), hipMemcpyHostToDevice, st);
        return 0;
    }
    void release()
    {
        if (p) (void)hipFree(p);
        p = nullptr; n = 0;
    }
    ~DevBuf() { release(); }
};

struct Level {
    int all_off = 0, n_all = 0;
    int n_small = 0, n_big = 0;
};

struct Step {
    int start_off = 0, n_start = 0, n_small = 0;
    int asm_parts_off = 0, asm_maxparts = 1, lds_small = 0;
    int act_off = 0, plist_off = 0, n_act = 0;
    int wp_off = 0;
    int nsub = 1, nca = 1, nca_use = 0, npipe_use = 0, maxcb = 0, maxsl = 0, split = 0;
    int lds_big = 0;
    int lds_plan = 0;
    int n_norm = 0, n_pk[4] = {0, 0, 0, 0};
    int maxsl_pk[4] = {0, 0, 0, 0}, maxcbp_po = 0;
    int n_sweep() const { return n_pk[0] + n_pk[1] + n_pk[2] + n_pk[3]; }
    int cpk_off = 0, cpk_parts_off = 0, n_cpk = 0, cpk_maxparts = 1;
    int rhp_off = 0, rhp_parts_off = 0, n_rhp = 0, rhp_maxparts = 1;
};


struct stmmqr_plan {
    int device = 0;
    hipStream_t stream = nullptr;
    hipStream_t side = nullptr;
    std::vector<hipEvent_t> ev_main, ev_prep, ev_side;
    hipEvent_t ev[8] = {};
    struct EvPair { hipEvent_t a, b; int cat, step; };
    std::vector<EvPair> evpairs;
    size_t evused = 0;
    long m = 0, n = 0, anz = 0, nf = 0, maxfn = 0, rjsize = 0, hisize = 0;
    int do_rank = 1;
    int ca_min = STM_CA_MIN_ROWS;
    int plan_algo = 0;
    int tall_min = STM_TALL_MIN;
    int tune = 0;
    std::vector<long> Sp, Sj, Qfill, PLinv, Sleft, Child, Childp, Super, Rp, Rj, Post, Hip, Fm;
    bool has_qfill = false;
    std::vector<FrontSym> fs;
    std::vector<std::vector<Level>> glevels;
    std::vector<std::vector<Step>> gsteps;
    std::vector<long long> wlists;
    std::vector<char> pair_front;
    int sweep = 2;
    std::vector<int> group;
    std::vector<int> h_tslot;
    std::vector<char> shared;
    std::vector<char> has_c;
    std::vector<long long> c_slot;
    int own_off = 0, n_own = 0;
    bool recycle = false;
    long maxstack = 0;
    std::vector<char> kept;
    std::vector<int> f_t0, f_t1, c_t1;
    long long rh_cap = 0;
    long long rh_est_total = 0;
    int rh_grow = 0;
    long long scr_doubles = 0;
    std::vector<FrontSym> fs_scr;
    bool scr_all = false, scr_valid = false;
    bool overflowed = false;
    bool early_end = false;
    bool full_schedule = false;
    bool early_phased = false;
    bool early_end_failed = false;
    bool arena_overflow = false;
    std::vector<int> lists;
    int post_off = 0, rh_parts_off = 0, rh_maxparts = 1;
    long long farena = 0, carena = 0;
    int tslots = 1;
    int gp_slabs = 1;
    long long tpanels = 0;
    long long wp_doubles = 0;
    long long wp2_doubles = 0;
    bool pattern_set = false;
    double bytes_assemble_idx = 0;

    DevBuf<FrontSym> d_fs;
    DevBuf<FrontNum> d_fnum;
    DevBuf<double> d_F, d_C, d_T, d_Gp, d_Tall, d_Sx, d_Ax, d_Tau, d_RH, d_Wp, d_Wp2;
    DevBuf<int> d_tslot, d_Sp, d_Sjrel, d_Sj0, d_Sleft, d_Child, d_Rjrel, d_Stair, d_Hii, d_Cmap, d_Cursor,
        d_lists, d_smap;
    DevBuf<long long> d_Rhoff;
    DevBuf<long long> d_wlists;
    DevBuf<double> d_Ypend;
    DevBuf<long long> d_ypoff;
    std::vector<long long> ypoff;
    long long yp_doubles = 0;
    DevBuf<double> d_msg;
    DevBuf<int> d_wcnt, d_wcnt2;
    DevBuf<int> d_wflag, d_wflag2;
    DevBuf<int> d_abort;
    size_t wcnt_n = 1;
    DevBuf<long long> d_Rboff, d_total;
    DevBuf<long long> d_rhtop, d_fin;
    DevBuf<char> d_kept;
    DevBuf<double> d_scr, d_bounce;
    DevBuf<FrontSym> d_fs_scr;
    DevBuf<unsigned long long> d_dbg, d_amax;
    DevBuf<double> d_sig;
    DevBuf<char> d_Rdead;

    bool factored = false, begun = false, first_group = true;
    bool whole_call = false;
    bool panel_wait_failed = false;
    bool serial_panels = false;
    long long rh_total = 0;
    long rank = 0;
    std::vector<FrontNum> h_fnum;
    DevBuf<int> d_Rj, d_PLinv, d_Qfill, d_Wmap, d_err;
    DevBuf<double> d_W, d_Xs, d_Io, d_Xf, d_Wq, d_Xall, d_Yall, d_U, d_Xr;
    DevBuf<int> d_rowbase;
    std::vector<int> level_lds_rt;
    DevBuf<int> d_Dq;
    DevBuf<QbDesc> d_qb;
    std::vector<Qt4ItemHost> t4items;
    std::vector<int> t4fronts;
    std::vector<long long> t4dqo, qbt4off;
    long long t4_doubles = 0, dq4_ints = 0, wq4_doubles = 0;
    DevBuf<Qt4ItemHost> d_t4items;
    DevBuf<int> d_t4fronts, d_Dq4;
    DevBuf<long long> d_t4dqo, d_qbt4off;
    DevBuf<double> d_T4, d_Wq4;
    bool t4_valid = false, t4_ok = false, t4_tried = false;
    struct QbLevel { int off = 0, n = 0, max_np = 0, max_nslab = 0, max_fm = 0, max_rsteps = 0, t4i_off = 0, t4i_n = 0;
                     int live_np = 0, live_rsteps = 0; };
    std::vector<QbDesc> h_qb;
    std::vector<char> t4_level_valid;
    DevBuf<int> d_Rm;
    int rhs_cap = 1;
    long long xf_doubles = 1, wq_doubles = 1;
    std::vector<QbLevel> level_qbig;
    hipGraphExec_t graph_exec = nullptr;
    double graph_tol = 0; int graph_ntol = 0, graph_dbg = 0; long long graph_opt = 0; long graph_nlaunch = 0;
    long sched_gen = 0, graph_gen = -1;
    bool rowmap_ready = false;
    std::vector<int> level_lds_qa, level_lds_qa_all, level_lds_rs;
    double last_tol = 0;
    long last_ntol = 0;
    stmmqr_stats stats = {};

    double device_bytes() const
    {
        double b = 0;
        auto add = [&](const auto &buf) { b += (double)buf.n * sizeof(*buf.p); };
        add(d_fs); add(d_fnum); add(d_F); add(d_C); add(d_T); add(d_Gp); add(d_Tall); add(d_Sx); add(d_Ax); add(d_Tau); add(d_RH);
        add(d_Wp); add(d_Wp2); add(d_tslot); add(d_Sp); add(d_Sjrel); add(d_Sj0); add(d_Sleft); add(d_Child); add(d_Rjrel);
        add(d_Stair); add(d_Hii); add(d_Cmap); add(d_Cursor); add(d_lists); add(d_smap); add(d_Rhoff); add(d_wlists);
        add(d_wcnt); add(d_wcnt2); add(d_wflag); add(d_wflag2); add(d_Rboff); add(d_Rdead); add(d_Ypend); add(d_ypoff);
        add(d_rhtop); add(d_fin); add(d_kept); add(d_scr); add(d_bounce); add(d_fs_scr);
        return b;
    }
    DevCtx ctx() const
    {
        DevCtx c;
        c.fs = d_fs.p; c.fnum = d_fnum.p; c.Farena = d_F.p; c.Carena = d_C.p; c.Tws = d_T.p; c.tslot = d_tslot.p;
        c.Tall = d_Tall.p;
        c.Gp = d_Gp.p; c.gp_slabs = gp_slabs; c.sig = d_sig.p; c.panel_algo = serial_panels ? 1 : plan_algo; c.ca_min_rows = ca_min;
        c.Sx = d_Sx.p; c.Sp = d_Sp.p; c.Sjrel = d_Sjrel.p; c.Sj0 = d_Sj0.p; c.Sleft = d_Sleft.p;
        c.Child = d_Child.p; c.Rjrel = d_Rjrel.p; c.Stair = d_Stair.p; c.Tau = d_Tau.p; c.Hii = d_Hii.p;
        c.Rdead = d_Rdead.p; c.Cmap = d_Cmap.p; c.Cursor = d_Cursor.p; c.Rhoff = d_Rhoff.p; c.Rboff = d_Rboff.p;
        c.tol = last_tol; c.ntol = (int)last_ntol;
        c.dbg = getenv("STMMQR_DBG") ? atoi(getenv("STMMQR_DBG")) : 0;
        c.sweep = sweep;
        c.tune = tune;
        c.Ypend = d_Ypend.p; c.ypoff = d_ypoff.p;
        c.rh_top = recycle ? d_rhtop.p : nullptr; c.rh_cap = rh_cap;
        if (serial_panels) c.dbg = (c.dbg & ~(2048 | 4096)) | 256;
        c.tall_min = tall_min;
        c.cbskip = 0;
        c.dbgbuf = d_dbg.p;
        c.abort = d_abort.p;
        return c;
    }
    ~stmmqr_plan()
    {
        for (auto &e : ev)
            if (e) (void)hipEventDestroy(e);
        for (auto &q : evpairs) { if (q.a) (void)hipEventDestroy(q.a); if (q.b) (void)hipEventDestroy(q.b); }
        if (graph_exec) (void)hipGraphExecDestroy(graph_exec);
        for (auto *v : {&ev_main, &ev_prep, &ev_side})
            for (auto &e : *v)
                if (e) (void)hipEventDestroy(e);
        if (stream) (void)hipStreamDestroy(stream);
    }
};

struct StepReq { int step, what, cb_first, cb_stride, cb_count; };
int stm_run_schedule(stmmqr_plan &P, bool detail, int grp, const StepReq *req);
int stm_ensure_device(int device);
extern "C" int stm_check_c_slot(const stmmqr_plan &P, stm_long f, long long csize, const char *what);
```

Baseline: 5545 GFLOP/s.

## Add specialized pipeline-only panel kernels with guarded fallback to generic panels

Adds templated k_panel_pipe and k_panel_pipe_pc kernels that compile only the tall column-pipeline panel path. The host marks each step as pipe-eligible at plan time and launches the specialized kernel for those steps. If a panel at runtime needs the in-place mode, the kernel sets an abort word, and the host re-runs the group or whole factorization with the generic kernels. The aim is to cut code size and register pressure in panel kernels, at the cost of more complexity and a possible full re-factorization when the guard fires.

After: 5576 GFLOP/s, median of 6. About the same (+0.6%).

```diff
diff --git a/include/stmmqr_hip.h b/include/stmmqr_hip.h
--- a/include/stmmqr_hip.h
+++ b/include/stmmqr_hip.h
@@ -119,6 +119,7 @@
     stm_long retries;
     double device_bytes;
     stm_long reschedules;
+    stm_long panel_fallbacks;
 } stmmqr_stats;
 
 typedef struct stmmqr_plan stmmqr_plan;
diff --git a/stm-multifrontal-qr-factorization-empowered-by-gcn_amd/capi.py b/stm-multifrontal-qr-factorization-empowered-by-gcn_amd/capi.py
--- a/stm-multifrontal-qr-factorization-empowered-by-gcn_amd/capi.py
+++ b/stm-multifrontal-qr-factorization-empowered-by-gcn_amd/capi.py
@@ -57,7 +57,8 @@
                                           "ms_host", "bytes_assemble", "bytes_pack", "flops_update", "ms_update"]] + \
                [("nlaunch", C.c_long), ("nlevels", C.c_long), ("ms_panel", C.c_double), ("ms_small", C.c_double),
                 ("npanel_launch", C.c_long), ("nupdate_launch", C.c_long), ("nsteps", C.c_long),
-                ("flops_update_pair", C.c_double), ("retries", C.c_long), ("device_bytes", C.c_double), ("reschedules", C.c_long)]
+                ("flops_update_pair", C.c_double), ("retries", C.c_long), ("device_bytes", C.c_double), ("reschedules", C.c_long),
+                ("panel_fallbacks", C.c_long)]
 
     def as_dict(self):
         return {k: getattr(self, k) for k, _ in self._fields_}
diff --git a/stm-multifrontal-qr-factorization-empowered-by-gcn_amd/csrc/stmmqr_host.cpp b/stm-multifrontal-qr-factorization-empowered-by-gcn_amd/csrc/stmmqr_host.cpp
--- a/stm-multifrontal-qr-factorization-empowered-by-gcn_amd/csrc/stmmqr_host.cpp
+++ b/stm-multifrontal-qr-factorization-empowered-by-gcn_amd/csrc/stmmqr_host.cpp
@@ -479,6 +479,9 @@
                     S.lds_plan = std::max(S.lds_plan, stm_front_lds(s));
                 if (stm_tall_panel(s, p, P.tall_min) && !stm_use_ca(s, p, g_opt.panel_algo, P.ca_min))
                     S.lds_plan = std::max(S.lds_plan, STM_NB * STM_WP_ROWS);
+                if (!stm_use_ca(s, p, g_opt.panel_algo, P.ca_min) &&
+                    !(stm_tall_panel(s, p, P.tall_min) && stm_panel_rows_est(s, p) <= STM_TALL_MAX))
+                    S.pipe_ok = 0;
             }
             S.lds_big = (int)std::min((long)LDS_CAP_DOUBLES, (((maxfm_big + 63) & ~63L) | 1) * STM_NB + 64);
             S.split = (S.maxsl >= 3 || ncbsum >= 512) ? 1 : 0;
@@ -753,7 +756,7 @@
     LCHK(P.d_wcnt.alloc(P.wcnt_n));
     LCHK(P.d_wcnt2.alloc(P.wcnt_n));
     LCHK(P.d_wflag.alloc(P.wcnt_n));
-    if (!P.d_abort.p) LCHK(P.d_abort.alloc(4));
+    if (!P.d_abort.p) LCHK(P.d_abort.alloc(5));
     LCHK(P.d_wflag2.alloc(P.wcnt_n));
     HIPCHK(hipMemset(P.d_wcnt.p, 0, P.wcnt_n * sizeof(int)));
     HIPCHK(hipMemset(P.d_wcnt2.p, 0, P.wcnt_n * sizeof(int)));
@@ -821,7 +824,7 @@
     HIPCHK(hipMemsetAsync(P.d_wcnt2.p, 0, P.wcnt_n * sizeof(int), st));
     HIPCHK(hipMemsetAsync(P.d_wflag.p, 0, P.wcnt_n * sizeof(int), st));
     HIPCHK(hipMemsetAsync(P.d_wflag2.p, 0, P.wcnt_n * sizeof(int), st));
-    HIPCHK(hipMemsetAsync(P.d_abort.p, 0, 4 * sizeof(int), st));
+    HIPCHK(hipMemsetAsync(P.d_abort.p, 0, 5 * sizeof(int), st));
     LCHK(stm_launch_sigma(P.d_Ax.p, (int)P.anz, P.d_amax.p, P.d_sig.p, st));
     LCHK(stm_launch_gather_sx(P.d_Ax.p, P.d_smap.p, P.d_Sx.p, (int)P.anz, st));
     P.stats.nlaunch += 6;
@@ -844,6 +847,7 @@
     HIPCHK(hipMemsetAsync(P.d_wflag.p, 0, P.wcnt_n * sizeof(int), st));
     HIPCHK(hipMemsetAsync(P.d_wflag2.p, 0, P.wcnt_n * sizeof(int), st));
     HIPCHK(hipMemsetAsync(P.d_abort.p, 0, 3 * sizeof(int), st));
+    HIPCHK(hipMemsetAsync(P.d_abort.p + 4, 0, sizeof(int), st));
     if (P.recycle) HIPCHK(hipMemsetAsync(P.d_rhtop.p, 0, 2 * sizeof(long long), st));
     HIPCHK(hipStreamSynchronize(st));
     return 0;
@@ -908,13 +912,21 @@
         }
         return 0;
     };
+    const bool pipe_on = !req && !P.panel_generic && !P.serial_panels && !(c.dbg & (64 | 256 | 512)) &&
+                         !(getenv("STMMQR_PANEL_PIPE") && atoi(getenv("STMMQR_PANEL_PIPE")) == 0);
+    bool guard_test = (c.dbg & 65536) != 0;
+    auto pipe_of = [&](const Step &S) -> int {
+        if (!pipe_on || !S.pipe_ok) return 0;
+        if (guard_test) { guard_test = false; return 2; }
+        return 1;
+    };
     auto panels = [&](const Step &S) -> int {
         const int *act = L0 + S.act_off, *pl = L0 + S.plist_off;
         return timed(t_panel, [&]() -> int {
             if (S.nca_use && !P.serial_panels) { LCHK(stm_launch_panel_ca(c, act, pl, S.n_act, S.nca, 1, st)); nlaunch++; }
             if (S.npipe_use || P.serial_panels) {
                 const int lds = (P.serial_panels || (c.dbg & (64 | 256))) ? S.lds_big : S.lds_plan;
-                LCHK(stm_launch_panel(c, act, pl, S.n_act, S.nsub, 1, lds, st));
+                LCHK(stm_launch_panel(c, act, pl, S.n_act, S.nsub, 1, lds, st, pipe_of(S)));
                 nlaunch++;
             }
             return 0;
@@ -1084,8 +1096,9 @@
                         const double panel_us = prow <= 512 ? 25.0 : prow <= 4096 ? 48.0 : 72.0;
                         if ((tiles > pass_tiles || (double)tiles > pass_k * panel_us) && (e = flush_alone())) return e;
                     }
+                    const int pipe = pipe_of(S);
                     if (pend && (abl & 4)) {
-                        LCHK(stm_launch_panel(c, act, pl, S.n_act, S.nsub, 1, lds, st));
+                        LCHK(stm_launch_panel(c, act, pl, S.n_act, S.nsub, 1, lds, st, pipe));
                         if (abl & 8) {
                             const Step &Q = *pend;
                             pend = nullptr;
@@ -1097,9 +1110,9 @@
                         const Step &Q = *pend;
                         pend = nullptr;
                         LCHK(stm_launch_panel_pc(c, act, pl, S.n_act, S.nsub, 1, lds, L0 + Q.act_off, L0 + Q.plist_off, Q.n_norm, 1, Q.maxcb - 1,
-                                                 Q.maxsl, P.d_Wp2.p, P.d_wlists.p + Q.wp_off, st));
+                                                 Q.maxsl, P.d_Wp2.p, P.d_wlists.p + Q.wp_off, st, pipe));
                     } else
-                        LCHK(stm_launch_panel(c, act, pl, S.n_act, S.nsub, 1, lds, st));
+                        LCHK(stm_launch_panel(c, act, pl, S.n_act, S.nsub, 1, lds, st, pipe));
                     nlaunch++;
                 } else if ((e = flush_alone()))
                     return e;
@@ -1198,6 +1211,15 @@
     return 0;
 }
 
+int pipe_guard_failed(stmmqr_plan &P)
+{
+    P.pipe_guard_hit = true;
+    P.panel_generic = true;
+    P.evused = 0;
+    return fail(STMMQR_ERR_DEVICE, "a panel planned for the column pipeline needed the in-place panel (factorize again: the plan now "
+                                   "takes the generic panel kernels)");
+}
+
 int run_pack(stmmqr_plan &P)
 {
     hipStream_t st = P.stream;
@@ -1216,11 +1238,14 @@
         }
         LCHK(stm_launch_rh_scan(c, L0 + P.post_off, (int)P.nf, P.d_total.p, P.d_fin.p, st));
         long long total = 0, top[2] = {0, 0};
+        int guard = 0;
         HIPCHK(hipMemcpyAsync(&total, P.d_total.p, sizeof(long long), hipMemcpyDeviceToHost, st));
         HIPCHK(hipMemcpyAsync(top, P.d_rhtop.p, 2 * sizeof(long long), hipMemcpyDeviceToHost, st));
+        HIPCHK(hipMemcpyAsync(&guard, P.d_abort.p + 4, sizeof(int), hipMemcpyDeviceToHost, st));
         HIPCHK(hipStreamSynchronize(st));
         P.rh_total = total;
         P.stats.nlaunch += 2;
+        if (guard) return pipe_guard_failed(P);
         if (top[1] != 0) {
             if (!P.rh_grow) P.rh_grow = 1;
             else P.overflowed = true;
@@ -1232,8 +1257,11 @@
     LCHK(stm_launch_rh_count(c, L0 + P.own_off, P.n_own, st));
     LCHK(stm_launch_rh_scan(c, L0 + P.post_off, (int)P.nf, P.d_total.p, P.d_Rboff.p, st));
     long long total = 0;
+    int guard = 0;
     HIPCHK(hipMemcpyAsync(&total, P.d_total.p, sizeof(long long), hipMemcpyDeviceToHost, st));
+    HIPCHK(hipMemcpyAsync(&guard, P.d_abort.p + 4, sizeof(int), hipMemcpyDeviceToHost, st));
     HIPCHK(hipStreamSynchronize(st));
+    if (guard) return pipe_guard_failed(P);
     P.rh_total = total;
     if ((size_t)total > P.d_RH.n) LCHK(P.d_RH.alloc((size_t)(total + total / 64 + 1024)));
     LCHK(stm_launch_rh_copy(c, L0 + P.own_off, L0 + P.rh_parts_off, P.n_own, P.rh_maxparts, P.d_RH.p, st));
@@ -1421,7 +1449,7 @@
         for (long long v : {(long long)g_opt.lookahead, (long long)g_opt.split_update, (long long)g_opt.fused_update, (long long)g_opt.pair_update,
                             (long long)P.serial_panels, (long long)c.tune, (long long)envl("STMMQR_LA_MIN", 2500), (long long)envl("STMMQR_LA_MIN_FUSED", 1500),
                             (long long)envl("STMMQR_LA_FUSED_ROWS", 5120), (long long)envl("STMMQR_LA_MAXPWG", 48), (long long)envl("STMMQR_LA_SYSFENCE", 0),
-                            (long long)envl("STMMQR_SIDE_RESERVE", 32)})
+                            (long long)envl("STMMQR_SIDE_RESERVE", 32), (long long)P.panel_generic, (long long)envl("STMMQR_PANEL_PIPE", 1)})
             optkey = (optkey ^ v) * 1099511628211LL;
         if (!P.graph_exec || P.graph_tol != c.tol || P.graph_ntol != c.ntol || P.graph_dbg != c.dbg || P.graph_gen != P.sched_gen ||
             P.graph_opt != optkey) {
@@ -1458,9 +1486,19 @@
     } else
         e = run_schedule(P, detail != 0, group);
     if (!e && !P.whole_call && !P.serial_panels) {
-        int failed = 0;
-        HIPCHK(hipMemcpyAsync(&failed, P.d_abort.p + 1, sizeof(int), hipMemcpyDeviceToHost, P.stream));
+        int word[4] = {0, 0, 0, 0};
+        HIPCHK(hipMemcpyAsync(word, P.d_abort.p + 1, 4 * sizeof(int), hipMemcpyDeviceToHost, P.stream));
         HIPCHK(hipStreamSynchronize(P.stream));
+        const int failed = word[0];
+        if (word[3]) {
+            P.stats.panel_fallbacks++;
+            P.panel_generic = true;
+        }
+        if (word[3] && !failed) {
+            if (g_opt.verbose) fprintf(stderr, "[stmmqr_hip] a panel needed the in-place path in group %d: running it again with the generic panel kernels\n", group);
+            e = reset_group(P, group);
+            if (!e) e = run_schedule(P, detail != 0, group);
+        }
         if (failed) {
             if (g_opt.verbose) fprintf(stderr, "[stmmqr_hip] a panel wait ran out in group %d: running it again with one-workgroup panels\n", group);
             P.stats.retries++;
@@ -1626,17 +1664,28 @@
 {
     if (!plan) return fail(STMMQR_ERR_INVALID, "null plan");
     const bool detail = g_opt.verbose >= 2 || (stats && stats->nlaunch == -1);
-    int arena_retries = 0, reschedules = 0;
+    int arena_retries = 0, reschedules = 0, fallbacks = 0;
     for (int attempt = 0; attempt < 2; attempt++) {
         plan->serial_panels = (attempt == 1);
         plan->panel_wait_failed = false;
+        plan->pipe_guard_hit = false;
         plan->whole_call = true;
         int e = stmmqr_factorize_begin(plan, Ap, Ai, Ax, ax_on_device, tol, ntol);
         if (!e) plan->stats.retries = (attempt == 1 ? 1 : 0) + arena_retries;
         if (!e) plan->stats.reschedules = reschedules;
+        if (!e) plan->stats.panel_fallbacks = fallbacks;
         for (int g = 0; g < (int)plan->glevels.size() && !e; g++) e = stmmqr_factorize_group(plan, g, detail);
         if (!e) e = stmmqr_factorize_finish(plan, stats);
         plan->whole_call = false;
+        if (e && plan->pipe_guard_hit) {
+            plan->pipe_guard_hit = false;
+            plan->panel_wait_failed = false;
+            if (g_opt.verbose) fprintf(stderr, "[stmmqr_hip] a panel needed the in-place path: factorizing again with the generic panel kernels\n");
+            fallbacks++;
+            attempt = -1;
+            Ap = nullptr; Ai = nullptr;
+            continue;
+        }
         if (e && plan->arena_overflow && plan->recycle) {
             plan->arena_overflow = false;
             if (g_opt.verbose) fprintf(stderr, "[stmmqr_hip] R+H arena overflow: factorizing again %s\n", plan->overflowed ? "without slab recycling" : "with the arena at its hard bound");
@@ -1740,7 +1789,7 @@
     LCHK(grow(P.d_wcnt, P.wcnt_n));
     LCHK(grow(P.d_wcnt2, P.wcnt_n));
     LCHK(grow(P.d_wflag, P.wcnt_n));
-    if (!P.d_abort.p) LCHK(P.d_abort.alloc(4));
+    if (!P.d_abort.p) LCHK(P.d_abort.alloc(5));
     LCHK(grow(P.d_wflag2, P.wcnt_n));
     HIPCHK(hipMemset(P.d_wcnt.p, 0, P.wcnt_n * sizeof(int)));
     HIPCHK(hipMemset(P.d_wcnt2.p, 0, P.wcnt_n * sizeof(int)));
diff --git a/stm-multifrontal-qr-factorization-empowered-by-gcn_amd/csrc/stmmqr_kernels.h b/stm-multifrontal-qr-factorization-empowered-by-gcn_amd/csrc/stmmqr_kernels.h
--- a/stm-multifrontal-qr-factorization-empowered-by-gcn_amd/csrc/stmmqr_kernels.h
+++ b/stm-multifrontal-qr-factorization-empowered-by-gcn_amd/csrc/stmmqr_kernels.h
@@ -52,7 +52,8 @@
 int stm_launch_setup(const DevCtx &c, const int *flist, int nfr, hipStream_t st);
 int stm_launch_assemble(const DevCtx &c, const int *flist, const int *nparts, int nfr, int maxparts, hipStream_t st);
 int stm_launch_front_wg(const DevCtx &c, const int *flist, int nfr, int lds_doubles, hipStream_t st);
-int stm_launch_panel(const DevCtx &c, const int *flist, const int *plist, int nfr, int nsub, int defer_ok, int lds_doubles, hipStream_t st);
+int stm_launch_panel(const DevCtx &c, const int *flist, const int *plist, int nfr, int nsub, int defer_ok, int lds_doubles, hipStream_t st,
+                     int pipe = 0);
 int stm_configure_capanel(void);
 int stm_launch_panel_ca(const DevCtx &c, const int *flist, const int *plist, int nfr, int nw, int defer_ok, hipStream_t st);
 int stm_launch_panel_ca_pc(const DevCtx &c, const int *flist, const int *plist, int nfr, int nw, int defer_ok, const int *uflist,
@@ -62,7 +63,7 @@
                             const long long *wpoff, int *wcnt, int *wflag, int epoch, int with_gram, hipStream_t st);
 int stm_launch_panel_pc(const DevCtx &c, const int *flist, const int *plist, int nfr, int nsub, int defer_ok, int lds_doubles,
                         const int *uflist, const int *uplist, int unfr, int ucb0, int uncb, int umaxsl, const double *Wp,
-                        const long long *uwpoff, hipStream_t st);
+                        const long long *uwpoff, hipStream_t st, int pipe = 0);
 int stm_launch_update_fw(const DevCtx &c, const int *flist, const int *plist, int nfr, int ncb, int maxsl, double *Wp,
                          const long long *wpoff, int *wcnt, int *wflag, int epoch, double *Wp2, int *wcnt2, hipStream_t st);
 int stm_launch_update_w(const DevCtx &c, const int *flist, const int *plist, int nfr, int cb0, int ncb, int maxsl, double *Wp,
diff --git a/stm-multifrontal-qr-factorization-empowered-by-gcn_amd/csrc/stmmqr_panel.hip b/stm-multifrontal-qr-factorization-empowered-by-gcn_amd/csrc/stmmqr_panel.hip
--- a/stm-multifrontal-qr-factorization-empowered-by-gcn_amd/csrc/stmmqr_panel.hip
+++ b/stm-multifrontal-qr-factorization-empowered-by-gcn_amd/csrc/stmmqr_panel.hip
@@ -1161,8 +1161,10 @@
 
 #define NTP 512
 
+template <bool PIPE>
 __device__ __forceinline__ void dev_k_panel(const DevCtx &c, const int *__restrict__ flist, const int *__restrict__ plist, int fi, int b,
-                                            int nsub, int defer_ok, int lds_doubles, PanelShared &ps, WaveShared &wsh, double *dyn_lds)
+                                            int nsub, int defer_ok, int lds_doubles, PanelShared &ps, WaveShared &wsh, double *dyn_lds,
+                                            int guard_test = 0)
 {
     const int f = flist[fi];
     const int p = plist[fi];
@@ -1184,6 +1186,10 @@
     }
     bool tall = stm_tall_panel(s, p, c.tall_min) && !(c.dbg & 256);
     if (!tall && b > 0) return;
+    if (PIPE && !tall) {
+        if (threadIdx.x == 0 && c.abort) st_agent(c.abort + 4, 1);
+        return;
+    }
     if (tall) {
         const int k1 = p * STM_NB, k2 = min(s.fn, k1 + STM_NB), nbp = k2 - k1;
         int mode, g1, tmax, w;
@@ -1196,6 +1202,8 @@
             if (!was_done && tmax - g1 <= STM_WP_ROWS && !(c.dbg & 16384) &&
                 STM_NB * ((tmax - g1 <= 128) ? 128 : (tmax - g1 <= 256) ? 256 : 512) <= lds_doubles)
                 mode = 2;
+            const bool guard = PIPE && !was_done && (mode == 0 || guard_test);
+            if (guard) mode = 0;
             if ((c.dbg & 16) && c.dbgbuf && threadIdx.x == 0 && !was_done) {
                 const int rws = tmax - g1;
                 atomicAdd(&c.dbgbuf[32 + (rws <= 128 ? 0 : rws <= 256 ? 1 : rws <= 512 ? 2 : rws <= 1024 ? 3 : rws <= 2048 ? 4 : rws <= 4096 ? 5 : 6)], 1ull);
@@ -1205,10 +1213,11 @@
             if (threadIdx.x == 0) {
                 st_agent(&pd->mode, mode); st_agent(&pd->pg1, g1); st_agent(&pd->pt, g1); st_agent(&pd->tmax, tmax);
                 st_agent(&pd->nlive, 0); st_agent(&pd->sw, w); st_agent(&pd->done_group, -1);
-                if (was_done) { pd->pnb = 0; pd->t_deferred = 0; }
+                if (was_done || guard) { pd->pnb = 0; pd->t_deferred = 0; }
+                if (guard && c.abort) st_agent(c.abort + 4, 1);
             }
             publish_progress(&num->hdr, p + 1);
-            if (was_done) return;
+            if (was_done || guard) return;
         } else {
             if (!wait_progress(&num->hdr, p + 1)) { if (threadIdx.x == 0) STM_SET_PERR(c, num); return; }
             mode = ld_agent(&pd->mode); g1 = ld_agent(&pd->pg1); tmax = ld_agent(&pd->tmax); w = ld_agent(&pd->sw);
@@ -1235,6 +1244,7 @@
             return;
         }
     }
+    if constexpr (PIPE) return;
     const int lds_front = stm_front_lds(s);
     if ((c.dbg & 64) || lds_front > lds_doubles || panel_rows(s, num, St, p) > lds_front - 65)
         dev_panel<NTP, true>(ps, s, num, F, St, c.Tau + s.rp, c.Rdead + s.col1, p, c.tol, c.ntol, T, dyn_lds,
@@ -1245,38 +1255,67 @@
     if (threadIdx.x == 0) { pd->mode = 0; pd->t_deferred = 0; }
 }
 
+#define PANEL_LDS extern __shared__ double dyn_lds[]; __shared__ PanelShared ps; __shared__ WaveShared wsh
+template <bool PIPE>
+__device__ __forceinline__ void dev_panel_launch(const DevCtx &c, const int *__restrict__ flist, const int *__restrict__ plist, int nsub,
+                                                 int defer_ok, int lds_doubles, int guard_test, PanelShared &ps, WaveShared &wsh,
+                                                 double *dyn_lds)
+{
+    const unsigned long long t0c = clock64(), t0w = wall_clock64();
+    dev_k_panel<PIPE>(c, flist, plist, blockIdx.x, blockIdx.y, nsub, defer_ok, lds_doubles, ps, wsh, dyn_lds, guard_test);
+    if ((c.dbg & 16) && c.dbgbuf && threadIdx.x == 0) {
+        atomicAdd(&c.dbgbuf[44], clock64() - t0c); atomicAdd(&c.dbgbuf[45], wall_clock64() - t0w); atomicAdd(&c.dbgbuf[46], 1ull);
+    }
+}
 __global__ __launch_bounds__(NTP) void k_panel(DevCtx c, const int *__restrict__ flist, const int *__restrict__ plist, int nsub,
                                                int defer_ok, int lds_doubles)
 {
-    extern __shared__ double dyn_lds[];
-    __shared__ PanelShared ps;
-    __shared__ WaveShared wsh;
-    const unsigned long long t0c = clock64(), t0w = wall_clock64();
-    dev_k_panel(c, flist, plist, blockIdx.x, blockIdx.y, nsub, defer_ok, lds_doubles, ps, wsh, dyn_lds);
-    if ((c.dbg & 16) && c.dbgbuf && threadIdx.x == 0) {
-        atomicAdd(&c.dbgbuf[44], clock64() - t0c); atomicAdd(&c.dbgbuf[45], wall_clock64() - t0w); atomicAdd(&c.dbgbuf[46], 1ull);
-    }
-}
-
+    PANEL_LDS;
+    dev_panel_launch<false>(c, flist, plist, nsub, defer_ok, lds_doubles, 0, ps, wsh, dyn_lds);
+}
+__global__ __launch_bounds__(NTP) void k_panel_pipe(DevCtx c, const int *__restrict__ flist, const int *__restrict__ plist, int nsub,
+                                                    int defer_ok, int lds_doubles, int guard_test)
+{
+    PANEL_LDS;
+    dev_panel_launch<true>(c, flist, plist, nsub, defer_ok, lds_doubles, guard_test, ps, wsh, dyn_lds);
+}
+
+template <bool PIPE>
+__device__ __forceinline__ void dev_panel_pc_launch(const DevCtx &c, const int *__restrict__ flist, const int *__restrict__ plist, int npan,
+                                                    int nsub, int defer_ok, int lds_doubles, const int *__restrict__ uflist,
+                                                    const int *__restrict__ uplist, int ucb0, const double *Wp,
+                                                    const long long *__restrict__ uwpoff, int rspw, int guard_test, PanelShared &ps,
+                                                    WaveShared &wsh, double *dyn_lds)
+{
+    if (blockIdx.z == 0) {
+        if ((int)blockIdx.x >= npan || (int)blockIdx.y >= nsub) return;
+        const unsigned long long t0c = clock64(), t0w = wall_clock64();
+        dev_k_panel<PIPE>(c, flist, plist, blockIdx.x, blockIdx.y, nsub, defer_ok, lds_doubles, ps, wsh, dyn_lds, guard_test);
+        if ((c.dbg & 16) && c.dbgbuf && threadIdx.x == 0) {
+            atomicAdd(&c.dbgbuf[44], clock64() - t0c); atomicAdd(&c.dbgbuf[45], wall_clock64() - t0w); atomicAdd(&c.dbgbuf[46], 1ull);
+        }
+        return;
+    }
+    dev_upd_c_h2(c, uflist, uplist, ucb0, Wp, uwpoff, (int)blockIdx.z - 1, blockIdx.x, blockIdx.y, rspw, dyn_lds, ps.stair);
+}
 __global__ __launch_bounds__(NTP) void k_panel_pc(DevCtx c, const int *__restrict__ flist, const int *__restrict__ plist, int npan,
                                                   int nsub, int defer_ok, int lds_doubles, const int *__restrict__ uflist,
                                                   const int *__restrict__ uplist, int ucb0, const double *Wp,
                                                   const long long *__restrict__ uwpoff, int rspw)
 {
-    extern __shared__ double dyn_lds[];
-    __shared__ PanelShared ps;
-    __shared__ WaveShared wsh;
-    if (blockIdx.z == 0) {
-        if ((int)blockIdx.x >= npan || (int)blockIdx.y >= nsub) return;
-        const unsigned long long t0c = clock64(), t0w = wall_clock64();
-        dev_k_panel(c, flist, plist, blockIdx.x, blockIdx.y, nsub, defer_ok, lds_doubles, ps, wsh, dyn_lds);
-        if ((c.dbg & 16) && c.dbgbuf && threadIdx.x == 0) {
-            atomicAdd(&c.dbgbuf[44], clock64() - t0c); atomicAdd(&c.dbgbuf[45], wall_clock64() - t0w); atomicAdd(&c.dbgbuf[46], 1ull);
-        }
-        return;
-    }
-    dev_upd_c_h2(c, uflist, uplist, ucb0, Wp, uwpoff, (int)blockIdx.z - 1, blockIdx.x, blockIdx.y, rspw, dyn_lds, ps.stair);
-}
+    PANEL_LDS;
+    dev_panel_pc_launch<false>(c, flist, plist, npan, nsub, defer_ok, lds_doubles, uflist, uplist, ucb0, Wp, uwpoff, rspw, 0, ps, wsh, dyn_lds);
+}
+__global__ __launch_bounds__(NTP) void k_panel_pipe_pc(DevCtx c, const int *__restrict__ flist, const int *__restrict__ plist, int npan,
+                                                       int nsub, int defer_ok, int lds_doubles, const int *__restrict__ uflist,
+                                                       const int *__restrict__ uplist, int ucb0, const double *Wp,
+                                                       const long long *__restrict__ uwpoff, int rspw, int guard_test)
+{
+    PANEL_LDS;
+    dev_panel_pc_launch<true>(c, flist, plist, npan, nsub, defer_ok, lds_doubles, uflist, uplist, ucb0, Wp, uwpoff, rspw, guard_test, ps,
+                              wsh, dyn_lds);
+}
+#undef PANEL_LDS
 int stm_launch_front_wg(const DevCtx &c, const int *flist, int nfr, int lds_doubles, hipStream_t st)
 {
     if (nfr <= 0) return 0;
@@ -1285,7 +1324,8 @@
     hipLaunchKernelGGL(k_front_wg, dim3(nfr), dim3(NT), bytes, st, c, flist, (int)(bytes / sizeof(double)));
     return (int)hipGetLastError();
 }
-int stm_launch_panel(const DevCtx &c, const int *flist, const int *plist, int nfr, int nsub, int defer_ok, int lds_doubles, hipStream_t st)
+int stm_launch_panel(const DevCtx &c, const int *flist, const int *plist, int nfr, int nsub, int defer_ok, int lds_doubles, hipStream_t st,
+                     int pipe)
 {
     if (nfr <= 0) return 0;
     size_t bytes = (size_t)lds_doubles * sizeof(double);
@@ -1293,19 +1333,24 @@
     int K = nfr;
     if (nsub > 1 && (c.dbg & 512)) K = getenv("STMMQR_CHUNK") ? atoi(getenv("STMMQR_CHUNK")) : 1;
     if (K < 1) K = 1;
-    for (int i = 0; i < nfr; i += K)
-        hipLaunchKernelGGL(k_panel, dim3(nfr - i < K ? nfr - i : K, nsub), dim3(NTP), bytes, st, c, flist + i, plist + i, nsub, defer_ok,
-                           (int)(bytes / sizeof(double)));
+    for (int i = 0; i < nfr; i += K) {
+        if (pipe)
+            hipLaunchKernelGGL(k_panel_pipe, dim3(nfr - i < K ? nfr - i : K, nsub), dim3(NTP), bytes, st, c, flist + i, plist + i, nsub,
+                               defer_ok, (int)(bytes / sizeof(double)), pipe == 2 ? 1 : 0);
+        else
+            hipLaunchKernelGGL(k_panel, dim3(nfr - i < K ? nfr - i : K, nsub), dim3(NTP), bytes, st, c, flist + i, plist + i, nsub, defer_ok,
+                               (int)(bytes / sizeof(double)));
+    }
     return (int)hipGetLastError();
 }
 int stm_launch_panel_pc(const DevCtx &c, const int *flist, const int *plist, int nfr, int nsub, int defer_ok, int lds_doubles,
                         const int *uflist, const int *uplist, int unfr, int ucb0, int uncb, int umaxsl, const double *Wp,
-                        const long long *uwpoff, hipStream_t st)
+                        const long long *uwpoff, hipStream_t st, int pipe)
 {
     if (unfr <= 0 || uncb <= 0 || umaxsl <= 0 || (c.dbg & 512)) {
         if (unfr > 0 && uncb > 0 && umaxsl > 0)
             (void)stm_launch_update_c(c, uflist, uplist, unfr, ucb0, uncb, umaxsl, Wp, uwpoff, st);
-        return stm_launch_panel(c, flist, plist, nfr, nsub, defer_ok, lds_doubles, st);
+        return stm_launch_panel(c, flist, plist, nfr, nsub, defer_ok, lds_doubles, st, pipe);
     }
     if (nfr <= 0 && !(nfr < 0)) {
         return stm_launch_update_c(c, uflist, uplist, unfr, ucb0, uncb, umaxsl, Wp, uwpoff, st);
@@ -1328,8 +1373,12 @@
         if (force > 0) rspw = force;
     }
     const int uy = (umaxsl + rspw - 1) / rspw;
-    hipLaunchKernelGGL(k_panel_pc, dim3(nfr > uncb ? nfr : uncb, nsub > uy ? nsub : uy, 1 + unfr), dim3(NTP), bytes, st, c, flist,
-                       plist, nfr, nsub, defer_ok, lds_arg, uflist, uplist, ucb0, Wp, uwpoff, rspw);
+    if (pipe)
+        hipLaunchKernelGGL(k_panel_pipe_pc, dim3(nfr > uncb ? nfr : uncb, nsub > uy ? nsub : uy, 1 + unfr), dim3(NTP), bytes, st, c, flist,
+                           plist, nfr, nsub, defer_ok, lds_arg, uflist, uplist, ucb0, Wp, uwpoff, rspw, pipe == 2 ? 1 : 0);
+    else
+        hipLaunchKernelGGL(k_panel_pc, dim3(nfr > uncb ? nfr : uncb, nsub > uy ? nsub : uy, 1 + unfr), dim3(NTP), bytes, st, c, flist,
+                           plist, nfr, nsub, defer_ok, lds_arg, uflist, uplist, ucb0, Wp, uwpoff, rspw);
     return (int)hipGetLastError();
 }
 int stm_configure_update(void);
@@ -1340,6 +1389,8 @@
     CK(hipFuncSetAttribute((const void *)k_front_wg, hipFuncAttributeMaxDynamicSharedMemorySize, 122880));
     CK(hipFuncSetAttribute((const void *)k_panel, hipFuncAttributeMaxDynamicSharedMemorySize, 131072));
     CK(hipFuncSetAttribute((const void *)k_panel_pc, hipFuncAttributeMaxDynamicSharedMemorySize, 131072));
+    CK(hipFuncSetAttribute((const void *)k_panel_pipe, hipFuncAttributeMaxDynamicSharedMemorySize, 131072));
+    CK(hipFuncSetAttribute((const void *)k_panel_pipe_pc, hipFuncAttributeMaxDynamicSharedMemorySize, 131072));
     { int e = stm_configure_update(); if (e) return e; }
     { int e = stm_configure_sweep(); if (e) return e; }
     return stm_configure_resident();
diff --git a/stm-multifrontal-qr-factorization-empowered-by-gcn_amd/csrc/stmmqr_plan.h b/stm-multifrontal-qr-factorization-empowered-by-gcn_amd/csrc/stmmqr_plan.h
--- a/stm-multifrontal-qr-factorization-empowered-by-gcn_amd/csrc/stmmqr_plan.h
+++ b/stm-multifrontal-qr-factorization-empowered-by-gcn_amd/csrc/stmmqr_plan.h
@@ -89,6 +89,7 @@
     int nsub = 1, nca = 1, nca_use = 0, npipe_use = 0, maxcb = 0, maxsl = 0, split = 0;
     int lds_big = 0;
     int lds_plan = 0;
+    int pipe_ok = 1;
     int n_norm = 0, n_pk[4] = {0, 0, 0, 0};
     int maxsl_pk[4] = {0, 0, 0, 0}, maxcbp_po = 0;
     int n_sweep() const { return n_pk[0] + n_pk[1] + n_pk[2] + n_pk[3]; }
@@ -182,6 +183,8 @@
     bool whole_call = false;
     bool panel_wait_failed = false;
     bool serial_panels = false;
+    bool panel_generic = false;
+    bool pipe_guard_hit = false;
     long long rh_total = 0;
     long rank = 0;
     std::vector<FrontNum> h_fnum;
```
